# HazyResearch/flash-fft-conv

Measured on AMD Instinct MI355X. Metric: FFT-conv fwd+bwd seq/s, B=16 H=768 L=16384 fft=32768 bf16, higher is better.
Workload: dtype bf16; 1 GPU; FlashFFTConv(32768) B=16 H=768 L=16384 bf16, fwd+bwd incl. k->k_f and dk (BASELINE configs[1]); heads_per_rank=768, parallelism=head-shard x1 (no collective)

## Files before the change

flash-fft-conv_amd/csrc/ffc_body.h:

```cpp
#pragma once
#include <stdint.h>

#include "ffc_layout.h"
#include "ffc_plan.h"

#ifndef FFC_FN
#define FFC_FN inline __attribute__((always_inline))
#endif

namespace ffc {

struct ConvArgs {
  const void* u;
  const void* pregate;
  const void* postgate;
  void* y;
  const void* kf;
  const uint8_t* tab;
  PlanTabs t;
  int B, H, L;
  int npair;
  int nchunk, ppc;
  int conj_kf;
  int fast;
// ... 67 lines not shown
  template <bool CONJ, bool AFORM>
  static FFC_FN void cmm(A16& ore, A16& oim, const Op& d, const Mat& F, int ms_lim = 2) {
#pragma unroll
    for (int ms = 0; ms < 2; ms++) {
      if (ms >= ms_lim) continue;
      const W4& fr = F.w[ms][0];
      const W4& fi_re = F.w[ms][CONJ ? 1 : 2];
      const W4& fi_im = F.w[ms][CONJ ? 2 : 1];
      if (AFORM) {
        B::template mfma<DT>(ore, d.r[ms], fr);
        B::template mfma<DT>(oim, d.r[ms], fi_im);
        B::template mfma<DT>(ore, d.i[ms], fi_re);
        B::template mfma<DT>(oim, d.i[ms], fr);
      } else {
        B::template mfma<DT>(ore, fr, d.r[ms]);
        B::template mfma<DT>(oim, fi_im, d.r[ms]);
        B::template mfma<DT>(ore, fi_re, d.i[ms]);
        B::template mfma<DT>(oim, fr, d.i[ms]);
      }
    }
  }
  static FFC_FN void to_op(const A16& re, const A16& im, Op& o) {
#pragma unroll
    for (int ms = 0; ms < 2; ms++)
#pragma unroll
      for (int d = 0; d < 4; d++) {
        o.r[ms][d] = B::template pack<DT>(re[8 * ms + 2 * d], re[8 * ms + 2 * d + 1]);
        o.i[ms][d] = B::template pack<DT>(im[8 * ms + 2 * d], im[8 * ms + 2 * d + 1]);
      }
  }
  struct Mat2 { W4 w[2][2]; };
  static FFC_FN void load_mat2_issue(Mat2& m, const uint8_t* p, i32 lane) {
#pragma unroll
    for (int ms = 0; ms < 2; ms++)
#pragma unroll
      for (int f = 0; f < 2; f++) {
        U4 v = B::g_r128(p, lane + (ms * 3 + f) * 64);
        m.w[ms][f] = B::w4(v.x, v.y, v.z, v.w);
      }
  }
  static FFC_FN W4 neg4(const W4& x) {
    return B::w4(x[0] ^ B::uconst(0x80008000u), x[1] ^ B::uconst(0x80008000u), x[2] ^ B::uconst(0x80008000u), x[3] ^ B::uconst(0x80008000u));
  }
  template <bool AFORM>
  static FFC_FN void cmm2(A16& ore, A16& oim, const Op& d, const Mat2& F) {
#pragma unroll
    for (int ms = 0; ms < 2; ms++) {
      const W4 ni = neg4(d.i[ms]);
      if (AFORM) {
        B::template mfma<DT>(ore, d.r[ms], F.w[ms][0]);
        B::template mfma<DT>(oim, d.r[ms], F.w[ms][1]);
        B::template mfma<DT>(ore, ni, F.w[ms][1]);
        B::template mfma<DT>(oim, d.i[ms], F.w[ms][0]);
      } else {
        B::template mfma<DT>(ore, F.w[ms][0], d.r[ms]);
        B::template mfma<DT>(oim, F.w[ms][1], d.r[ms]);
        B::template mfma<DT>(ore, F.w[ms][1], ni);
        B::template mfma<DT>(oim, F.w[ms][0], d.i[ms]);
      }
    }
  }
  static FFC_FN void cmul(A16& re, A16& im, const CT16& t) { B::template cmul16<false>(re, im, t.re, t.im); }
  static FFC_FN void cmul_conj(A16& re, A16& im, const CT16& t) { B::template cmul16<true>(re, im, t.re, t.im); }
  static FFC_FN void cis_rev(i32 phase, float sign, f32* c, f32* s, int nmask = GEO::N - 1, float inv_n = 1.0f / (float)GEO::N) {
    f32 x = B::i2f(phase & nmask) * inv_n;
    f32 cc = B::cos_rev(x), ss = B::sin_rev(x);
    B::settle(cc, ss);
    *c = cc;
    *s = ss * sign;
  }
  static FFC_FN void chain8(i32 base, i32 step, float sign, float scale, f32 (&tr)[8], f32 (&ti)[8]) {
    f32 c0, s0, c1, s1, c8, s8;
    cis_rev(base, sign, &c0, &s0);
    cis_rev(step, sign, &c1, &s1);
    cis_rev(step * 8, sign, &c8, &s8);
    tr[0] = c0 * scale; ti[0] = s0 * scale;
    tr[4] = tr[0] * c8 - ti[0] * s8; ti[4] = tr[0] * s8 + ti[0] * c8;
#pragma unroll
    for (int i = 1; i < 4; i++) {
      tr[i] = tr[i - 1] * c1 - ti[i - 1] * s1; ti[i] = tr[i - 1] * s1 + ti[i - 1] * c1;
      tr[4 + i] = tr[3 + i] * c1 - ti[3 + i] * s1; ti[4 + i] = tr[3 + i] * s1 + ti[3 + i] * c1;
    }
  }
  using F2 = typename B::F2;
  static FFC_FN void chain8p(i32 base, i32 step, float sign, float scale, F2 (&tr)[4], F2 (&ti)[4],
                             int nmask = GEO::N - 1, float inv_n = 1.0f / (float)GEO::N, f32* w8c = nullptr, f32* w8s = nullptr) {
    f32 c0, s0, c1, s1, c8, s8;
    cis_rev(base, sign, &c0, &s0, nmask, inv_n);
    cis_rev(step, sign, &c1, &s1, nmask, inv_n);
    cis_rev(step * 8, sign, &c8, &s8, nmask, inv_n);
    c0 = c0 * scale; s0 = s0 * scale;
    f32 c2 = c1 * c1 - s1 * s1, s2 = (c1 + c1) * s1;
    tr[0] = B::f2(c0, c0 * c1 - s0 * s1);
    ti[0] = B::f2(s0, c0 * s1 + s0 * c1);
    B::cmulp(tr[0], ti[0], c2, s2, tr[1], ti[1]);
    B::cmulp(tr[0], ti[0], c8, s8, tr[2], ti[2]);
    B::cmulp(tr[1], ti[1], c8, s8, tr[3], ti[3]);
    if (w8c) { *w8c = c8; *w8s = s8; }
  }
  static FFC_FN void apply8(A16& re, A16& im, int half, const F2 (&tr)[4], const F2 (&ti)[4]) {
#pragma unroll
    for (int i = 0; i < 4; i++) B::template cmul2v<false>(re, im, 8 * half + 2 * i, tr[i], ti[i]);
  }
  static constexpr bool CHAIN16_A = GEO::N1 == 32 && (!B::LEAN_OUTER || GEO::N2 == 32);
  static FFC_FN void twiddle16(A16& re, A16& im, i32 base, i32 step, float sign, float scale,
                               int nmask = GEO::N - 1, float inv_n = 1.0f / (float)GEO::N) {
    F2 tr[4], ti[4];
    f32 c8, s8;
    chain8p(base, step, sign, scale, tr, ti, nmask, inv_n, &c8, &s8);
    apply8(re, im, 0, tr, ti);
    const f32 c16 = c8 * c8 - s8 * s8, s16 = (c8 + c8) * s8;
#pragma unroll
    for (int i = 0; i < 4; i++) B::cmulp(tr[i], ti[i], c16, s16, tr[i], ti[i]);
    apply8(re, im, 1, tr, ti);
  }
#ifndef FFC_PK_GATE
#define FFC_PK_GATE 1
#endif
  static FFC_FN u32 mul2(u32 a, u32 g) {
    if constexpr (DT == DT_F16 && FFC_PK_GATE != 0) return B::pk_mul_f16(a, g);
    f32 lo = B::template unpack_lo<DT>(a) * B::template unpack_lo<DT>(g);
    f32 hi = B::template unpack_hi<DT>(a) * B::template unpack_hi<DT>(g);
    return B::template pack<DT>(lo, hi);
  }
  static FFC_FN void xpose(const U2 (&raw)[8], int t, W4& op) {
#pragma unroll
    for (int d = 0; d < 4; d++) {
      u32 a = (t < 2) ? raw[2 * d].x : raw[2 * d].y;
      u32 b = (t < 2) ? raw[2 * d + 1].x : raw[2 * d + 1].y;
      op[d] = (t & 1) ? ((a >> 16) | (b & 0xffff0000u)) : ((a & 0xffffu) | (b << 16));
    }
  }

  static FFC_FN void xpose2(const U2 (&raw)[8], int tp, int th, W4& op) {
#pragma unroll
    for (int d = 0; d < 4; d++) {
      u32 a = tp ? raw[2 * d].y : raw[2 * d].x;
      u32 b = tp ? raw[2 * d + 1].y : raw[2 * d + 1].x;
      op[d] = th ? ((a >> 16) | (b & 0xffff0000u)) : ((a & 0xffffu) | (b << 16));
    }
  }

  static FFC_FN void copy_tab(const uint8_t* src, int lds_off, int bytes) {
    const i32 tid = B::lane() + B::wave() * 64;
    for (int i = 0; i < bytes / 16; i += GEO::WGW * 64) {
      i32 idx = tid + i;
      pred ok = idx < bytes / 16;
      U4 v = B::g_r128p(src, idx, ok);
      B::lds_w128(idx * 16 + lds_off, v, ok);
    }
  }
  static constexpr int TAB_T = GEO::WGW * 64;
  template <int BYTES>
  static FFC_FN void tab_issue(const uint8_t* src, U4 (&v)[(BYTES / 16 + TAB_T - 1) / TAB_T]) {
    const i32 tid = B::lane() + B::wave() * 64;
#pragma unroll
    for (int it = 0; it < (BYTES / 16 + TAB_T - 1) / TAB_T; it++) v[it] = B::g_r128(src, B::imin(tid + it * TAB_T, BYTES / 16 - 1));
  }
  template <int BYTES>
  static FFC_FN void tab_commit(int lds_off, const U4 (&v)[(BYTES / 16 + TAB_T - 1) / TAB_T]) {
    const i32 tid = B::lane() + B::wave() * 64;
#pragma unroll
    for (int it = 0; it < (BYTES / 16 + TAB_T - 1) / TAB_T; it++) {
      i32 idx = tid + it * TAB_T;
      B::lds_w128(idx * 16 + lds_off, v[it], idx < BYTES / 16);
    }
  }
  static FFC_FN void setup_tables(const uint8_t* tab, const PlanTabs& t) {
    U4 f1[(6144 / 16 + TAB_T - 1) / TAB_T], f2[(6144 / 16 + TAB_T - 1) / TAB_T], f3[(6144 / 16 + TAB_T - 1) / TAB_T],
       tw[(8192 / 16 + TAB_T - 1) / TAB_T], tw2[(8192 / 16 + TAB_T - 1) / TAB_T], fs[(3072 / 16 + TAB_T - 1) / TAB_T];
    if constexpr (GEO::OUTER) tab_issue<6144>(tab + t.mat[0], f1);
    tab_issue<6144>(tab + t.mat[1], f2);
    tab_issue<8192>(tab + t.twin, tw);
    if constexpr (GEO::N3 != GEO::N2) tab_issue<6144>(tab + t.mat[2], f3);
    if constexpr (GEO::TW2_SEP) tab_issue<8192>(tab + t.twin2, tw2);
    if constexpr (GEO::HAS_SP) tab_issue<3072>(tab + t.mat_sp, fs);
    B::sched_fence();
    if constexpr (GEO::OUTER) tab_commit<6144>(GEO::L_F1, f1);
    tab_commit<6144>(GEO::L_F2, f2);
    tab_commit<8192>(GEO::L_TW, tw);
    if constexpr (GEO::N3 != GEO::N2) tab_commit<6144>(GEO::L_F3, f3);
    if constexpr (GEO::TW2_SEP) tab_commit<8192>(GEO::L_TW2, tw2);
    if constexpr (GEO::HAS_SP) tab_commit<3072>(GEO::L_FS, fs);
    B::barrier();
  }
  static FFC_FN void lds_mat(Mat& m, int off) {
    const i32 lane = B::lane();
#pragma unroll
    for (int q = 0; q < 6; q++) {
      U4 v = B::lds_r128(lane * 16 + (off + q * 1024));
      m.w[q / 3][q % 3] = B::w4(v.x, v.y, v.z, v.w);
    }
#pragma unroll
    for (int q = 0; q < 6; q++) B::pin(m.w[q / 3][q % 3]);
  }
  static FFC_FN void lds_ct16(CT16& c, int off) {
    const i32 lane = B::lane();
#pragma unroll
    for (int rr = 0; rr < 8; rr++) {
      U4 v = B::lds_r128(lane * 16 + (off + rr * 1024));
      c.re[2 * rr] = B::as_f32(v.x); c.re[2 * rr + 1] = B::as_f32(v.y);
      c.im[2 * rr] = B::as_f32(v.z); c.im[2 * rr + 1] = B::as_f32(v.w);
    }
  }
  template <bool CONJ>
  static FFC_FN void cmul_lds(A16& re, A16& im, int off) {
    const i32 lane = B::lane();
#pragma unroll
    for (int rr = 0; rr < 8; rr++) {
      U4 v = B::lds_r128(lane * 16 + (off + rr * 1024));
      B::template cmul2<CONJ>(re, im, 2 * rr, B::as_f32(v.x), B::as_f32(v.y), B::as_f32(v.z), B::as_f32(v.w));
    }
  }
  static FFC_FN void cmul_small(CT16& t, int off) {
    const i32 hi = B::lane() >> 5;
#pragma unroll
    for (int rr = 0; rr < 8; rr++) {
      U4 v = B::lds_r128(hi * 128 + (off + rr * 16));
      f32 br[2] = {B::as_f32(v.x), B::as_f32(v.z)}, bi[2] = {B::as_f32(v.y), B::as_f32(v.w)};
#pragma unroll
      for (int q = 0; q < 2; q++) {
        int r = 2 * rr + q;
        f32 x = t.re[r], y = t.im[r];
        t.re[r] = x * br[q] - y * bi[q];
        t.im[r] = x * bi[q] + y * br[q];
      }
    }
  }

  struct Unit { int eb; int wq; };
  static FFC_FN Pass make_pass(const ConvArgs& a, int k0) {
    Pass ps;
    ps.k0 = k0; ps.R = a.R;
    ps.mat_fwd = a.tab + a.t.matk[k0][0]; ps.mat_inv = a.tab + a.t.matk[k0][1];
    return ps;
  }

  static FFC_FN int64_t row_off(int b, bool ok, int64_t sb, int h, int L) { return (int64_t)(ok ? b : 0) * sb + (int64_t)h * L; }
  struct RowIO {
    const uint16_t* src[2]; const uint16_t* gate[2]; uint16_t* dst[2]; bool valid[2];
  };
  static FFC_FN U4 gload8(const uint16_t* base, i32 n, int L, int fast, bool rowok) {
    if (B::FAST_ONLY || fast) return fast == 2 ? B::g_r128_nt(base, B::imin(n, L - 8) >> 3) : B::g_r128(base, B::imin(n, L - 8) >> 3);
    u32 w[4];
#pragma unroll
    for (int q = 0; q < 4; q++) {
      u32 lo = B::g_r16(base, n + 2 * q, ((n + 2 * q) < L) && rowok);
      u32 hi = B::g_r16(base, n + (2 * q + 1), ((n + (2 * q + 1)) < L) && rowok);
      w[q] = lo | (hi << 16);
    }
    U4 v; v.x = w[0]; v.y = w[1]; v.z = w[2]; v.w = w[3];
    return v;
  }
  static FFC_FN void gstore8(uint16_t* base, i32 n, int L, int fast, bool rowok, U4 v) {
    if (B::FAST_ONLY || fast) {
      if (fast == 2) B::g_w128_nt(base, n >> 3, v, (n < L) && rowok);
      else B::g_w128(base, n >> 3, v, (n < L) && rowok);
      return;
    }
    u32 w[4] = {v.x, v.y, v.z, v.w};
#pragma unroll
    for (int q = 0; q < 4; q++) {
      B::g_w16(base, n + 2 * q, w[q] & 0xffffu, ((n + 2 * q) < L) && rowok);
      B::g_w16(base, n + (2 * q + 1), w[q] >> 16, ((n + (2 * q + 1)) < L) && rowok);
    }
  }
  static FFC_FN i32 pair_off(i32 row, i32 m, pred* swapped) {
    i32 n2 = m / GEO::N3, n3 = m % GEO::N3;
    i32 sig = (n2 / GEO::PER) % GEO::CR;
    *swapped = (sig & 1) >= 1;
    return row * (GEO::Mi * 2) + (n2 * GEO::CR + (((n3 >> 3) ^ (sig >> 1)) << 1)) * 8;
  }
  static constexpr int CPR = GEO::OUTER ? 16 * GEO::S1 : GEO::Mi / 8;
  static constexpr int NCH = GEO::OUTER ? 8 : 2;

  template <int NC> struct RowRegsT { U4 v[NC][2]; };
  using RowRegs = RowRegsT<NCH>;
  template <int NC, int I0 = 0>
  static FFC_FN void rows_load(const ConvArgs& a, int h, int pq, Unit un, RowRegsT<NC>& X) {
    const i32 lane = B::opaque(B::lane());
    const int fast = a.fast ? (a.stream ? 2 : 1) : 0;
    if constexpr (!GEO::OUTER) {
      if (fast) {
#pragma unroll
        for (int ii = 0; ii < NC; ii++) {
          i32 idx = lane + (ii + I0) * 64;
          i32 row = idx / CPR, m = (idx % CPR) * 8;
#pragma unroll
          for (int pl = 0; pl < 2; pl++) {
            i32 b = (row + pq * GEO::G) * 2 + pl;
            X.v[ii][pl] = gload8_rows((const uint16_t*)a.u, b, h, a, a.sbu, m, 1, b < a.B);
          }
        }
        return;
      }
    }
#pragma unroll
    for (int ii = 0; ii < NC; ii++) {
      const int i = ii + I0;
      i32 idx = lane + i * 64;
      i32 row = idx / CPR, m = (idx % CPR) * 8 + (GEO::OUTER ? un.wq * 128 * GEO::S1 : 0);
#pragma unroll
      for (int pl = 0; pl < 2; pl++) {
        if constexpr (GEO::OUTER) {
          if (fast && ((i * 64) / CPR) * GEO::Mi >= a.L) { X.v[ii][pl] = U4{B::uconst(0), B::uconst(0), B::uconst(0), B::uconst(0)}; continue; }
          const int b = 2 * pq + pl;
          const bool ok = b < a.B;
          const int64_t ro = row_off(b, ok, a.sbu, h, a.L);
          X.v[ii][pl] = gload8((const uint16_t*)a.u + ro, row * GEO::Mi + m, a.L, fast, ok);
        } else {
          i32 b = (row + pq * GEO::G) * 2 + pl;
          X.v[ii][pl] = gload8_rows((const uint16_t*)a.u, b, h, a, a.sbu, m, fast, b < a.B);
        }
      }
    }
  }
#ifndef FFC_GATE_BATCH
#define FFC_GATE_BATCH 4
#endif
  template <int NC, int I0>
  static FFC_FN void rows_store_g(const ConvArgs& a, int h, int pq, Unit un, const RowRegsT<NC>& X) {
    constexpr int GB = FFC_GATE_BATCH <= 0 ? 1 : (NC < FFC_GATE_BATCH ? NC : FFC_GATE_BATCH);
    static_assert(NC % GB == 0, "gate batch");
    const i32 lane = B::opaque(B::lane());
    const int fast = a.stream ? 2 : 1;
    const bool hasg = a.pregate != nullptr, hasa = a.aux_in != nullptr;
#pragma unroll
    for (int ib = 0; ib < NC; ib += GB) {
      U4 G[GB][2], A[GB][2];
#pragma unroll
      for (int jj = 0; jj < GB; jj++) {
        const int i = ib + jj + I0;
        i32 idx = lane + i * 64;
        i32 row = idx / CPR, m = (idx % CPR) * 8 + (GEO::OUTER ? un.wq * 128 * GEO::S1 : 0);
        if (GEO::OUTER && ((i * 64) / CPR) * GEO::Mi >= a.L) continue;
#pragma unroll
        for (int pl = 0; pl < 2; pl++) {
          if constexpr (GEO::OUTER) {
            const int b = 2 * pq + pl;
            const bool ok = b < a.B;
            const i32 n = row * GEO::Mi + m;
            if (hasg) G[jj][pl] = gload8((const uint16_t*)a.pregate + row_off(b, ok, a.sbg, h, a.L), n, a.L, fast, ok);
            if (hasa) A[jj][pl] = gload8((const uint16_t*)a.aux_in + row_off(b, ok, a.sbai, h, a.L), n, a.L, fast, ok);
          } else {
            i32 b = (row + pq * GEO::G) * 2 + pl;
            if (hasg) G[jj][pl] = gload8_rows((const uint16_t*)a.pregate, b, h, a, a.sbg, m, fast, b < a.B);
            if (hasa) A[jj][pl] = gload8_rows((const uint16_t*)a.aux_in, b, h, a, a.sbai, m, fast, b < a.B);
          }
        }
      }
      B::sched_fence();
#pragma unroll
      for (int jj = 0; jj < GB; jj++) {
        const int ii = ib + jj, i = ii + I0;
        i32 idx = lane + i * 64;
        i32 row = idx / CPR, m = (idx % CPR) * 8 + (GEO::OUTER ? un.wq * 128 * GEO::S1 : 0);
        pred sw;
        i32 off = pair_off(row, m, &sw) + un.eb;
        const bool beyond = GEO::OUTER && ((i * 64) / CPR) * GEO::Mi >= a.L;
#pragma unroll
        for (int pl = 0; pl < 2; pl++) {
          U4 v = X.v[ii][pl];
          if (GEO::OUTER) {
            pred ok = ((row * GEO::Mi + m) < a.L) && ((2 * pq + pl) < a.B);
            v.x = B::sel(ok, v.x, B::uconst(0)); v.y = B::sel(ok, v.y, B::uconst(0));
            v.z = B::sel(ok, v.z, B::uconst(0)); v.w = B::sel(ok, v.w, B::uconst(0));
          }
          if (hasa && !beyond) {
            if constexpr (GEO::OUTER) {
              const int b = 2 * pq + pl;
              const bool ok = b < a.B;
              gstore8((uint16_t*)a.aux_out + row_off(b, ok, a.sbao, h, a.L), row * GEO::Mi + m, a.L, fast, ok, mul4(v, A[jj][pl]));
            } else {
              i32 b = (row + pq * GEO::G) * 2 + pl;
              gstore8_rows((uint16_t*)a.aux_out, b, h, a, a.sbao, m, fast, b < a.B, mul4(v, A[jj][pl]));
            }
          }
          if (hasg && !beyond) v = mul4(v, G[jj][pl]);
          U4 o;
          o.x = B::sel(sw, v.z, v.x); o.y = B::sel(sw, v.w, v.y);
          o.z = B::sel(sw, v.x, v.z); o.w = B::sel(sw, v.y, v.w);
          B::lds_w128(off + pl * GEO::PLANE, o, B::ptrue());
        }
      }
    }
  }
  template <int NC, int I0 = 0>
  static FFC_FN void rows_store(const ConvArgs& a, int h, int pq, Unit un, const RowRegsT<NC>& X) {
    if constexpr (FFC_GATE_BATCH > 0) {
      if (a.fast && (a.pregate || a.aux_in)) { rows_store_g<NC, I0>(a, h, pq, un, X); return; }
    }
    const i32 lane = B::opaque(B::lane());
    const int fast = a.fast ? (a.stream ? 2 : 1) : 0;
#pragma unroll
    for (int ii = 0; ii < NC; ii++) {
      const int i = ii + I0;
      i32 idx = lane + i * 64;
      i32 row = idx / CPR, m = (idx % CPR) * 8 + (GEO::OUTER ? un.wq * 128 * GEO::S1 : 0);
      pred sw;
      i32 off = pair_off(row, m, &sw) + un.eb;
#pragma unroll
      for (int pl = 0; pl < 2; pl++) {
        U4 v = X.v[ii][pl];
        if (fast && GEO::OUTER) {
          pred ok = ((row * GEO::Mi + m) < a.L) && ((2 * pq + pl) < a.B);
          v.x = B::sel(ok, v.x, B::uconst(0)); v.y = B::sel(ok, v.y, B::uconst(0));
          v.z = B::sel(ok, v.z, B::uconst(0)); v.w = B::sel(ok, v.w, B::uconst(0));
        }
        if (a.aux_in && !(GEO::OUTER && fast && ((i * 64) / CPR) * GEO::Mi >= a.L)) {
          if constexpr (GEO::OUTER) {
            const int b = 2 * pq + pl;
            const bool ok = b < a.B;
            const i32 n = row * GEO::Mi + m;
            U4 r = gload8((const uint16_t*)a.aux_in + row_off(b, ok, a.sbai, h, a.L), n, a.L, fast, ok);
            gstore8((uint16_t*)a.aux_out + row_off(b, ok, a.sbao, h, a.L), n, a.L, fast, ok, mul4(v, r));
          } else {
            i32 b = (row + pq * GEO::G) * 2 + pl;
            U4 r = gload8_rows((const uint16_t*)a.aux_in, b, h, a, a.sbai, m, fast, b < a.B);
            gstore8_rows((uint16_t*)a.aux_out, b, h, a, a.sbao, m, fast, b < a.B, mul4(v, r));
          }
        }
        if (a.pregate && !(GEO::OUTER && fast && ((i * 64) / CPR) * GEO::Mi >= a.L)) {
          U4 g;
          if constexpr (GEO::OUTER) {
            const int b = 2 * pq + pl;
            const bool ok = b < a.B;
            const int64_t ro = row_off(b, ok, a.sbg, h, a.L);
            g = gload8((const uint16_t*)a.pregate + ro, row * GEO::Mi + m, a.L, fast, ok);
          } else {
            i32 b = (row + pq * GEO::G) * 2 + pl;
            g = gload8_rows((const uint16_t*)a.pregate, b, h, a, a.sbg, m, fast, b < a.B);
          }
          v.x = mul2(v.x, g.x); v.y = mul2(v.y, g.y); v.z = mul2(v.z, g.z); v.w = mul2(v.w, g.w);
        }
        U4 o;
        o.x = B::sel(sw, v.z, v.x); o.y = B::sel(sw, v.w, v.y);
        o.z = B::sel(sw, v.x, v.z); o.w = B::sel(sw, v.y, v.w);
        B::lds_w128(off + pl * GEO::PLANE, o, B::ptrue());
      }
    }
  }
  template <int NC = NCH>
  static FFC_FN void rows_in(const ConvArgs& a, int h, int pq, Unit un) {
    RowRegsT<NC> X;
    rows_load<NC>(a, h, pq, un, X);
    rows_store<NC>(a, h, pq, un, X);
  }
  static constexpr bool HAS_DMA = GEO::OUTER && GEO::N1 == 32 && GEO::S1 == 1;
  static constexpr int DMA_ROW0 = GEO::N1 / 2;
  static FFC_FN void rows_dma(const ConvArgs& a, int h, int pq, Unit un) {
    if (a.stream) rows_dma_t<true>(a, h, pq, un);
    else rows_dma_t<false>(a, h, pq, un);
  }
  template <bool NT>
  static FFC_FN void rows_dma_t(const ConvArgs& a, int h, int pq, Unit un) {
    const i32 lane = B::opaque(B::lane());
#pragma unroll
    for (int pl = 0; pl < 2; pl++) {
      const int b = 2 * pq + pl;
      const uint16_t* base = (const uint16_t*)a.u + row_off(b < a.B ? b : a.B - 1, true, a.sbu, h, a.L);
#pragma unroll
      for (int r = 0; r < GEO::N1 / 2; r++) {
        i32 n = B::imin(lane * 2 + (r * GEO::Mi + un.wq * 128), a.L - 2);
        B::template g2lds32<NT>(base, n >> 1, un.eb + pl * GEO::PLANE + (DMA_ROW0 + r) * (GEO::Mi * 2) + un.wq * 256);
      }
    }
  }
  static FFC_FN void rows_dma_finish(const ConvArgs& a, int pq, Unit un) {
    B::vm_wait0();
    const i32 lane = B::opaque(B::lane());
#pragma unroll
    for (int pl = 0; pl < 2; pl++) {
      const bool ok = (2 * pq + pl) < a.B;
#pragma unroll
      for (int r = 0; r < GEO::N1 / 2; r++) {
        if (ok && (r + 1) * GEO::Mi <= a.L) continue;
        i32 n = lane * 2 + (r * GEO::Mi + un.wq * 128);
        B::lds_w32p(lane * 4 + (un.eb + pl * GEO::PLANE + (DMA_ROW0 + r) * (GEO::Mi * 2) + un.wq * 256), B::uconst(0),
                    B::pnot((n < a.L) && ok));
      }
    }
    B::lds_fence();
  }

  static FFC_FN U4 gload8_rows(const uint16_t* base, i32 b, int h, const ConvArgs& a, int64_t sb, i32 n, int fast, pred ok) {
    const int sbi = (int)sb;
    if (fast) {
      i32 o16 = b * (sbi >> 3) + (h * (a.L >> 3) + (n >> 3));
      return B::g_r128p(base, o16, ok && (n < a.L));
    }
    u32 w[4];
#pragma unroll
    for (int q = 0; q < 4; q++) {
      i32 e0 = b * sbi + (h * a.L + n + 2 * q);
      u32 lo = B::g_r16(base, e0, ok && ((n + 2 * q) < a.L));
      u32 hi = B::g_r16(base, e0 + 1, ok && ((n + (2 * q + 1)) < a.L));
      w[q] = lo | (hi << 16);
    }
    U4 v; v.x = w[0]; v.y = w[1]; v.z = w[2]; v.w = w[3];
    return v;
  }
  static FFC_FN void gstore8_rows(uint16_t* base, i32 b, int h, const ConvArgs& a, int64_t sb, i32 n, int fast, pred ok, U4 v) {
    const int sbi = (int)sb;
    if (fast) {
      i32 o16 = b * (sbi >> 3) + (h * (a.L >> 3) + (n >> 3));
      B::g_w128(base, o16, v, ok && (n < a.L));
      return;
    }
    u32 w[4] = {v.x, v.y, v.z, v.w};
#pragma unroll
    for (int q = 0; q < 4; q++) {
      i32 e0 = b * sbi + (h * a.L + n + 2 * q);
      B::g_w16(base, e0, w[q] & 0xffffu, ok && ((n + 2 * q) < a.L));
      B::g_w16(base, e0 + 1, w[q] >> 16, ok && ((n + (2 * q + 1)) < a.L));
    }
  }

#ifndef FFC_GATE_BATCH_OUT
#define FFC_GATE_BATCH_OUT FFC_GATE_BATCH
#endif
  template <int NC, bool ADD = false, bool GATE = true>
  static FFC_FN void rows_out_g(const ConvArgs& a, int h, int pq, Unit un) {
    static_assert(ADD || GATE, "rows_out_g: nothing to load");
    constexpr int GB = FFC_GATE_BATCH_OUT <= 0 ? 1 : (NC < FFC_GATE_BATCH_OUT ? NC : FFC_GATE_BATCH_OUT);
    static_assert(NC % GB == 0, "gate batch");
    const i32 lane = B::opaque(B::lane());
    const int fast = a.stream ? 2 : 1;
#pragma unroll
    for (int ib = 0; ib < NC; ib += GB) {
      U4 G[GB][2], Rr[GB][2];
#pragma unroll
      for (int jj = 0; jj < GB; jj++) {
        const int i = ib + jj;
        i32 idx = lane + i * 64;
        i32 row = idx / CPR, m = (idx % CPR) * 8 + (GEO::OUTER ? un.wq * 128 * GEO::S1 : 0);
#pragma unroll
        for (int pl = 0; pl < 2; pl++) {
          if constexpr (GEO::OUTER) {
            const int b = 2 * pq + pl;
            const bool ok = b < a.B;
            if constexpr (GATE) G[jj][pl] = gload8((const uint16_t*)a.postgate + row_off(b, ok, a.sbp, h, a.L), row * GEO::Mi + m, a.L, fast, ok);
            if constexpr (ADD) Rr[jj][pl] = gload8((const uint16_t*)a.addend + row_off(b, ok, a.sba, h, a.L), row * GEO::Mi + m, a.L, fast, ok);
          } else {
            i32 b = (row + pq * GEO::G) * 2 + pl;
            if constexpr (GATE) G[jj][pl] = gload8_rows((const uint16_t*)a.postgate, b, h, a, a.sbp, m, fast, b < a.B);
            if constexpr (ADD) Rr[jj][pl] = gload8_rows((const uint16_t*)a.addend, b, h, a, a.sba, m, fast, b < a.B);
          }
        }
      }
      B::sched_fence();
#pragma unroll
      for (int jj = 0; jj < GB; jj++) {
        const int i = ib + jj;
        i32 idx = lane + i * 64;
        i32 row = idx / CPR, m = (idx % CPR) * 8 + (GEO::OUTER ? un.wq * 128 * GEO::S1 : 0);
        pred sw;
        i32 off = pair_off(row, m, &sw) + un.eb;
#pragma unroll
        for (int pl = 0; pl < 2; pl++) {
          U4 o = B::lds_r128(off + pl * GEO::PLANE);
          U4 v;
          v.x = B::sel(sw, o.z, o.x); v.y = B::sel(sw, o.w, o.y);
          v.z = B::sel(sw, o.x, o.z); v.w = B::sel(sw, o.y, o.w);
          if constexpr (ADD && GATE) v = fma4(v, G[jj][pl], Rr[jj][pl]);
          else if constexpr (ADD) v = sum4(v, Rr[jj][pl]);
          else v = mul4(v, G[jj][pl]);
          if constexpr (GEO::OUTER) {
            const int b = 2 * pq + pl;
            const bool ok = b < a.B;
            gstore8((uint16_t*)a.y + row_off(b, ok, a.sby, h, a.L), row * GEO::Mi + m, a.L, fast, ok, v);
          } else {
            i32 b = (row + pq * GEO::G) * 2 + pl;
            gstore8_rows((uint16_t*)a.y, b, h, a, a.sby, m, fast, b < a.B, v);
          }
        }
      }
    }
  }
  template <int NC = NCH, bool ADD = B::HAS_ADD>
  static FFC_FN void rows_out(const ConvArgs& a, int h, int pq, Unit un) {
    if constexpr (FFC_GATE_BATCH > 0) {
      if (a.fast && a.postgate) { rows_out_g<NC, ADD>(a, h, pq, un); return; }
      if constexpr (ADD) {
        if (a.fast) { rows_out_g<NC, true, false>(a, h, pq, un); return; }
      }
    }
    const i32 lane = B::opaque(B::lane());
    const int fast = a.fast ? (a.stream ? 2 : 1) : 0;
#pragma unroll
    for (int i = 0; i < NC; i++) {
      i32 idx = lane + i * 64;
      i32 row = idx / CPR, m = (idx % CPR) * 8 + (GEO::OUTER ? un.wq * 128 * GEO::S1 : 0);
      pred sw;
      i32 off = pair_off(row, m, &sw) + un.eb;
#pragma unroll
      for (int pl = 0; pl < 2; pl++) {
        U4 o = B::lds_r128(off + pl * GEO::PLANE);
        U4 v;
        v.x = B::sel(sw, o.z, o.x); v.y = B::sel(sw, o.w, o.y);
// ... 1202 lines not shown
    kf_mul<SZ>(a, kfB, reB, imB); to_op(reB, imB, opB);
    reB = B::a16_zero(); imB = B::a16_zero();
    cmm<true, true>(reB, imB, opB, R.F2);
    cmul_conj(reA, imA, R.tw); to_op(reA, imA, opA);
    reA = B::a16_zero(); imA = B::a16_zero();
    cmm<true, true>(reA, imA, opA, R.F2);
    cmul_conj(reB, imB, R.tw); to_op(reB, imB, opB);
    reB = B::a16_zero(); imB = B::a16_zero();
    cmm<true, true>(reB, imB, opB, R.F2);
    oi_twiddle<RP>(a.s_inv, tauA, reA, imA, ps);
    tile_store(tauA, R, reA, imA);
    oi_twiddle<RP>(a.s_inv, tauB, reB, imB, ps);
    tile_store(tauB, R, reB, imB);
  }

  template <bool SZ>
  static FFC_FN void inner_tile2x_fold(const ConvArgs& a, int h, int tau, const InnerRegs& R, Unit un, uint8_t* zsA, uint8_t* zsB) {
    static_assert(CAN_FOLD && GEO::UPW >= 2, "folded outer twiddle, two units per workgroup");
    constexpr int DB = GEO::EBYTES;
    const i32 lane = B::opaque(B::lane());
    const uint8_t* fold = a.tab + a.t.fold;
    Mat2 FA, FB, GB, GA;
    load_mat2_issue(FA, fold + (0 * GEO::NT + tau) * 6144, lane);
    KfRegs kf;
    load_kf(a, h, tau, kf);
    Op opA, opB;
    load_tile_op(tau, opA, un, R);
    load_tile_op(tau, opB, un, R, DB);
    load_mat2_issue(FB, fold + (1 * GEO::NT + tau) * 6144, lane);
    A16 reA, imA, reB, imB;
    reA = B::a16_zero(); imA = B::a16_zero();
    cmm2<true>(reA, imA, opA, FA);
    reB = B::a16_zero(); imB = B::a16_zero();
    cmm2<true>(reB, imB, opB, FA);
    load_mat2_issue(GB, fold + (2 * GEO::NT + tau) * 6144, lane);
    cmul(reA, imA, R.tw); to_op(reA, imA, opA);
    reA = B::a16_zero(); imA = B::a16_zero();
    cmm2<false>(reA, imA, opA, FB);
    cmul(reB, imB, R.tw); to_op(reB, imB, opB);
    reB = B::a16_zero(); imB = B::a16_zero();
    cmm2<false>(reB, imB, opB, FB);
    load_mat2_issue(GA, fold + (3 * GEO::NT + tau) * 6144, lane);
    if constexpr (SZ) { z_store(zsA, tau, reA, imA, Z_STREAM); z_store(zsB, tau, reB, imB, Z_STREAM); }
    {
      CT16 k;
#pragma unroll
      for (int rq = 0; rq < 4; rq++) {
        u32 wv[4] = {kf.v[rq].x, kf.v[rq].y, kf.v[rq].z, kf.v[rq].w};
#pragma unroll
        for (int q = 0; q < 4; q++) {
          k.re[4 * rq + q] = B::template unpack_lo<DT>(wv[q]);
          k.im[4 * rq + q] = B::template unpack_hi<DT>(wv[q]);
        }
      }
      if constexpr (!SZ) k.im = B::a16_scale(k.im, a.conj_kf ? -1.0f : 1.0f);
      cmul(reA, imA, k); to_op(reA, imA, opA);
      reA = B::a16_zero(); imA = B::a16_zero();
      cmm2<true>(reA, imA, opA, GB);
      cmul(reB, imB, k); to_op(reB, imB, opB);
      reB = B::a16_zero(); imB = B::a16_zero();
      cmm2<true>(reB, imB, opB, GB);
    }
    cmul_conj(reA, imA, R.tw); to_op(reA, imA, opA);
    reA = B::a16_zero(); imA = B::a16_zero();
    cmm2<true>(reA, imA, opA, GA);
    cmul_conj(reB, imB, R.tw); to_op(reB, imB, opB);
    reB = B::a16_zero(); imB = B::a16_zero();
    cmm2<true>(reB, imB, opB, GA);
    tile_store(tau, R, reA, imA);
    tile_store(tau, R, reB, imB, DB);
  }
  template <bool SZ = false>
  static FFC_FN void inner_tile2x(const ConvArgs& a, int h, int tau, const InnerRegs& R, Unit un, uint8_t* zsA = nullptr, uint8_t* zsB = nullptr) {
    static_assert(GEO::N3 == GEO::N2 && GEO::OUTER && GEO::UPW >= 2, "inner_tile2x: two units per workgroup");
    constexpr int DB = GEO::EBYTES;
    KfRegs kf;
    load_kf(a, h, tau, kf);
    Op opA, opB;
    load_tile_op(tau, opA, un, R);
    load_tile_op(tau, opB, un, R, DB);
    A16 reA, imA, reB, imB;
    reA = B::a16_zero(); imA = B::a16_zero();
    cmm<false, true>(reA, imA, opA, R.F2);
    reB = B::a16_zero(); imB = B::a16_zero();
    cmm<false, true>(reB, imB, opB, R.F2);
    cmul(reA, imA, R.tw); to_op(reA, imA, opA);
    reA = B::a16_zero(); imA = B::a16_zero();
    cmm<false, false>(reA, imA, opA, R.F2);
    cmul(reB, imB, R.tw); to_op(reB, imB, opB);
    reB = B::a16_zero(); imB = B::a16_zero();
    cmm<false, false>(reB, imB, opB, R.F2);
    if constexpr (SZ) { z_store(zsA, tau, reA, imA, Z_STREAM); z_store(zsB, tau, reB, imB, Z_STREAM); }
    {
      CT16 k;
#pragma unroll
      for (int rq = 0; rq < 4; rq++) {
        u32 wv[4] = {kf.v[rq].x, kf.v[rq].y, kf.v[rq].z, kf.v[rq].w};
#pragma unroll
        for (int q = 0; q < 4; q++) {
          k.re[4 * rq + q] = B::template unpack_lo<DT>(wv[q]);
          k.im[4 * rq + q] = B::template unpack_hi<DT>(wv[q]);
        }
      }
      if constexpr (!SZ) k.im = B::a16_scale(k.im, a.conj_kf ? -1.0f : 1.0f);
      cmul(reA, imA, k); to_op(reA, imA, opA);
      reA = B::a16_zero(); imA = B::a16_zero();
      cmm<true, true>(reA, imA, opA, R.F2);
      cmul(reB, imB, k); to_op(reB, imB, opB);
      reB = B::a16_zero(); imB = B::a16_zero();
      cmm<true, true>(reB, imB, opB, R.F2);
    }
    cmul_conj(reA, imA, R.tw); to_op(reA, imA, opA);
    reA = B::a16_zero(); imA = B::a16_zero();
    cmm<true, true>(reA, imA, opA, R.F2);
    cmul_conj(reB, imB, R.tw); to_op(reB, imB, opB);
    reB = B::a16_zero(); imB = B::a16_zero();
    cmm<true, true>(reB, imB, opB, R.F2);
    {
      const i32 lane = B::opaque(B::lane());
      const i32 c = lane & 31, hi = lane >> 5;
      const i32 sUl = c / GEO::N2, mlane = (c % GEO::N2) * GEO::N3;
      if constexpr (GEO::N3 == 32) {
        i32 k1 = sUl * GEO::SV + tau * GEO::G;
        F2 tr[4], ti[4];
        f32 c8, s8;
        chain8p(B::mul24(mlane + hi * 4, k1), k1, 1.0f, a.s_inv, tr, ti, GEO::N - 1, 1.0f / (float)GEO::N, &c8, &s8);
        apply8(reA, imA, 0, tr, ti);
        apply8(reB, imB, 0, tr, ti);
        const f32 c16 = c8 * c8 - s8 * s8, s16 = (c8 + c8) * s8;
#pragma unroll
        for (int i = 0; i < 4; i++) B::cmulp(tr[i], ti[i], c16, s16, tr[i], ti[i]);
        apply8(reA, imA, 1, tr, ti);
        apply8(reB, imB, 1, tr, ti);
      } else
#pragma unroll
      for (int half = 0; half < 2; half++) {
        const int sV = (16 * half) / GEO::N3;
        i32 k1 = sUl * GEO::SV + (sV + tau * GEO::G);
        i32 n30 = hi * 4 + ((16 * half) % GEO::N3);
        F2 tr[4], ti[4];
        chain8p(B::mul24(mlane + n30, k1), k1, 1.0f, a.s_inv, tr, ti);
        apply8(reA, imA, half, tr, ti);
        apply8(reB, imB, half, tr, ti);
      }
    }
    tile_store(tau, R, reA, imA);
    tile_store(tau, R, reB, imB, DB);
  }

  static FFC_FN void unit_barrier() {
    if constexpr (GEO::NW > 1) B::barrier();
    else B::lds_fence();
  }
  template <bool HALF, bool PROF = false, bool RP = false, bool SZ = false, bool SP = false, bool GS = false>
  static FFC_FN void outer_jobs(const ConvArgs& a, int h, int p0, int p1, int u, Unit un, int wg_linear = 0) {
    static_assert(!GS || (HALF && !RP && !SP && HALF_C), "direct-store phase C: single-pass fft 32768, L <= N/2");
    constexpr int NC = HALF ? NCH / 2 : NCH;
    constexpr bool PREFETCH = HALF && !RP;
    constexpr bool FOLDF = CAN_FOLD && !RP && !SP && !PROF && !B::LEAN_OUTER;
    constexpr bool CROSS = !SP && !RP && !PROF && !B::LEAN_OUTER && GEO::N3 == GEO::N2 && GEO::NW > 1 && GEO::UPW >= 2;
    const int npass = RP ? a.R : 1;
    const int iters = ((p1 - p0 + GEO::UPW - 1) / GEO::UPW) * npass;
    RowRegsT<NC> X;
    if constexpr (PREFETCH) { if (p0 + u < p1) rows_load<NC>(a, h, p0 + u, un, X); }
    unsigned long long acc[8] = {0, 0, 0, 0, 0, 0, 0, 0}, t0 = 0, t1 = 0;
#define FFC_TICK(k) if (PROF) { t1 = B::clock(); acc[k] += t1 - t0; t0 = t1; }
    const bool second = B::wave() >= 4;
#define FFC_PRIO(x) if constexpr (GEO::NW > 1) B::template setprio<x>();
#pragma unroll 1
    for (int it = 0; it < iters; it++) {
      const int p = p0 + (RP ? it / npass : it) * GEO::UPW + u;
      const Pass ps = RP ? make_pass(a, it % npass) : Pass();
      const int hk = RP ? h * ps.R + ps.k0 : h;
      const bool act = p < p1;
      if (PROF) t0 = B::clock();
      FFC_PRIO(1)
      if (act) {
        if constexpr (RP) {
          rows_in_rp<NC>(a, h, p, un, ps);
        } else {
          if constexpr (!PREFETCH) rows_load<NC>(a, h, p, un, X);
          rows_store<NC>(a, h, p, un, X);
        }
        B::lds_fence();
        FFC_TICK(0)
        FFC_PRIO(0)
        outer_stage<true, HALF, RP, false, FOLDF>(a.L, un, a.s_fwd, ps);
        FFC_TICK(1)
      }
      unit_barrier();
      FFC_TICK(2)
      if constexpr (CROSS) {
        const int ug = u >> 1, wl = (u & 1) * GEO::NW + un.wq;
        const int pA = p0 + it * GEO::UPW + 2 * ug;
        if (pA < p1) {
          Unit ua;
          ua.eb = 2 * ug * GEO::EBYTES; ua.wq = wl;
          InnerRegs R;
          load_inner(R, ua);
          uint8_t* zA = SZ ? z_slot(a.zsave, h, a.npair, pA) : nullptr;
          if (pA + 1 < p1) {
#pragma unroll 1
            for (int tt = 0; tt < 2; tt++) {
              if (tt == 0) { FFC_PRIO(3) } else if (second) { FFC_PRIO(2) } else { FFC_PRIO(1) }
              if constexpr (FOLDF) inner_tile2x_fold<SZ>(a, hk, wl * 2 + tt, R, ua, zA, zA + (int64_t)GEO::N * 4);
              else inner_tile2x<SZ>(a, hk, wl * 2 + tt, R, ua, zA, zA + (int64_t)GEO::N * 4);
            }
          } else {
            inner_tile2<false, SZ, FOLDF, HALF>(a, hk, wl * 2, R, ua, Pass(), zA);
          }
        }
      } else if (act) {
        InnerRegs R;
        load_inner(R, un);
        if constexpr (SP) {
          Mat Fs;
          lds_mat_sp(Fs);
#pragma unroll 1
          for (int tt = 0; tt < GEO::TPW; tt += 2) inner_tile2_sp(a, hk, un.wq * GEO::TPW + tt, R, Fs, un);
        } else if constexpr (GEO::N3 == GEO::N2) {
#pragma unroll 1
          for (int tt = 0; tt < GEO::TPW; tt += 2) {
            if (tt == 0) { FFC_PRIO(3) } else if (second) { FFC_PRIO(2) } else { FFC_PRIO(1) }
            inner_tile2<RP, SZ, FOLDF, HALF>(a, hk, un.wq * GEO::TPW + tt, R, un, ps,
                                SZ ? (RP ? z_slot_rp(a.zsave, h, a.npair, p, ps.R, ps.k0) : z_slot(a.zsave, h, a.npair, p)) : nullptr);
          }
        } else {
          KfRegs kf0;
          load_kf(a, h, un.wq * GEO::TPW, kf0);
#pragma unroll 1
          for (int tt = 0; tt < GEO::TPW; tt++) {
            KfRegs kfn;
            if (tt + 1 < GEO::TPW) load_kf(a, h, un.wq * GEO::TPW + tt + 1, kfn);
            inner_tile(a, un.wq * GEO::TPW + tt, R, un, kf0);
            kf0 = kfn;
          }
        }
      }
      FFC_TICK(3)
      unit_barrier();
      FFC_TICK(4)
      FFC_PRIO(3)
      if constexpr (PREFETCH) { if (it + 1 < iters && p + GEO::UPW < p1) rows_load<NC>(a, h, p + GEO::UPW, un, X); }
      if constexpr (GS) {
        if (act) {
          outer_inv_half<true>(un, &a, h, p);
          FFC_TICK(5)
        }
      } else if (act) {
        outer_stage<false, HALF, RP>(a.L, un, 1.0f, ps, a.flags);
        B::lds_fence();
        FFC_TICK(5)
        FFC_PRIO(2)
        if constexpr (SZ) {
          if (a.yraw) {
            ConvArgs ar = a;
            ar.y = a.yraw; ar.postgate = nullptr; ar.addend = nullptr; ar.sby = (int64_t)a.H * a.L;
            if constexpr (RP) rows_out_rp<NC, false>(ar, h, p, un, ps);
            else rows_out<NC, false>(ar, h, p, un);
          }
        }
        if constexpr (RP) rows_out_rp<NC>(a, h, p, un, ps);
        else rows_out<NC>(a, h, p, un);
        FFC_TICK(6)
      }
    }
#undef FFC_TICK
#undef FFC_PRIO
    if (PROF && a.prof) {
      const i32 lane = B::lane();
      unsigned long long* dst = a.prof + ((long long)wg_linear * GEO::WGW + B::wave()) * 8;
#pragma unroll
      for (int k = 0; k < 8; k++) B::g_w64(dst, lane * 0 + k, B::u2_from64(acc[k]), lane < 1);
    }
  }

  template <bool HALF = false, bool SZ = false, bool SP = false, bool GS = false>
  static FFC_FN void conv(const ConvArgs& a, int h, int chunk) {
    setup_tables(a.tab, a.t);
    conv_job<HALF, false, SZ, SP, GS>(a, h, chunk);
  }
  template <bool HALF = false, bool RP = false, bool SZ = false, bool SP = false, bool GS = false>
  static FFC_FN void conv_job(const ConvArgs& a, int h, int chunk) {
    const int wv = B::wave();
    Unit un;
    un.wq = wv % GEO::NW;
    const int u = wv / GEO::NW;
    un.eb = u * GEO::EBYTES;
    const int p0 = chunk * a.ppc;
    int p1 = p0 + a.ppc;
    if (p1 > a.npair) p1 = a.npair;
    if constexpr (GEO::OUTER) {
      outer_jobs<HALF, false, RP, SZ, SP, GS>(a, h, p0, p1, u, un);
    } else {
      const int q0 = p0 / GEO::G, q1 = (p1 + GEO::G - 1) / GEO::G;
      const int iters = (q1 - q0 + GEO::UPW - 1) / GEO::UPW;
      InnerRegs R;
      load_inner(R, un);
      if constexpr (RP) {
        static_assert(GEO::G == 1, "inner-only multi-pass: one pair per tile");
#ifndef FFC_IP_MERGE
#define FFC_IP_MERGE 1
#endif
        if (FFC_IP_MERGE != 0 && a.fast && a.L <= GEO::N && !a.aux_in) {
          const i32 lane = B::opaque(B::lane());
#pragma unroll 1
          for (int it = 0; it < iters; it++) {
            const int q = q0 + it * GEO::UPW + u;
            if (q >= q1) continue;
            RowRegs X, Y;
            rows_load<NCH>(a, h, q, un, X);
            if (a.pregate) {
              RowRegs G;
#pragma unroll
              for (int ii = 0; ii < NCH; ii++) {
                i32 idx = lane + ii * 64;
                i32 m = (idx % CPR) * 8;
#pragma unroll
                for (int pl = 0; pl < 2; pl++) {
                  i32 b = (idx / CPR + q * GEO::G) * 2 + pl;
                  G.v[ii][pl] = gload8_rows((const uint16_t*)a.pregate, b, h, a, a.sbg, m, 1, b < a.B);
                }
              }
#pragma unroll
              for (int ii = 0; ii < NCH; ii++)
#pragma unroll
                for (int pl = 0; pl < 2; pl++) X.v[ii][pl] = mul4(X.v[ii][pl], G.v[ii][pl]);
            }
#pragma unroll 1
            for (int k0 = 0; k0 < a.R; k0++) {
              InnerPass ip;
              load_inner_pass(ip, k0);
              KfRegs kf;
              load_kf(a, h * a.R + k0, 0, kf);
#pragma unroll
              for (int ii = 0; ii < NCH; ii++) {
                i32 idx = lane + ii * 64;
                pred sw;
                i32 off = pair_off(idx / CPR, (idx % CPR) * 8, &sw) + un.eb;
#pragma unroll
                for (int pl = 0; pl < 2; pl++) {
                  const U4& v = X.v[ii][pl];
                  U4 o;
                  o.x = B::sel(sw, v.z, v.x); o.y = B::sel(sw, v.w, v.y);
                  o.z = B::sel(sw, v.x, v.z); o.w = B::sel(sw, v.y, v.w);
                  B::lds_w128(off + pl * GEO::PLANE, o, B::ptrue());
                }
              }
              B::lds_fence();
              inner_tile<true, SZ>(a, 0, R, un, kf, &ip, (SZ && a.zsave) ? z_slot_small(a.zsave, h, a.npair, q, a.R, k0) : nullptr);
              B::lds_fence();
#pragma unroll
              for (int ii = 0; ii < NCH; ii++) {
                i32 idx = lane + ii * 64;
                pred sw;
                i32 off = pair_off(idx / CPR, (idx % CPR) * 8, &sw) + un.eb;
#pragma unroll
                for (int pl = 0; pl < 2; pl++) {
                  U4 o = B::lds_r128(off + pl * GEO::PLANE);
                  U4 v;
                  v.x = B::sel(sw, o.z, o.x); v.y = B::sel(sw, o.w, o.y);
                  v.z = B::sel(sw, o.x, o.z); v.w = B::sel(sw, o.y, o.w);
                  if (k0 == 0) Y.v[ii][pl] = v;
                  else Y.v[ii][pl] = add4(Y.v[ii][pl], v, 1.0f);
                }
              }
              B::lds_fence();
            }
#pragma unroll
            for (int ii = 0; ii < NCH; ii++) {
              i32 idx = lane + ii * 64;
              i32 m = (idx % CPR) * 8;
#pragma unroll
              for (int pl = 0; pl < 2; pl++) {
                i32 b = (idx / CPR + q * GEO::G) * 2 + pl;
                U4 v = Y.v[ii][pl];
                if constexpr (SZ) {
                  if (a.yraw) gstore8_rows((uint16_t*)a.yraw, b, h, a, (int64_t)a.H * a.L, m, 1, b < a.B, v);
                }
                if constexpr (B::HAS_ADD) {
                  U4 r = gload8_rows((const uint16_t*)a.addend, b, h, a, a.sba, m, 1, b < a.B);
                  if (a.postgate) v = fma4(v, gload8_rows((const uint16_t*)a.postgate, b, h, a, a.sbp, m, 1, b < a.B), r);
                  else v = sum4(v, r);
                } else {
                  if (a.postgate) v = mul4(v, gload8_rows((const uint16_t*)a.postgate, b, h, a, a.sbp, m, 1, b < a.B));
                }
                gstore8_rows((uint16_t*)a.y, b, h, a, a.sby, m, 1, b < a.B, v);
              }
            }
          }
          return;
        }
#pragma unroll 1
        for (int it = 0; it < iters * a.R; it++) {
          const int q = q0 + (it / a.R) * GEO::UPW + u;
          const int k0 = it % a.R;
          if (q < q1) {
            Pass ps; ps.k0 = k0; ps.R = a.R;
            InnerPass ip;
            load_inner_pass(ip, k0);
            KfRegs kf;
            load_kf(a, h * a.R + k0, 0, kf);
            rows_in_rp<NCH>(a, h, q, un, ps);
            B::lds_fence();
            inner_tile<true, SZ>(a, 0, R, un, kf, &ip, (SZ && a.zsave) ? z_slot_small(a.zsave, h, a.npair, q, a.R, k0) : nullptr);
            B::lds_fence();
            if constexpr (SZ) {
              if (a.yraw) {
                ConvArgs ar = a;
                ar.y = a.yraw; ar.postgate = nullptr; ar.addend = nullptr; ar.sby = (int64_t)a.H * a.L;
                rows_out_rp<NCH, false>(ar, h, q, un, ps);
              }
            }
            rows_out_rp<NCH>(a, h, q, un, ps);
            B::lds_fence();
          }
        }
        return;
      }
#pragma unroll 1
      for (int it = 0; it < iters; it++) {
        const int q = q0 + it * GEO::UPW + u;
        const bool act = q < q1;
        if (act) {
          KfRegs kf;
          load_kf(a, h, 0, kf);
          rows_in(a, h, q, un);
          B::lds_fence();
          inner_tile<false, SZ>(a, 0, R, un, kf, nullptr, (SZ && a.zsave) ? z_slot_small(a.zsave, h, a.npair, q, 1, 0) : nullptr);
          B::lds_fence();
          if constexpr (SZ) {
            if (a.yraw) {
              ConvArgs ar = a;
              ar.y = a.yraw; ar.postgate = nullptr; ar.addend = nullptr; ar.sby = (int64_t)a.H * a.L;
              rows_out<NCH, false>(ar, h, q, un);
            }
          }
          rows_out(a, h, q, un);
        }
      }
    }
  }
};

}
```

flash-fft-conv_amd/csrc/ffc_bwd_launch.h:

```cpp
#pragma once
#ifndef FFC_GATE_BATCH
#define FFC_GATE_BATCH 1
#define FFC_GATE_BATCH_OUT 2
#endif
#include "ffc_dev.h"
using namespace ffc;

template <class GEO, int DT, bool HALF, int ZM, bool GS = false>
__global__ __launch_bounds__(GEO::WGW * 64, 2) __attribute__((amdgpu_num_vgpr(128))) void bwd_kernel(DkfArgs d) {
  if constexpr (GEO::NW == 1) {
    const int total = ((d.c.H + 7) & ~7) * d.c.nchunk;
    for (int id = blockIdx.x; id < total; id += gridDim.x) {
      int h, chunk;
      if (map_id(id, d.c.H, d.c.nchunk, &h, &chunk)) Modes<DevBO, GEO, DT>::template bwd<HALF, false, true, ZM>(d, h, chunk, blockIdx.x);
    }
  } else {
    int h, chunk;
    if (!map_block(d.c.H, d.c.nchunk, &h, &chunk)) return;
    stagger_start(d.c.flags);
    Modes<DevBO, GEO, DT>::template bwd<HALF, false, true, ZM, GS>(d, h, chunk, blockIdx.x);
  }
}
template <class GEO, int DT>
__global__ __launch_bounds__(GEO::WGW * 64, 2) void bwd_kernel_small(DkfArgs d) {
  using M = Modes<DevB, GEO, DT>;
  M::BD::setup_tables(d.c.tab, d.c.t);
  if constexpr (GEO::N == 1024) { if (d.c.R > 1) M::BD::setup_tables_ipass(d.c.tab, d.c.t, d.c.R); }
  const int total = ((d.c.H + 7) & ~7) * d.c.nchunk;
  for (int id = blockIdx.x; id < total; id += gridDim.x) {
    int h, chunk;
    if (map_id(id, d.c.H, d.c.nchunk, &h, &chunk)) M::template bwd<false, false, false>(d, h, chunk, id);
  }
}
template <class GEO, int DT, bool HALF, int ZM, bool FASTK>
__global__ __launch_bounds__(GEO::WGW * 64, 2) __attribute__((amdgpu_num_vgpr(128))) void bwd_rp_kernel(DkfArgs d) {
  using BK = typename std::conditional<FASTK, DevBOF, DevBO>::type;
  int h, chunk;
  if (!map_block(d.c.H, d.c.nchunk, &h, &chunk)) return;
  Modes<BK, GEO, DT>::BD::setup_tables(d.c.tab, d.c.t);
  const int wv = DevBO::wave(), wg = blockIdx.x;
#pragma unroll 1
  for (int k0 = 0; k0 < d.c.R; k0++) Modes<BK, GEO, DT>::template bwd<HALF, true, true, ZM>(d, h, chunk, wg, k0, wv);
}

template <int ZM>
struct BwdLaunchZ {
template <class GEO, int DT>
struct T {
  static int run(const DkfArgs& d, hipStream_t st) {
    static_assert(Body<DevB, GEO, DT>::IPASS_BYTES == IPASS_BYTES, "ffc_route.h");
    const BwdRoute r = bwd_route<GEO>(d, false);
    if (r.err) return ffc_fail(r.err);
    constexpr int T_ = GEO::WGW * 64;
    if constexpr (!GEO::OUTER && ZM != 0) {
      return ffc_fail("single-tile sizes are launched by the recomputing unit (run-time spectrum switch)");
    } else if constexpr (!GEO::OUTER) {
      return ffc_launch(bwd_kernel_small<GEO, DT>, "bwd_kernel", r.grid, T_, r.lds_max, r.lds, st, d);
    } else if (r.gs) {
      if constexpr (GEO::N == 32768)
        return ffc_launch(bwd_kernel<GEO, DT, true, ZM, true>, "bwd_kernel (direct store)", r.grid, T_, r.lds_max, r.lds, st, d);
      else
        return ffc_fail("internal: the backward route names a kernel that does not exist");
    } else {
      return pick([&](auto mp, auto half, auto fastk) -> int {
        constexpr bool MP = decltype(mp)::value, HALF = decltype(half)::value, FASTK = decltype(fastk)::value;
        if constexpr (MP && GEO::N == 32768)
          return ffc_launch(bwd_rp_kernel<GEO, DT, HALF, ZM, FASTK>, "bwd_rp_kernel", r.grid, T_, r.lds_max, r.lds, st, d);
        else if constexpr (!MP && !FASTK)
          return ffc_launch(bwd_kernel<GEO, DT, HALF, ZM>, "bwd_kernel", r.grid, T_, r.lds_max, r.lds, st, d);
        else
          return ffc_fail("internal: the backward route names a kernel that does not exist");
      }, r.multi_pass, r.half, r.fastk);
    }
  }
};
};
```

flash-fft-conv_amd/csrc/ffc_conv_launch.h:

```cpp
#pragma once
#include "ffc_dev.h"

template <class FAM>
struct ConvLaunch {
template <class GEO, int DT>
struct T {
  static int run(const ffc::ConvArgs& a, hipStream_t st) {
    using namespace ffc;
    static_assert(Body<DevB, GEO, DT>::IPASS_BYTES == IPASS_BYTES, "ffc_route.h");
    const FwdRoute r = fwd_route<GEO>(a);
    if (r.err) return ffc_fail(r.err);
    if (r.gs) {
      if constexpr (!FAM::HAS_ADD && GEO::N == 32768)
        return pick([&](auto sz) -> int {
          return ffc_launch(FAM::template kernel_gs<GEO, DT, decltype(sz)::value>(), FAM::what(false, decltype(sz)::value, false, true), r.grid, GEO::WGW * 64, r.lds_max, r.lds, st, a);
        }, r.sz);
      else
        return ffc_fail("internal: the forward route names a kernel that does not exist");
    }
    return pick([&](auto mp, auto half, auto sz, auto sp) -> int {
      constexpr bool MP = decltype(mp)::value, HALF = decltype(half)::value, SZ = decltype(sz)::value, SP = decltype(sp)::value;
      if constexpr (fwd_kernel_exists<GEO>(FAM::HAS_ADD, MP, HALF, SZ, SP))
        return ffc_launch(FAM::template kernel<GEO, DT, MP, HALF, SZ, SP>(), FAM::what(MP, SZ, SP, GEO::OUTER), r.grid, GEO::WGW * 64, r.lds_max, r.lds, st, a);
      else
        return ffc_fail("internal: the forward route names a kernel that does not exist");
    }, r.multi_pass, r.half, r.sz, r.sp);
  }
};
};
```

flash-fft-conv_amd/csrc/ffc_k_conv.hip:

```cpp
#include "ffc_conv_launch.h"
using namespace ffc;

static constexpr int SMALL_WAVES = 2;
template <class GEO, int DT, bool HALF, bool SZ = false, bool SP = false, bool GS = false>
__global__ __launch_bounds__(GEO::WGW * 64, GEO::OUTER ? 2 : SMALL_WAVES) void conv_kernel(ConvArgs a) {
  using BD = Body<DevB, GEO, DT>;
  if constexpr (GEO::OUTER && GEO::NW == 1) {
    BD::setup_tables(a.tab, a.t);
    const int total = ((a.H + 7) & ~7) * a.nchunk;
    for (int id = blockIdx.x; id < total; id += gridDim.x) {
      int h, chunk;
      if (map_id(id, a.H, a.nchunk, &h, &chunk)) BD::template conv_job<HALF, false, SZ>(a, h, chunk);
    }
  } else if constexpr (!GEO::OUTER) {
    BD::setup_tables(a.tab, a.t);
    const int total = ((a.H + 7) & ~7) * a.nchunk;
    for (int id = blockIdx.x; id < total; id += gridDim.x) {
      int h, chunk;
      if (map_id(id, a.H, a.nchunk, &h, &chunk)) BD::template conv_job<HALF, false, SZ>(a, h, chunk);
    }
  } else {
    int h, chunk;
    if (!map_block(a.H, a.nchunk, &h, &chunk)) return;
    stagger_start(a.flags);
    if constexpr (GEO::NW > 1 && !SP) {
      BD::setup_tables(a.tab, a.t);
      if (a.kfuse_k || a.kfuse_x) Modes<DevB, GEO, DT>::kfft_head(a, h);
      BD::template conv_job<HALF, false, SZ, SP, GS>(a, h, chunk);
    } else {
      BD::template conv<HALF, SZ, SP, GS>(a, h, chunk);
    }
  }
}

template <class GEO, int DT, bool HALF, bool SZ = false>
__global__ __launch_bounds__(GEO::WGW * 64, 2) void conv_rp_kernel(ConvArgs a) {
  using BD = Body<DevB, GEO, DT>;
  if constexpr (!GEO::OUTER) {
    BD::setup_tables(a.tab, a.t);
    BD::setup_tables_ipass(a.tab, a.t, a.R);
    const int total = ((a.H + 7) & ~7) * a.nchunk;
    for (int id = blockIdx.x; id < total; id += gridDim.x) {
      int h, chunk;
      if (map_id(id, a.H, a.nchunk, &h, &chunk)) BD::template conv_job<HALF, true, SZ>(a, h, chunk);
    }
  } else {
    int h, chunk;
    if (!map_block(a.H, a.nchunk, &h, &chunk)) return;
    BD::setup_tables(a.tab, a.t);
    BD::template conv_job<HALF, true, SZ>(a, h, chunk);
  }
}

struct ConvKernels {
  static constexpr bool HAS_ADD = false;
  template <class GEO, int DT, bool MP, bool HALF, bool SZ, bool SP>
  static constexpr auto kernel() {
    if constexpr (MP) return conv_rp_kernel<GEO, DT, HALF, SZ>;
    else return conv_kernel<GEO, DT, HALF, SZ, SP>;
  }
  template <class GEO, int DT, bool SZ>
  static constexpr auto kernel_gs() { return conv_kernel<GEO, DT, true, SZ, false, true>; }
  static const char* what(bool mp, bool sz, bool sp, bool outer) {
    if (mp) return sz && outer ? "conv_rp_kernel (spectrum-saving)" : "conv_rp_kernel";
    if (sz) return outer ? "conv_kernel (spectrum-saving)" : "conv_kernel (spectrum-saving, single tile)";
    return sp ? "conv_kernel (frequency-sparse)" : "conv_kernel";
  }
};
template __global__ void conv_kernel<Geo<1, 16, 16>, DT_BF16, true>(ConvArgs);
template __global__ void conv_kernel<Geo<1, 16, 16>, DT_F16, true>(ConvArgs);
template __global__ void conv_kernel<Geo<1, 16, 32>, DT_BF16, true>(ConvArgs);
template __global__ void conv_kernel<Geo<1, 16, 32>, DT_F16, true>(ConvArgs);
template __global__ void conv_kernel<Geo<1, 32, 32>, DT_BF16, true>(ConvArgs);
template __global__ void conv_kernel<Geo<1, 32, 32>, DT_F16, true>(ConvArgs);

static inline bool ffc_stride_ok(int64_t* sb, int64_t B, int64_t H, int64_t L) {
  if (*sb == 0) *sb = H * L;
  return *sb >= H * L && (B - 1) * *sb + H * L < ((int64_t)1 << 31);
}

extern "C" int64_t ffc_spectrum_bytes(const ffc_plan* p, int64_t B, int64_t H) {
  if (!p || B <= 0 || H <= 0) return 0;
  if (p->hp.N1 <= 1) {
    const int64_t G = (32 / p->hp.N2) * (32 / p->hp.N3);
    return H * (((B + 1) / 2 + G - 1) / G) * p->hp.R * 4096;
  }
  return ((B + 1) / 2) * H * (int64_t)p->hp.N * 4;
}

struct FwdCall {
  const void *u, *kf, *pregate, *postgate;
  void* y;
  int64_t B, H, L;
  void* stream;
  int conj_kf;
  int64_t sb_u, sb_pre, sb_post, sb_y;
  void *zsave, *yraw;
  int sparse;
  const void* addend; int64_t sb_add;
  const float* kfuse_k; int64_t kfuse_Lk;
  const void* kfuse_x; float kfuse_xscale;
};
static FwdCall fwd_call(const void* u, const void* kf, const void* pregate, const void* postgate, void* y, int64_t B, int64_t H, int64_t L,
                        void* stream) {
  FwdCall c{};
  c.u = u; c.kf = kf; c.pregate = pregate; c.postgate = postgate; c.y = y; c.B = B; c.H = H; c.L = L; c.stream = stream;
  return c;
}
static bool kfft_in_launch(const ffc_plan* p, int64_t B, int64_t H) {
  int nchunk = 0, ppc = 0;
  if (B > 0 && H > 0) ffc_choose_chunks(p, (int)H, (int)((B + 1) / 2), &nchunk, &ppc, true);
  return fwd_takes_kfft(p->hp, nchunk, 0, p->env_flags);
}

static int conv_fwd_impl(const ffc_plan* p, const FwdCall& c) {
  const void *u = c.u, *kf = c.kf, *pregate = c.pregate, *postgate = c.postgate, *addend = c.addend;
  void *y = c.y, *zsave = c.zsave;
  const int64_t B = c.B, H = c.H, L = c.L;
  const int sparse = c.sparse;
  int64_t sb_u = c.sb_u, sb_pre = c.sb_pre, sb_post = c.sb_post, sb_y = c.sb_y, sb_add = c.sb_add;
  if (!p || !u || !kf || !y) return ffc_fail("null arg");
  if (B <= 0 || H <= 0) return ffc_fail("empty batch/heads");
  if (L <= 0 || L > p->hp.N) return ffc_fail("L must be in (0, fft_size]");
  if ((uintptr_t)kf & 15) return ffc_fail("k_f must be 16-byte aligned");
  if (!ffc_stride_ok(&sb_u, B, H, L) || !ffc_stride_ok(&sb_pre, B, H, L) || !ffc_stride_ok(&sb_post, B, H, L) ||
      !ffc_stride_ok(&sb_y, B, H, L) || !ffc_stride_ok(&sb_add, B, H, L))
    return ffc_fail("tensor too large (>= 2^31 elements) or batch stride smaller than H*L");
  ConvArgs a{};
  a.u = u; a.pregate = pregate; a.postgate = postgate; a.y = y; a.kf = kf;
  a.tab = p->d_blob; a.t = p->hp.tabs;
  a.B = (int)B; a.H = (int)H; a.L = (int)L; a.npair = (int)((B + 1) / 2);
  a.sbu = sb_u; a.sbg = sb_pre; a.sbp = sb_post; a.sby = sb_y;
  a.addend = addend; a.sba = sb_add;
  a.conj_kf = c.conj_kf;
  a.zsave = zsave; a.yraw = (zsave || p->hp.N1 <= 1) ? c.yraw : nullptr;
  a.sparse = sparse;
  if (sparse && (sparse < 0 || sparse > 4 || zsave || p->hp.R > 1 || p->hp.N2 != 32 || p->hp.N3 != 32 || p->hp.N1 <= 1))
    return ffc_fail("frequency-sparse forward: fft 16384 / 32768, 1 <= rows <= 4, no spectrum buffer");
  if (zsave && (ffc_spectrum_bytes(p, B, H) == 0 || ((uintptr_t)zsave & 15))) return ffc_fail("spectrum buffer: unsupported plan or misaligned");
  a.s_inv = (float)p->hp.s_inv; a.s_fwd = (float)p->hp.s_fwd;
  a.flags = p->env_flags;
  a.fast = (L % 8 == 0) && !(((uintptr_t)u | (uintptr_t)y | (uintptr_t)pregate | (uintptr_t)postgate | (uintptr_t)addend) & 15) &&
           !((sb_u | sb_pre | sb_post | sb_y | sb_add) & 7);
  ffc_choose_chunks(p, a.H, a.npair, &a.nchunk, &a.ppc, true);
  a.persist = ffc_persist(p);
  a.R = p->hp.R;
  if (c.kfuse_k) {
    a.kfuse_k = c.kfuse_k; a.kfuse_Lk = (int)c.kfuse_Lk;
    a.kfuse_scale = (float)(p->hp.s_k / p->hp.s_fwd) / (p->hp.dtype == DT_F16 ? 256.f : 1.f);
    a.kfuse_fast = (c.kfuse_Lk % 4 == 0) && !((uintptr_t)c.kfuse_k & 15);
  }
  if (c.kfuse_x) { a.kfuse_x = c.kfuse_x; a.kfuse_scale = c.kfuse_xscale; a.kfuse_Lk = p->hp.N; a.kfuse_fast = 1; }
  a.stream = p->env_stream >= 0 ? p->env_stream : (p->hp.R > 1 ? 0 : 1);
  if (addend) return ffc_conv_res_launch(p->hp.N, p->hp.dtype, a, (hipStream_t)c.stream);
  return ffc_dispatch<ConvLaunch<ConvKernels>::T>(p->hp.N, p->hp.dtype, a, (hipStream_t)c.stream);
}

extern "C" int ffc_conv_fwd_strided(const ffc_plan* p, const void* u, const void* kf, const void* pregate, const void* postgate,
                                    void* y, int64_t B, int64_t H, int64_t L, int conj_kf, int64_t sb_u, int64_t sb_pre,
                                    int64_t sb_post, int64_t sb_y, void* stream) {
  FwdCall c = fwd_call(u, kf, pregate, postgate, y, B, H, L, stream);
  c.conj_kf = conj_kf; c.sb_u = sb_u; c.sb_pre = sb_pre; c.sb_post = sb_post; c.sb_y = sb_y;
  return conv_fwd_impl(p, c);
}
extern "C" int ffc_conv_fwd_z(const ffc_plan* p, const void* u, const void* kf, const void* pregate, const void* postgate, void* y,
                              void* zsave, void* y_raw, int64_t B, int64_t H, int64_t L, int64_t sb_u, int64_t sb_pre, int64_t sb_post,
                              int64_t sb_y, void* stream) {
  if (!zsave && !(y_raw && p && p->hp.N1 <= 1)) return ffc_fail("null spectrum buffer (y_raw alone: single-tile sizes, fft <= 2048)");
  if (y_raw && ((uintptr_t)y_raw & 15)) return ffc_fail("y_raw must be 16-byte aligned");
  FwdCall c = fwd_call(u, kf, pregate, postgate, y, B, H, L, stream);
  c.zsave = zsave; c.yraw = y_raw; c.sb_u = sb_u; c.sb_pre = sb_pre; c.sb_post = sb_post; c.sb_y = sb_y;
  return conv_fwd_impl(p, c);
}

extern "C" int ffc_conv_fwd_res(const ffc_plan* p, const void* u, const void* kf, const void* pregate, const void* postgate,
                                const void* addend, void* y, void* zsave, void* y_raw, int64_t B, int64_t H, int64_t L, int conj_kf,
                                int64_t sb_u, int64_t sb_pre, int64_t sb_post, int64_t sb_add, int64_t sb_y, void* stream) {
  if (!p) return ffc_fail("null arg");
  if (y_raw && !zsave && p->hp.N1 > 1) return ffc_fail("y_raw without a spectrum buffer: single-tile sizes only (fft <= 2048)");
  if (y_raw && ((uintptr_t)y_raw & 15)) return ffc_fail("y_raw must be 16-byte aligned");
  if ((zsave || y_raw) && conj_kf) return ffc_fail("spectrum buffer / y_raw: forward pass only (conj_kf = 0)");
  if (addend && y && B > 0 && H > 0 && L > 0) {
    const int64_t sa = sb_add ? sb_add : H * L, sy = sb_y ? sb_y : H * L;
    const uintptr_t a0 = (uintptr_t)addend, a1 = a0 + (uintptr_t)(((B - 1) * sa + H * L) * 2);
    const uintptr_t y0 = (uintptr_t)y, y1 = y0 + (uintptr_t)(((B - 1) * sy + H * L) * 2);
    if (a0 < y1 && y0 < a1) return ffc_fail("addend overlaps y");
  }
  FwdCall c = fwd_call(u, kf, pregate, postgate, y, B, H, L, stream);
  c.conj_kf = conj_kf; c.zsave = zsave; c.yraw = y_raw; c.addend = addend;
  c.sb_u = sb_u; c.sb_pre = sb_pre; c.sb_post = sb_post; c.sb_y = sb_y; c.sb_add = sb_add;
  return conv_fwd_impl(p, c);
}

extern "C" int ffc_conv_fwd_sparse(const ffc_plan* p, const void* u, const void* kf, const void* pregate, const void* postgate,
                                   void* y, int64_t B, int64_t H, int64_t L, int conj_kf, int rows, void* stream) {
  if (rows < 1) return ffc_fail("frequency-sparse forward: rows must be >= 1");
  FwdCall c = fwd_call(u, kf, pregate, postgate, y, B, H, L, stream);
  c.conj_kf = conj_kf; c.sparse = rows;
  return conv_fwd_impl(p, c);
}

extern "C" int ffc_conv_fwd(const ffc_plan* p, const void* u, const void* kf, const void* pregate, const void* postgate, void* y,
                            int64_t B, int64_t H, int64_t L, int conj_kf, void* stream) {
  return ffc_conv_fwd_strided(p, u, kf, pregate, postgate, y, B, H, L, conj_kf, 0, 0, 0, 0, stream);
}

template <class GEO, int DT, bool GS = false>
__global__ __launch_bounds__(GEO::WGW * 64, 2) void conv_prof_kernel(ConvArgs a) {
  int h, chunk;
  if (!map_block(a.H, a.nchunk, &h, &chunk)) return;
  using BD = Body<DevB, GEO, DT>;
  BD::setup_tables(a.tab, a.t);
  const int wv = DevB::wave();
  typename BD::Unit un;
  un.wq = wv % GEO::NW;
  const int u = wv / GEO::NW;
  un.eb = u * GEO::EBYTES;
  const int p0 = chunk * a.ppc;
  int p1 = p0 + a.ppc;
  if (p1 > a.npair) p1 = a.npair;
  if constexpr (GS) BD::template outer_jobs<true, true, false, false, false, true>(a, h, p0, p1, u, un, blockIdx.x);
  else if (16 * GEO::Mi >= a.L) BD::template outer_jobs<true, true>(a, h, p0, p1, u, un, blockIdx.x);
  else BD::template outer_jobs<false, true>(a, h, p0, p1, u, un, blockIdx.x);
}

extern "C" int ffc_conv_fwd_prof(const ffc_plan* p, const void* u, const void* kf, void* y, int64_t B, int64_t H, int64_t L,
                                 unsigned long long* prof, int* grid_out, void* stream) {
  if (!p || p->hp.N != 32768 || p->hp.dtype != DT_BF16) return ffc_fail("prof build: N=32768 bf16 only");
  using GEO = Geo<32, 32, 32>;
  ConvArgs a{};
  a.u = u; a.y = y; a.kf = kf; a.tab = p->d_blob; a.t = p->hp.tabs;
  a.B = (int)B; a.H = (int)H; a.L = (int)L; a.npair = (int)((B + 1) / 2); a.s_inv = (float)p->hp.s_inv; a.s_fwd = (float)p->hp.s_fwd;
  a.fast = (L % 8 == 0) && !(((uintptr_t)u | (uintptr_t)y) & 15);
  a.sbu = a.sbg = a.sbp = a.sby = H * L;
  a.flags = p->env_flags;
  a.prof = prof;
  ffc_choose_chunks(p, a.H, a.npair, &a.nchunk, &a.ppc);
  const FwdRoute r = fwd_route<GEO>(a);
  const int grid = r.grid;
  if (grid_out) *grid_out = grid;
  if (r.gs) return ffc_launch(conv_prof_kernel<GEO, DT_BF16, true>, "conv_prof_kernel", grid, GEO::WGW * 64, GEO::LDS_BYTES, GEO::LDS_BYTES, (hipStream_t)stream, a);
  return ffc_launch(conv_prof_kernel<GEO, DT_BF16>, "conv_prof_kernel", grid, GEO::WGW * 64, GEO::LDS_BYTES, GEO::LDS_BYTES, (hipStream_t)stream, a);
}

extern "C" int ffc_conv_fwd_k(const ffc_plan* p, const float* k, int64_t Lk, void* kf_out, const void* u, const void* pregate,
                              const void* postgate, void* y, void* zsave, void* y_raw, int64_t B, int64_t H, int64_t L, void* stream) {
  if (!p || !k || !kf_out) return ffc_fail("null arg");
  if (y_raw && ((uintptr_t)y_raw & 15)) return ffc_fail("y_raw must be 16-byte aligned");
  const bool fuse = kfft_in_launch(p, B, H) && Lk > 0 && Lk <= p->hp.N && H * Lk < ((int64_t)1 << 31);
  if (!fuse) {
    int rc = ffc_kernel_fft(p, k, H, Lk, kf_out, stream);
    if (rc) return rc;
  }
  FwdCall c = fwd_call(u, kf_out, pregate, postgate, y, B, H, L, stream);
  c.zsave = zsave; c.yraw = y_raw;
  if (fuse) { c.kfuse_k = k; c.kfuse_Lk = Lk; }
  return conv_fwd_impl(p, c);
}

extern "C" int ffc_conv_fwd_kx(const ffc_plan* p, const void* xpair, float scale, void* kf_out, const void* u, void* y, void* zsave,
                               int64_t B, int64_t H, int64_t L, void* stream) {
  if (!p || !xpair || !kf_out) return ffc_fail("null arg");
  const bool fuse = kfft_in_launch(p, B, H) && !((uintptr_t)xpair & 15);
  if (!fuse) {
    int rc = ffc_kernel_fft_c(p, xpair, H, kf_out, scale, stream);
    if (rc) return rc;
  }
  FwdCall c = fwd_call(u, kf_out, nullptr, nullptr, y, B, H, L, stream);
  c.zsave = zsave;
  if (fuse) { c.kfuse_x = xpair; c.kfuse_xscale = scale; }
  return conv_fwd_impl(p, c);
}
```

flash-fft-conv_amd/csrc/ffc_modes.h:

```cpp
#pragma once
#include "ffc_body.h"

namespace ffc {

struct KfArgs {
  const float* k;
  void* kf;
  const uint8_t* tab;
  PlanTabs t;
  int H, Lk;
  float scale;
  float s_fwd;
  float prescale;
  const void* xpair;
  int fast;
  int R;
};

struct DkfArgs {
  ConvArgs c;
  const void* dout;
  float* ws;
  int64_t sbd, sbdu, sbdpre, sbdpost;
  void* du;
// ... 688 lines not shown
    ConvArgs av = a;
    ConvArgs ad = a;
    ad.u = d.dout; ad.pregate = a.postgate; ad.sbu = d.sbd; ad.sbg = a.sbp;
    float* slab = RP ? d.ws + (((int64_t)chunk * a.H + h) * a.R + k0) * (GEO::NT * 2048)
                     : d.ws + ((int64_t)chunk * a.H + h) * (GEO::NT * 2048);
    InnerRegs R;
    if constexpr (GEO::OUTER) {
      const int iters = (p1 - p0 + GEO::UPW - 1) / GEO::UPW;
      uint8_t* zs = (uint8_t*)d.zscratch + ((int64_t)(wg_linear * GEO::UPW + u)) * (GEO::N * 4);
      WAcc W;
      w_acc_zero(W);
#pragma unroll 1
      for (int it = 0; it < iters; it++) {
        const int p = p0 + it * GEO::UPW + u;
        const bool act = p < p1;
        if (act) {
          if constexpr (RP) BD::template rows_in_rp<NCX>(av, h, p, un, ps);
          else BD::template rows_in<NCX>(av, h, p, un);
          B::lds_fence();
          BD::template outer_stage<true, HALF, RP>(a.L, un, a.s_fwd, ps);
        }
        BD::unit_barrier();
        if (act) {
          BD::template load_inner<false>(R, un);
#pragma unroll 1
          for (int tt = 0; tt < GEO::TPW; tt++) {
            A16 re, im;
            BD::template tile_fwd<false>(un.wq * GEO::TPW + tt, R, un, re, im);
            z_store(zs, un.wq * GEO::TPW + tt, re, im, (a.flags & 4) != 0);
          }
        }
        BD::unit_barrier();
        if (act) {
          if constexpr (RP) BD::template rows_in_rp<NCX>(ad, h, p, un, ps);
          else BD::template rows_in<NCX>(ad, h, p, un);
          B::lds_fence();
          BD::template outer_stage<true, HALF, RP>(a.L, un, a.s_fwd, ps);
        }
        BD::unit_barrier();
        if (act) {
          BD::template load_inner<false>(R, un);
          bwd_tiles<false, RP>(a, h, un, R, zs, slab, it == 0, W, ps);
        } else if (it == 0) {
#pragma unroll 1
          for (int tt = GEO::TPW; tt < GEO::TPW; tt++) w_zero(slab, un.wq * GEO::TPW + tt);
        }
        BD::unit_barrier();
      }
      w_acc_finish(slab, u, un, W);
    } else if (a.R > 1) {
      if constexpr (GEO::N == 1024) {
        BD::setup_tables_ipass(a.tab, a.t, a.R);
        const int q0 = p0, q1 = p1;
        const int iters = (q1 - q0 + GEO::UPW - 1) / GEO::UPW;
        BD::template load_inner<false>(R, un);
#pragma unroll 1
        for (int k0 = 0; k0 < a.R; k0++) {
          Pass ps; ps.k0 = k0; ps.R = a.R;
          InnerPass ip;
          BD::load_inner_pass_lean(ip, k0);
          A16 wre = B::a16_zero(), wim = B::a16_zero();
#pragma unroll 1
          for (int it = 0; it < iters; it++) {
            const int q = q0 + it * GEO::UPW + u;
            if (q < q1) {
              ZReg zv;
              A16 re, im;
              BD::template rows_in_rp<BD::NCH>(av, h, q, un, ps);
              B::lds_fence();
              BD::template tile_fwd<true, true, false, true>(0, R, un, re, im, &ip);
              z_pack(re, im, zv);
              B::lds_fence();
              BD::template rows_in_rp<BD::NCH>(ad, h, q, un, ps);
              B::lds_fence();
              BD::template tile_fwd<true, true, false, true>(0, R, un, re, im, &ip);
              w_add(wre, wim, zv, re, im);
              B::lds_fence();
            }
          }
          reduce_store_w(d.ws + (((int64_t)chunk * a.H + h) * a.R + k0) * 2048, u, wre, wim);
        }
      }
    } else {
      const int q0 = p0 / GEO::G, q1 = (p1 + GEO::G - 1) / GEO::G;
      const int iters = (q1 - q0 + GEO::UPW - 1) / GEO::UPW;
      BD::load_inner(R, un);
      A16 wre, wim;
      wre = B::a16_zero(); wim = B::a16_zero();
#pragma unroll 1
      for (int it = 0; it < iters; it++) {
        const int q = q0 + it * GEO::UPW + u;
        if (q < q1) {
          ZReg zv;
          A16 re, im;
          BD::rows_in(av, h, q, un);
          B::lds_fence();
          BD::tile_fwd(0, R, un, re, im);
          z_pack(re, im, zv);
          B::lds_fence();
          BD::rows_in(ad, h, q, un);
          B::lds_fence();
          BD::tile_fwd(0, R, un, re, im);
#pragma unroll
          for (int r = 0; r < 16; r++) {
            u32 pr = zv.r[r >> 1], pi = zv.i[r >> 1];
            f32 ur = (r & 1) ? B::template unpack_hi<DT>(pr) : B::template unpack_lo<DT>(pr);
            f32 ui = (r & 1) ? B::template unpack_hi<DT>(pi) : B::template unpack_lo<DT>(pi);
            wre[r] = wre[r] + (re[r] * ur + im[r] * ui);
            wim[r] = wim[r] + (im[r] * ur - re[r] * ui);
          }
          B::lds_fence();
        }
      }
      reduce_store_w(slab, u, wre, wim);
    }
  }
  static FFC_FN void z_unpack(const typename BD::KfRegs& z, A16& re, A16& im) {
#pragma unroll
    for (int rq = 0; rq < 4; rq++) {
      u32 wv[4] = {z.v[rq].x, z.v[rq].y, z.v[rq].z, z.v[rq].w};
#pragma unroll
      for (int q = 0; q < 4; q++) {
        re[4 * rq + q] = B::template unpack_lo<DT>(wv[q]);
        im[4 * rq + q] = B::template unpack_hi<DT>(wv[q]);
      }
    }
  }
  static FFC_FN void kf_plain_mul(const typename BD::KfRegs& kf, A16& re, A16& im) {
    typename BD::CT16 k;
#pragma unroll
    for (int rq = 0; rq < 4; rq++) {
      u32 wv[4] = {kf.v[rq].x, kf.v[rq].y, kf.v[rq].z, kf.v[rq].w};
#pragma unroll
      for (int q = 0; q < 4; q++) {
        k.re[4 * rq + q] = B::template unpack_lo<DT>(wv[q]);
        k.im[4 * rq + q] = B::template unpack_hi<DT>(wv[q]);
      }
    }
    BD::cmul(re, im, k);
  }
  static FFC_FN void kf_conj_mul(const typename BD::KfRegs& kf, A16& re, A16& im) {
    typename BD::CT16 k;
#pragma unroll
    for (int rq = 0; rq < 4; rq++) {
      u32 wv[4] = {kf.v[rq].x, kf.v[rq].y, kf.v[rq].z, kf.v[rq].w};
#pragma unroll
      for (int q = 0; q < 4; q++) {
        k.re[4 * rq + q] = B::template unpack_lo<DT>(wv[q]);
        k.im[4 * rq + q] = B::template unpack_hi<DT>(wv[q]);
      }
    }
    BD::cmul_conj(re, im, k);
  }
  template <bool HALF = false, bool RP = false, bool SETUP = true, int ZM = -1, bool GS = false>
  static FFC_FN void bwd(const DkfArgs& d, int h, int chunk, int wg_linear, int k0 = 0, int wv_in = 0) {
    static_assert(!GS || (HALF && !RP && BD::HALF_C), "direct-store phase C: single-pass fft 32768, L <= N/2");
    const ConvArgs& a = d.c;
    const Pass ps = RP ? make_pass(a.tab, a.t, a.R, k0) : Pass();
    const int hk = RP ? h * a.R + k0 : h;
    constexpr int NCX = HALF ? BD::NCH / 2 : BD::NCH;
    if constexpr (!RP && SETUP) BD::setup_tables(a.tab, a.t);
    const int wv = RP ? wv_in : B::wave();
    Unit un;
    un.wq = wv % GEO::NW;
    const int u = wv / GEO::NW;
    un.eb = u * GEO::EBYTES;
    const int p0 = chunk * a.ppc;
    int p1 = p0 + a.ppc;
    if (p1 > a.npair) p1 = a.npair;
    ConvArgs av = a;
    ConvArgs ad = a;
    ad.u = d.dout; ad.pregate = a.postgate; ad.sbu = d.sbd; ad.sbg = a.sbp;
    ConvArgs ao = a;
    ao.y = d.du; ao.postgate = a.pregate; ao.sby = d.sbdu; ao.sbp = a.sbg;
    ConvArgs ap = a;
    ap.y = d.dpre; ap.postgate = a.u; ap.sby = d.sbdpre; ap.sbp = a.sbu;
    ConvArgs aq = a;
    aq.y = d.dpost; aq.postgate = d.dout; aq.sby = d.sbdpost; aq.sbp = d.sbd;
    const bool dpost_tf = d.dpost != nullptr && d.yraw == nullptr;
    if constexpr (!(RP && GEO::OUTER)) {
      if (d.dpost && d.yraw) { ad.aux_in = d.yraw; ad.aux_out = d.dpost; ad.sbai = (int64_t)a.H * a.L; ad.sbao = d.sbdpost; }
    }
    float* slab = RP ? d.ws + (((int64_t)chunk * a.H + h) * a.R + k0) * (GEO::NT * 2048)
                     : d.ws + ((int64_t)chunk * a.H + h) * (GEO::NT * 2048);
    InnerRegs R;
    if constexpr (GEO::OUTER) {
      const int iters = (p1 - p0 + GEO::UPW - 1) / GEO::UPW;
      uint8_t* zs = (uint8_t*)d.zscratch + ((int64_t)(wg_linear * GEO::UPW + u)) * (GEO::N * 4);
      WAcc W;
      w_acc_zero(W);
      const bool have_z = ZM < 0 ? d.zin != nullptr : ZM == 1;
      constexpr bool FOLDZ = BD::CAN_FOLD && GEO::N1 == 32 && ZM == 1 && !RP;
      constexpr bool DMA_OK = BD::HAS_DMA && HALF && !RP && ZM != 0;
      const bool dma = DMA_OK && have_z && a.fast && !ad.pregate && !ad.aux_in && !dpost_tf && !(a.flags & 8);
      if constexpr (DMA_OK) { if (dma && p0 + u < p1) BD::rows_dma(ad, h, p0 + u, un); }
      const bool second = wv >= 4;
#define FFC_BPRIO(x) if constexpr (GEO::NW > 1) B::template setprio<x>();
#pragma unroll 1
      for (int it = 0; it < iters; it++) {
        const int p = p0 + it * GEO::UPW + u;
        const bool act = p < p1;
        FFC_BPRIO(1)
        const void* zp = !have_z ? (const void*)zs
                         : RP ? (const void*)BD::z_slot_rp(const_cast<void*>(d.zin), h, a.npair, act ? p : p0, a.R, k0)
                              : (const void*)BD::z_slot(const_cast<void*>(d.zin), h, a.npair, act ? p : p0);
        if (have_z) {
          if (dpost_tf) {
            BD::unit_barrier();
            if (act) {
              BD::template load_inner<false>(R, un);
#pragma unroll 1
              for (int tt = 0; tt < GEO::TPW; tt++) {
                const int tau = un.wq * GEO::TPW + tt;
                typename BD::KfRegs zv, kf;
                z_load(zp, tau, zv, BD::Z_STREAM);
                BD::load_kf(a, hk, tau, kf);
                A16 re, im;
                z_unpack(zv, re, im);
                kf_plain_mul(kf, re, im);
                BD::template tile_inv<false, RP>(a.s_inv, tau, R, un, re, im, 0, ps);
              }
            }
            BD::unit_barrier();
            if (act) {
              BD::template outer_stage<false, HALF, RP>(a.L, un, 1.0f, ps, a.flags);
              B::lds_fence();
              if constexpr (RP) BD::template rows_out_rp<NCX>(aq, h, p, un, ps);
              else BD::template rows_out<NCX>(aq, h, p, un);
            }
          }
          if (act) {
            bool done = false;
            if constexpr (DMA_OK) {
              if (dma) {
                BD::rows_dma_finish(ad, p, un);
                FFC_BPRIO(0)
                BD::template outer_stage<true, HALF, RP, true, FOLDZ>(a.L, un, a.s_fwd, ps);
                done = true;
              }
            }
            if (!done) {
              if constexpr (RP) BD::template rows_in_rp<NCX>(ad, h, p, un, ps);
              else BD::template rows_in<NCX>(ad, h, p, un);
              B::lds_fence();
              FFC_BPRIO(0)
              BD::template outer_stage<true, HALF, RP, false, FOLDZ>(a.L, un, a.s_fwd, ps);
            }
          }
        } else {
          if (act) {
            if constexpr (RP) BD::template rows_in_rp<NCX>(av, h, p, un, ps);
            else BD::template rows_in<NCX>(av, h, p, un);
            B::lds_fence();
            FFC_BPRIO(0)
            BD::template outer_stage<true, HALF, RP>(a.L, un, a.s_fwd, ps);
          }
          BD::unit_barrier();
          FFC_BPRIO(3)
          if (act) {
            BD::template load_inner<false>(R, un);
#pragma unroll 1
            for (int tt = 0; tt < GEO::TPW; tt++) {
              const int tau = un.wq * GEO::TPW + tt;
              A16 re, im;
              BD::template tile_fwd<false>(tau, R, un, re, im);
              z_store(zs, tau, re, im, (a.flags & 4) != 0);
              if (dpost_tf) {
                typename BD::KfRegs kf;
                BD::load_kf(a, hk, tau, kf);
                kf_plain_mul(kf, re, im);
                BD::template tile_inv<false, RP>(a.s_inv, tau, R, un, re, im, 0, ps);
              }
            }
          }
          BD::unit_barrier();
          FFC_BPRIO(1)
          if (dpost_tf) {
            if (act) {
              BD::template outer_stage<false, HALF, RP>(a.L, un, 1.0f, ps, a.flags);
              B::lds_fence();
              if constexpr (RP) BD::template rows_out_rp<NCX>(aq, h, p, un, ps);
              else BD::template rows_out<NCX>(aq, h, p, un);
            }
          }
          if (act) {
            if constexpr (RP) BD::template rows_in_rp<NCX>(ad, h, p, un, ps);
            else BD::template rows_in<NCX>(ad, h, p, un);
            B::lds_fence();
            FFC_BPRIO(0)
            BD::template outer_stage<true, HALF, RP>(a.L, un, a.s_fwd, ps);
          }
        }
        BD::unit_barrier();
        FFC_BPRIO(3)
        if (act) {
          BD::template load_inner<false>(R, un);
          bwd_tiles<true, RP, ZM == 1>(a, hk, un, R, zp, slab, it == 0, W, ps, have_z && BD::Z_STREAM, second);
        } else if (it == 0) {
#pragma unroll 1
          for (int tt = GEO::TPW; tt < GEO::TPW; tt++) w_zero(slab, un.wq * GEO::TPW + tt);
        }
        BD::unit_barrier();
        FFC_BPRIO(3)
        if constexpr (GS) {
          if (act) {
            BD::template outer_inv_half<true>(un, &ao, h, p, [&]() {
              if constexpr (DMA_OK) {
                if (dma && p + GEO::UPW < p1) { B::lds_wait0(); BD::rows_dma(ad, h, p + GEO::UPW, un); }
              }
            });
          }
        } else if (act) {
          BD::template outer_stage<false, HALF, RP>(a.L, un, 1.0f, ps, a.flags);
          B::lds_fence();
          if constexpr (DMA_OK) { if (dma && p + GEO::UPW < p1) BD::rows_dma(ad, h, p + GEO::UPW, un); }
          FFC_BPRIO(2)
          if constexpr (RP) {
            BD::template rows_out_rp<NCX>(ao, h, p, un, ps);
            if (d.dpre) BD::template rows_out_rp<NCX>(ap, h, p, un, ps);
          } else {
            BD::template rows_out<NCX>(ao, h, p, un);
            if (d.dpre) BD::template rows_out<NCX>(ap, h, p, un);
          }
        }
      }
#undef FFC_BPRIO
      if constexpr (!RP && GEO::NW > 1) {
        if (d.dk_out || d.dk_pair) {
          using MB = Modes<B, GEO, DT_BF16>;
          if constexpr (DT != DT_BF16) {
            B::barrier();
            MB::BD::setup_tables(d.tab_bf, d.t_bf);
          }
          if constexpr (GEO::UPW == 1) MB::dk_tail(d, h, un.wq);
          else MB::dk_tail_multi(d, h, u, un.wq);
          return;
        }
      }
      if constexpr (RP && GEO::NW > 1 && GEO::UPW == 1 && DT == DT_BF16) {
        if (d.dk_out) { dk_tail_rp(d, h, un.wq, ps); return; }
      }
      w_acc_finish(slab, u, un, W);
    } else if (a.R > 1) {
      if constexpr (GEO::N == 1024) {
        if constexpr (SETUP) BD::setup_tables_ipass(a.tab, a.t, a.R);
        const int q0 = p0, q1 = p1;
        const int iters = (q1 - q0 + GEO::UPW - 1) / GEO::UPW;
        BD::template load_inner<false>(R, un);
#pragma unroll 1
        for (int k0 = 0; k0 < a.R; k0++) {
          Pass ps; ps.k0 = k0; ps.R = a.R;
          InnerPass ip;
          BD::load_inner_pass_lean(ip, k0);
          A16 wre = B::a16_zero(), wim = B::a16_zero();
#pragma unroll 1
          for (int it = 0; it < iters; it++) {
            const int q = q0 + it * GEO::UPW + u;
            if (q < q1) {
              ZReg zv;
              A16 re, im;
              typename BD::KfRegs kf;
              BD::load_kf(a, h * a.R + k0, 0, kf);
              typename BD::KfRegs zk;
              if (d.zin) {
                z_load(BD::z_slot_small(const_cast<void*>(d.zin), h, a.npair, q, a.R, k0), 0, zk, BD::Z_STREAM);
              } else {
                BD::template rows_in_rp<BD::NCH>(av, h, q, un, ps);
                B::lds_fence();
                BD::template tile_fwd<true, true, false, true>(0, R, un, re, im, &ip);
                z_pack(re, im, zv);
                B::lds_fence();
              }
              if (ad.aux_in && k0 == 0) BD::template rows_aux_rp<BD::NCH>(ad, h, q, un);
              BD::template rows_in_rp<BD::NCH>(ad, h, q, un, ps);
              B::lds_fence();
              BD::template tile_fwd<true, true, false, true>(0, R, un, re, im, &ip);
              if (d.zin) w_add_k(wre, wim, zk, re, im);
              else w_add(wre, wim, zv, re, im);
              kf_conj_mul(kf, re, im);
              B::lds_fence();
              BD::template tile_inv<true, false, true, false, true>(a.s_inv, 0, R, un, re, im, 0, Pass(), &ip);
              B::lds_fence();
              BD::template rows_out_rp<BD::NCH>(ao, h, q, un, ps);
              if (d.dpre) BD::template rows_out_rp<BD::NCH>(ap, h, q, un, ps);
              B::lds_fence();
            }
          }
          reduce_store_w(d.ws + (((int64_t)chunk * a.H + h) * a.R + k0) * 2048, u, wre, wim);
        }
      }
    } else {
      const int q0 = p0 / GEO::G, q1 = (p1 + GEO::G - 1) / GEO::G;
      const int iters = (q1 - q0 + GEO::UPW - 1) / GEO::UPW;
      BD::load_inner(R, un);
      A16 wre = B::a16_zero(), wim = B::a16_zero();
#pragma unroll 1
      for (int it = 0; it < iters; it++) {
        const int q = q0 + it * GEO::UPW + u;
        if (q < q1) {
          ZReg zv;
          A16 re, im;
          typename BD::KfRegs kf;
          BD::load_kf(a, h, 0, kf);
          typename BD::KfRegs zk;
          if (d.zin) {
            z_load(BD::z_slot_small(const_cast<void*>(d.zin), h, a.npair, q, 1, 0), 0, zk, BD::Z_STREAM);
          } else {
            BD::rows_in(av, h, q, un);
            B::lds_fence();
            BD::tile_fwd(0, R, un, re, im);
            z_pack(re, im, zv);
            B::lds_fence();
          }
          BD::rows_in(ad, h, q, un);
          B::lds_fence();
          BD::tile_fwd(0, R, un, re, im);
          if (d.zin) w_add_k(wre, wim, zk, re, im);
          else w_add(wre, wim, zv, re, im);
          kf_conj_mul(kf, re, im);
          B::lds_fence();
          BD::tile_inv(a.s_inv, 0, R, un, re, im);
          B::lds_fence();
          BD::rows_out(ao, h, q, un);
          if (d.dpre) BD::rows_out(ap, h, q, un);
          B::lds_fence();
        }
      }
      reduce_store_w(slab, u, wre, wim);
    }
  }

  static FFC_FN void w_add(A16& wre, A16& wim, const ZReg& zv, const A16& re, const A16& im) {
#pragma unroll
    for (int r = 0; r < 16; r++) {
      u32 pr = zv.r[r >> 1], pi = zv.i[r >> 1];
      f32 ur = (r & 1) ? B::template unpack_hi<DT>(pr) : B::template unpack_lo<DT>(pr);
      f32 ui = (r & 1) ? B::template unpack_hi<DT>(pi) : B::template unpack_lo<DT>(pi);
      wre[r] = wre[r] + (re[r] * ur + im[r] * ui);
      wim[r] = wim[r] + (im[r] * ur - re[r] * ui);
    }
  }
  static FFC_FN void w_add_k(A16& wre, A16& wim, const typename BD::KfRegs& z, const A16& re, const A16& im) {
#pragma unroll
    for (int rq = 0; rq < 4; rq++) {
      u32 wv[4] = {z.v[rq].x, z.v[rq].y, z.v[rq].z, z.v[rq].w};
#pragma unroll
      for (int q = 0; q < 4; q++) {
        const int r = 4 * rq + q;
        f32 ur = B::template unpack_lo<DT>(wv[q]), ui = B::template unpack_hi<DT>(wv[q]);
        wre[r] = wre[r] + (re[r] * ur + im[r] * ui);
        wim[r] = wim[r] + (im[r] * ur - re[r] * ui);
      }
    }
  }
  static FFC_FN void reduce_store_w(float* slab, int u, const A16& wre, const A16& wim) {
    static_assert(!GEO::OUTER, "single-tile geometries");
    if constexpr (GEO::UPW == 1) {
      store_w(slab, wre, wim);
    } else {
      static_assert(GEO::UPW == 8 && GEO::UPW * GEO::EBYTES >= 8 * 4096, "one wave per unit, 4 KB of exchange buffer each");
      const i32 lane = B::opaque(B::lane());
      f32 sr[2], si[2];
#pragma unroll
      for (int plane = 0; plane < 2; plane++) {
        B::barrier();
#pragma unroll
        for (int r = 0; r < 16; r++) B::lds_w32(((u * 16 + r) * 64 + lane) * 4, B::as_u32(plane ? wim[r] : wre[r]));
        B::barrier();
#pragma unroll
        for (int k = 0; k < 2; k++) {
          f32 acc = B::fconst(0.f);
#pragma unroll
          for (int v = 0; v < 8; v++) acc = acc + B::as_f32(B::lds_r32(((v * 16 + (2 * u + k)) * 64 + lane) * 4));
          if (plane) si[k] = acc; else sr[k] = acc;
        }
      }
      B::barrier();
      const i32 c = lane & 31, hi = lane >> 5;
      const i32 idx = ((hi + 2 * (u >> 1)) * 32 + c) * 2 + (u & 1);
      U4 n;
      n.x = B::as_u32(sr[0]); n.y = B::as_u32(si[0]); n.z = B::as_u32(sr[1]); n.w = B::as_u32(si[1]);
      B::g_w128(slab, idx, n, B::ptrue());
    }
  }
  static FFC_FN void store_w(float* slab, const A16& re, const A16& im) {
// ... 227 lines not shown
```

flash-fft-conv_amd/csrc/ffc_route.h:

```cpp
#pragma once
#include <stdint.h>
#include <type_traits>
#include "ffc_body.h"
#include "ffc_modes.h"
#include "ffc_big.h"

namespace ffc {

template <class F>
inline int pick(F&& f) { return f(); }
template <class F, class... Bs>
inline int pick(F&& f, bool b, Bs... bs) {
  return b ? pick([&](auto... r) { return f(std::true_type{}, r...); }, bs...)
           : pick([&](auto... r) { return f(std::false_type{}, r...); }, bs...);
}
template <class F>
inline int level_dispatch(int n0, bool f16, bool fwd, F&& f) {
  return pick([&](auto n32, auto h, auto fw) -> int {
    return f(std::integral_constant<int, decltype(n32)::value ? 32 : 16>{}, std::integral_constant<int, decltype(h)::value ? DT_F16 : DT_BF16>{}, fw);
  }, n0 == 32, f16, fwd);
}

template <class F>
inline bool with_geo(int N, F&& f) {
  switch (N) {
    case 256: f(Geo<1, 16, 16>{}); return true;
    case 512: f(Geo<1, 16, 32>{}); return true;
    case 1024: case 2048: f(Geo<1, 32, 32>{}); return true;
    case 4096: f(Geo<16, 16, 16>{}); return true;
    case 8192: f(Geo<32, 16, 16>{}); return true;
    case 16384: f(Geo<16, 32, 32>{}); return true;
    case 32768: case 65536: case 131072: f(Geo<32, 32, 32>{}); return true;
  }
  return false;
}

static constexpr int IPASS_BYTES = 2 * 6144 + 2 * 8192;
static constexpr const char* NO_MULTI_PASS = "multi-pass plan on a geometry without multi-pass kernels";

inline int cap_two_per_cu(int grid, int persist) {
  const int cap = (persist > 0 && persist < (1 << 29)) ? 2 * persist : (1 << 30);
  return grid > cap ? cap : grid;
}

struct FwdRoute {
  bool multi_pass;
  bool half;
  bool sz;
  bool sp;
  int grid, lds_max, lds;
  const char* err;
  bool gs;
};
template <class GEO>
inline bool direct_store_ok(bool half, bool multi_pass, int fast, bool plain, int flags) {
  return GEO::N == 32768 && half && !multi_pass && fast && plain && !(flags & 256);
}
template <class GEO>
inline FwdRoute fwd_route(const ConvArgs& a) {
  FwdRoute r{};
  r.grid = ((a.H + 7) & ~7) * a.nchunk;
  r.lds_max = r.lds = GEO::LDS_BYTES;
  if (a.R > 1) {
    r.multi_pass = true;
    if (GEO::N == 32768) {
      r.half = 16 * GEO::Mi >= a.L;
      r.sz = a.zsave != nullptr;
    } else if (GEO::N == 1024) {
      r.sz = a.zsave || a.yraw;
      r.grid = cap_two_per_cu(r.grid, a.persist);
      r.lds_max = GEO::LDS_BYTES + 2 * IPASS_BYTES;
      r.lds = GEO::LDS_BYTES + a.R * IPASS_BYTES;
    } else {
      r.err = NO_MULTI_PASS;
    }
    return r;
  }
  if (GEO::OUTER && GEO::NW == 1 && r.grid > a.persist) r.grid = a.persist;
  if (!GEO::OUTER && a.persist > 0 && a.persist < (1 << 29) && r.grid > 2 * a.persist) r.grid = 2 * a.persist;
  r.half = GEO::OUTER && (GEO::N1 / 2) * GEO::Mi >= a.L;
  if (a.sparse) {
    if (GEO::HAS_SP) r.sp = true;
    else r.err = "frequency-sparse kernel: fft 16384 / 32768 only";
    return r;
  }
  r.sz = a.zsave || (!GEO::OUTER && a.yraw);
  r.gs = direct_store_ok<GEO>(r.half, false, a.fast, !a.postgate && !a.addend && !a.yraw, a.flags);
  return r;
}
template <class GEO>
constexpr bool fwd_kernel_exists(bool add, bool multi_pass, bool half, bool sz, bool sp) {
  if (multi_pass) return !sp && (GEO::N == 32768 || (GEO::N == 1024 && !half));
  if (sp) return GEO::HAS_SP && !add && !sz;
  return GEO::OUTER || !half;
}

struct BwdRoute {
  bool multi_pass;
  bool half;
  bool fastk;
  bool small;
  int grid, lds_max, lds;
  const char* err;
  bool gs;
};
template <class GEO>
inline BwdRoute bwd_route(const DkfArgs& d, bool dkf) {
  const ConvArgs& c = d.c;
  BwdRoute r{};
  r.grid = ((c.H + 7) & ~7) * c.nchunk;
  r.lds_max = r.lds = GEO::LDS_BYTES;
  if (c.R > 1 && GEO::OUTER) {
    if (GEO::N != 32768) { r.err = NO_MULTI_PASS; return r; }
    r.multi_pass = true;
    r.half = 16 * GEO::Mi >= c.L;
    r.fastk = !dkf && c.fast && (FFC_RP_FASTK != 0);
    return r;
  }
  if (GEO::OUTER) {
    if (GEO::NW == 1 && c.persist > 0 && r.grid > c.persist) r.grid = c.persist;
    r.half = (GEO::N1 / 2) * GEO::Mi >= c.L;
    r.gs = !dkf && direct_store_ok<GEO>(r.half, false, c.fast, !c.pregate && !d.dpre, c.flags);
    return r;
  }
  r.small = true;
  if (c.R > 1 && GEO::N != 1024) { r.err = NO_MULTI_PASS; return r; }
  r.lds_max = GEO::LDS_BYTES + 2 * IPASS_BYTES;
  r.lds = GEO::LDS_BYTES + (c.R > 1 ? c.R * IPASS_BYTES : 0);
  if (!dkf) r.grid = cap_two_per_cu(r.grid, c.persist);
  return r;
}

inline bool fwd_takes_kfft(const HostPlan& hp, int nchunk, int sparse, int flags) {
  return nchunk == 1 && hp.N >= 8192 && hp.N <= 32768 && hp.R == 1 && !sparse && !(flags & 64);
}
enum { DK_SEPARATE = 0, DK_TAIL = 1, DK_TAIL_MULTI = 2 };
inline bool bwd_takes_dk(const HostPlan& hp, int nchunk, int flags) {
  return nchunk == 1 && hp.N >= ((flags & 128) ? 8192 : 16384) && hp.N <= 32768 && hp.R == 1 && !(flags & 32);
}
inline bool bwd_takes_dk_multi(const HostPlan& hp, int nchunk, int flags) {
  return nchunk == 1 && hp.R > 1 && hp.N1 > 1 && hp.dtype == DT_BF16 && !(flags & 32);
}
inline int bwd_dk_form(const HostPlan& hp, int nchunk, int flags, bool complex_rows) {
  if (bwd_takes_dk(hp, nchunk, flags)) return DK_TAIL;
  return (!complex_rows && bwd_takes_dk_multi(hp, nchunk, flags)) ? DK_TAIL_MULTI : DK_SEPARATE;
}
inline void set_dk_tail(DkfArgs* d, float* dk, void* pair, int Lk, float scale, int fast, const uint8_t* tab_bf, const PlanTabs& t_bf) {
  d->dk_out = dk; d->dk_pair = pair; d->Lk = Lk; d->dk_scale = scale; d->dk_fast = fast;
  d->tab_bf = tab_bf; d->t_bf = t_bf;
}

inline int decode_dtype(int dtype, int dir, BigArgs* a) {
  a->lf32 = (dtype & 16) ? 1 : 0;
  a->half = (dtype & 32) ? 1 : 0;
  const int e = (dtype >> 8) & 0xff;
  if (e > 30 || (e && !(a->lf32 && dir))) return -1;
  a->lpre = (float)(1u << e);
  return dtype & 15;
}
inline const char* set_long_side(BigArgs* a, int dir, int64_t Hin, int64_t Llong, int64_t pitch_in, int64_t pitch_out, int64_t pitch_gate) {
  const int64_t hl = Hin * Llong;
  if ((dir ? pitch_out : pitch_in) != 0) return "outer pass: the short side (pair-plane tensor) is contiguous, its pitch must be 0";
  int64_t pl = dir ? pitch_in : pitch_out, pg = a->gate ? pitch_gate : 0;
  if (!pl) pl = hl;
  if (!pg) pg = hl;
  if (pl < hl || pg < hl) return "outer pass: a batch pitch is smaller than Hin * Llong";
  if (a->lf32 && pl != hl) return "outer pass: the fp32 long side is contiguous";
  a->pin = dir ? pl : 0; a->pout = dir ? 0 : pl; a->pgate = pg;
  a->strided = (pl != hl || pg != hl) ? 1 : 0;
  a->fast = (Llong % 8 == 0) && !(((uintptr_t)a->in | (uintptr_t)a->out | (uintptr_t)a->gate) & 15) && !((pl | pg) & 7);
  return nullptr;
}
inline bool half_rows_ok(const BigArgs& a, int64_t Bv, int64_t npair) { return !a.half || (Bv == 1 && npair == 1); }
inline const char* set_level(BigArgs* a, int dir, int64_t Bv, int64_t npair, int64_t Hin, int64_t Mi, int64_t Llong, float scale,
                             int64_t pitch_in, int64_t pitch_out, int64_t pitch_gate) {
  a->Bp_valid = (int)Bv; a->npair = (int)npair; a->Hin = (int)Hin; a->Mi = (int)Mi; a->Llong = (int)Llong; a->scale = scale;
  return set_long_side(a, dir, Hin, Llong, pitch_in, pitch_out, pitch_gate);
}
inline bool level_pipe(const BigArgs& a, bool fwd, bool opt_in) {
  return opt_in && a.R == 1 && a.fast && !a.lf32 && !a.half && !a.strided && !(fwd && a.gate);
}
inline bool level_wide(const BigArgs& a) { return a.Llong > 32 * a.Mi; }
inline const char* level_wide_check(const BigArgs& a) {
  if (a.strided) return "outer pass (R passes), wide form: contiguous long side only";
  if (a.lf32 || a.half) return "outer pass (R passes), long side beyond the first 32 rows: 16-bit rows and all short-side rows only";
  if (GeoBig<32>::WGW % a.R) return "outer pass (R passes), wide form: R must divide the workgroup's waves";
  return nullptr;
}
inline int level_wide_cols(int R) { return 128 * (GeoBig<32>::WGW / R); }
inline int64_t level_blocks(const BigArgs& a, int cols) { return (int64_t)a.npair * a.Hin * (a.Mi / cols); }

}
```

flash-fft-conv_amd/csrc/ffc_sim.cpp:

```cpp
#include <math.h>
#include <pthread.h>
#include <stdint.h>
#include <stdlib.h>
#include <string.h>

#include <atomic>
#include <thread>
#include <vector>

#define FFC_FN inline __attribute__((always_inline))
#include "ffc_body.h"
#include "ffc_modes.h"
#include "ffc_big.h"
#include "ffc_route.h"

namespace ffc {

template <class T>
struct Vec {
  T v[64];
  Vec() {}
  Vec(T s) { for (int i = 0; i < 64; i++) v[i] = s; }
};
#define VOP(op)                                                                           \
  template <class T> inline Vec<T> operator op(const Vec<T>& a, const Vec<T>& b) {        \
    Vec<T> r; for (int i = 0; i < 64; i++) r.v[i] = a.v[i] op b.v[i]; return r; }         \
  template <class T> inline Vec<T> operator op(const Vec<T>& a, T b) {                    \
    Vec<T> r; for (int i = 0; i < 64; i++) r.v[i] = a.v[i] op b; return r; }              \
  template <class T> inline Vec<T> operator op(T a, const Vec<T>& b) {                    \
    Vec<T> r; for (int i = 0; i < 64; i++) r.v[i] = a op b.v[i]; return r; }
VOP(+) VOP(-) VOP(*) VOP(/) VOP(%) VOP(&) VOP(|) VOP(^)
#undef VOP
template <class T> inline Vec<T> operator<<(const Vec<T>& a, int s) { Vec<T> r; for (int i = 0; i < 64; i++) r.v[i] = a.v[i] << s; return r; }
template <class T> inline Vec<T> operator>>(const Vec<T>& a, int s) { Vec<T> r; for (int i = 0; i < 64; i++) r.v[i] = a.v[i] >> s; return r; }
inline Vec<uint32_t> operator&(const Vec<uint32_t>& a, unsigned b) { Vec<uint32_t> r; for (int i = 0; i < 64; i++) r.v[i] = a.v[i] & b; return r; }
inline Vec<int> operator*(const Vec<int>& a, long b) { return a * (int)b; }
inline Vec<bool> operator<(const Vec<int>& a, int b) { Vec<bool> r; for (int i = 0; i < 64; i++) r.v[i] = a.v[i] < b; return r; }
inline Vec<bool> operator<(const Vec<int>& a, const Vec<int>& b) { Vec<bool> r; for (int i = 0; i < 64; i++) r.v[i] = a.v[i] < b.v[i]; return r; }
inline Vec<bool> operator>=(const Vec<int>& a, int b) { Vec<bool> r; for (int i = 0; i < 64; i++) r.v[i] = a.v[i] >= b; return r; }
inline Vec<bool> operator&&(const Vec<bool>& a, const Vec<bool>& b) { Vec<bool> r; for (int i = 0; i < 64; i++) r.v[i] = a.v[i] && b.v[i]; return r; }
inline Vec<bool> operator&&(const Vec<bool>& a, bool b) { Vec<bool> r; for (int i = 0; i < 64; i++) r.v[i] = a.v[i] && b; return r; }

struct WgCtx {
  std::vector<uint8_t> lds;
  pthread_barrier_t bar;
  int nwaves;
};
static thread_local WgCtx* g_wg = nullptr;
static thread_local int g_wave = 0;
static thread_local Vec<float> g_agpr[128];
static std::atomic<long> g_dma_count{0};
static std::atomic<long> g_gs_count{0};
static int g_sim_flags = 0;

static inline float dt_to_f32(int DT, uint16_t h) { return DT == DT_BF16 ? bf16_to_f32(h) : f16_to_f32(h); }
static inline uint16_t f32_to_dt(int DT, float f) { return DT == DT_BF16 ? f32_to_bf16(f) : f32_to_f16(f); }

struct SimB {
  static constexpr bool LEAN_OUTER = false;
  static constexpr bool FAST_ONLY = false;
  static constexpr bool HAS_ADD = false;
  using f32 = Vec<float>;
  using i32 = Vec<int>;
  using u32 = Vec<uint32_t>;
  using pred = Vec<bool>;
  struct U2 { u32 x, y; };
  struct U4 { u32 x, y, z, w; };
  struct A16 { f32 v[16]; f32& operator[](int i) { return v[i]; } const f32& operator[](int i) const { return v[i]; } };
  struct W4 { u32 v[4]; u32& operator[](int i) { return v[i]; } const u32& operator[](int i) const { return v[i]; } };
  struct A4 { f32 v[4]; f32& operator[](int i) { return v[i]; } const f32& operator[](int i) const { return v[i]; } };
  static A4 a4_zero() { A4 z; for (int i = 0; i < 4; i++) z.v[i] = f32(0.f); return z; }
  template <bool CONJ> static void cmul16(A16& re, A16& im, const A16& tr, const A16& ti) {
    for (int r = 0; r < 16; r++) {
      f32 a = re[r], b = im[r];
      if (!CONJ) { re[r] = a * tr[r] - b * ti[r]; im[r] = a * ti[r] + b * tr[r]; }
      else { re[r] = a * tr[r] + b * ti[r]; im[r] = b * tr[r] - a * ti[r]; }
    }
  }
  struct F2 { f32 x, y; };
  static F2 f2(const f32& a, const f32& b) { F2 v; v.x = a; v.y = b; return v; }
  static f32 f2_lo(const F2& v) { return v.x; }
  static f32 f2_hi(const F2& v) { return v.y; }
  static void cmulp(const F2& xr, const F2& xi, const f32& wr, const f32& wi, F2& yr, F2& yi) {
    F2 r, i;
    r.x = xr.x * wr - xi.x * wi; r.y = xr.y * wr - xi.y * wi;
    i.x = xr.x * wi + xi.x * wr; i.y = xr.y * wi + xi.y * wr;
    yr = r; yi = i;
  }
  template <bool CONJ>
  static void cmul2v(A16& re, A16& im, int r0, const F2& tr, const F2& ti) { cmul2<CONJ>(re, im, r0, tr.x, tr.y, ti.x, ti.y); }
  static void cmac2_conj(F2& wr, F2& wi, const A16& a, const A16& b, int r0, const F2& zr, const F2& zi) {
    wr.x = wr.x + (a[r0] * zr.x + b[r0] * zi.x);
    wr.y = wr.y + (a[r0 + 1] * zr.y + b[r0 + 1] * zi.y);
    wi.x = wi.x + (b[r0] * zr.x - a[r0] * zi.x);
    wi.y = wi.y + (b[r0 + 1] * zr.y - a[r0 + 1] * zi.y);
  }
  static void agpr_reserve() {}
  template <int I> static f32 agpr_get() { return g_agpr[I]; }
  template <int I> static void agpr_set(const f32& x) { g_agpr[I] = x; }
  static void pin(W4&) {}
  static void pin4(U4&) {}
  static void sched_fence() {}
  template <bool CONJ>
  static void cmul2(A16& re, A16& im, int r0, const f32& tr0, const f32& tr1, const f32& ti0, const f32& ti1) {
    const f32* tr[2] = {&tr0, &tr1}; const f32* ti[2] = {&ti0, &ti1};
    for (int q = 0; q < 2; q++) {
      f32 a = re[r0 + q], b = im[r0 + q];
      if (!CONJ) { re[r0 + q] = a * *tr[q] - b * *ti[q]; im[r0 + q] = a * *ti[q] + b * *tr[q]; }
      else { re[r0 + q] = a * *tr[q] + b * *ti[q]; im[r0 + q] = b * *tr[q] - a * *ti[q]; }
    }
  }
  static A16 a16_scale(const A16& a, float s) { A16 r; for (int i = 0; i < 16; i++) r[i] = a[i] * f32(s); return r; }
  static A16 a16_zero() { A16 z; for (int i = 0; i < 16; i++) z.v[i] = f32(0.f); return z; }
  static W4 w4(const u32& a, const u32& b, const u32& c, const u32& e) { W4 v; v.v[0] = a; v.v[1] = b; v.v[2] = c; v.v[3] = e; return v; }
  static bool HAS_TR;

  static i32 lane() { i32 r; for (int i = 0; i < 64; i++) r.v[i] = i; return r; }
  static int wave() { return g_wave; }
  static void barrier() { if (g_wg->nwaves > 1) pthread_barrier_wait(&g_wg->bar); }
  static f32 fconst(float c) { return f32(c); }
  static pred ptrue() { return pred(true); }
  static pred pfalse() { return pred(false); }
  static f32 as_f32(const u32& a) { f32 r; for (int i = 0; i < 64; i++) memcpy(&r.v[i], &a.v[i], 4); return r; }
  static u32 as_u32(const f32& a) { u32 r; for (int i = 0; i < 64; i++) memcpy(&r.v[i], &a.v[i], 4); return r; }

  static uint8_t* L() { return g_wg->lds.data(); }
  static void chk(int off, int n) { if (off < 0 || off + n > (int)g_wg->lds.size() || (off & (n - 1))) abort(); }
  static U2 lds_r64(const i32& off) {
    U2 r;
    for (int i = 0; i < 64; i++) { chk(off.v[i], 8); memcpy(&r.x.v[i], L() + off.v[i], 4); memcpy(&r.y.v[i], L() + off.v[i] + 4, 4); }
    return r;
  }
  static void lds_w64(const i32& off, const U2& v) {
    for (int i = 0; i < 64; i++) { chk(off.v[i], 8); memcpy(L() + off.v[i], &v.x.v[i], 4); memcpy(L() + off.v[i] + 4, &v.y.v[i], 4); }
  }
  static void lds_w32(const i32& off, const u32& v) {
    for (int i = 0; i < 64; i++) { chk(off.v[i], 4); memcpy(L() + off.v[i], &v.v[i], 4); }
  }
  static void lds_w128(const i32& off, const U4& v, const pred& p) {
    for (int i = 0; i < 64; i++)
      if (p.v[i]) {
        chk(off.v[i], 16);
        memcpy(L() + off.v[i], &v.x.v[i], 4); memcpy(L() + off.v[i] + 4, &v.y.v[i], 4);
        memcpy(L() + off.v[i] + 8, &v.z.v[i], 4); memcpy(L() + off.v[i] + 12, &v.w.v[i], 4);
      }
  }
  static U4 lds_r128(const i32& off) {
    U4 r;
    for (int i = 0; i < 64; i++) {
      chk(off.v[i], 16);
      memcpy(&r.x.v[i], L() + off.v[i], 4); memcpy(&r.y.v[i], L() + off.v[i] + 4, 4);
      memcpy(&r.z.v[i], L() + off.v[i] + 8, 4); memcpy(&r.w.v[i], L() + off.v[i] + 12, 4);
    }
    return r;
  }
  static void lds_w16(const i32& off, const u32& v) {
    for (int i = 0; i < 64; i++) { chk(off.v[i], 2); uint16_t h = (uint16_t)v.v[i]; memcpy(L() + off.v[i], &h, 2); }
  }
  static u32 lds_r32(const i32& off) {
    u32 r;
    for (int i = 0; i < 64; i++) { chk(off.v[i], 4); memcpy(&r.v[i], L() + off.v[i], 4); }
    return r;
  }
  static u32 lds_r16(const i32& off) {
    u32 r;
    for (int i = 0; i < 64; i++) { chk(off.v[i], 2); uint16_t h; memcpy(&h, L() + off.v[i], 2); r.v[i] = h; }
    return r;
  }
  static U2 lds_r64_tr(const i32& off) {
    U2 r;
    for (int g = 0; g < 4; g++) {
      uint16_t M[16][4];
      for (int i = 0; i < 16; i++) { chk(off.v[g * 16 + i], 8); memcpy(M[i], L() + off.v[g * 16 + i], 8); }
      for (int i = 0; i < 16; i++) {
        uint16_t e[4];
        for (int j = 0; j < 4; j++) e[j] = M[4 * j + (i >> 2)][i & 3];
        r.x.v[g * 16 + i] = e[0] | ((uint32_t)e[1] << 16);
        r.y.v[g * 16 + i] = e[2] | ((uint32_t)e[3] << 16);
      }
    }
    return r;
  }
  static void lds_fence() {}
  template <bool NT>
  static void g2lds32(const void* base, const i32& dw, int lds_off) {
    g_dma_count++;
    for (int i = 0; i < 64; i++) { chk(lds_off + 4 * i, 4); memcpy(L() + lds_off + 4 * i, (const uint32_t*)base + dw.v[i], 4); }
  }
  template <bool NT>
  static void g2lds128(const void* base, const i32& o16, int lds_off) {
    g_dma_count++;
    for (int i = 0; i < 64; i++) { chk(lds_off + 16 * i, 16); memcpy(L() + lds_off + 16 * i, (const uint8_t*)base + 16 * (int64_t)o16.v[i], 16); }
  }
  static void vm_wait0() {}
  static void lds_wait0() {}
  static void lds_w32p(const i32& off, const u32& v, const pred& p) {
    for (int i = 0; i < 64; i++) if (p.v[i]) { chk(off.v[i], 4); memcpy(L() + off.v[i], &v.v[i], 4); }
  }
  static pred pnot(const pred& p) { pred r; for (int i = 0; i < 64; i++) r.v[i] = !p.v[i]; return r; }
  static i32 mul24(const i32& a, const i32& b) { return a * b; }
  static unsigned long long clock() { return 0; }
  template <int P> static void setprio() {}
  static U2 u2_from64(unsigned long long v) { U2 r; r.x = u32((uint32_t)v); r.y = u32((uint32_t)(v >> 32)); return r; }
  static void settle(f32&, f32&) {}
  static f32 i2f(const i32& a) { f32 r; for (int i = 0; i < 64; i++) r.v[i] = (float)a.v[i]; return r; }
// ... 1 lines not shown
  static f32 sin_rev(const f32& a) { f32 r; for (int i = 0; i < 64; i++) r.v[i] = (float)sin(6.283185307179586 * (double)a.v[i]); return r; }
  static i32 opaque(const i32& x) { return x; }
  static u32 uconst(uint32_t c) { return u32(c); }
  static i32 imin(const i32& a, int b) { i32 r; for (int i = 0; i < 64; i++) r.v[i] = a.v[i] < b ? a.v[i] : b; return r; }
  static u32 merge_lo(const u32& a, const u32& b) { u32 r; for (int i = 0; i < 64; i++) r.v[i] = (a.v[i] & 0xffffu) | (b.v[i] << 16); return r; }
  static u32 merge_hi(const u32& a, const u32& b) { u32 r; for (int i = 0; i < 64; i++) r.v[i] = (a.v[i] >> 16) | (b.v[i] & 0xffff0000u); return r; }
  static u32 sel(const pred& p, const u32& a, const u32& b) { u32 r; for (int i = 0; i < 64; i++) r.v[i] = p.v[i] ? a.v[i] : b.v[i]; return r; }
  static u32 g_r16(const void* base, const i32& e, const pred& p) {
    u32 r;
    for (int i = 0; i < 64; i++) { uint16_t h = 0; if (p.v[i]) memcpy(&h, (const uint8_t*)base + (int64_t)e.v[i] * 2, 2); r.v[i] = h; }
    return r;
  }
  static void g_w16(void* base, const i32& e, const u32& v, const pred& p) {
    for (int i = 0; i < 64; i++) if (p.v[i]) { uint16_t h = (uint16_t)v.v[i]; memcpy((uint8_t*)base + (int64_t)e.v[i] * 2, &h, 2); }
  }
  static u32 g_r32(const void* base, const i32& e, const pred& p) {
    u32 r;
    for (int i = 0; i < 64; i++) { uint32_t h = 0; if (p.v[i]) memcpy(&h, (const uint8_t*)base + (int64_t)e.v[i] * 4, 4); r.v[i] = h; }
    return r;
  }
  static void g_w32(void* base, const i32& e, const u32& v, const pred& p) {
    for (int i = 0; i < 64; i++) if (p.v[i]) memcpy((uint8_t*)base + (int64_t)e.v[i] * 4, &v.v[i], 4);
  }
  static U2 g_r64(const void* base, const i32& o8, const pred& p) {
    U2 r;
    for (int i = 0; i < 64; i++) {
      if (p.v[i]) { const uint8_t* q = (const uint8_t*)base + (int64_t)o8.v[i] * 8; memcpy(&r.x.v[i], q, 4); memcpy(&r.y.v[i], q + 4, 4); }
      else { r.x.v[i] = 0; r.y.v[i] = 0; }
    }
    return r;
  }
  static void g_w64(void* base, const i32& o8, const U2& v, const pred& p) {
    for (int i = 0; i < 64; i++)
      if (p.v[i]) { uint8_t* q = (uint8_t*)base + (int64_t)o8.v[i] * 8; memcpy(q, &v.x.v[i], 4); memcpy(q + 4, &v.y.v[i], 4); }
  }
  static void g_w64_nt(void* base, const i32& o8, const U2& v, const pred& p) { g_w64(base, o8, v, p); }
  static U4 g_r128(const void* base, const i32& o16) {
    U4 r;
    for (int i = 0; i < 64; i++) {
      const uint8_t* q = (const uint8_t*)base + (int64_t)o16.v[i] * 16;
      memcpy(&r.x.v[i], q, 4); memcpy(&r.y.v[i], q + 4, 4); memcpy(&r.z.v[i], q + 8, 4); memcpy(&r.w.v[i], q + 12, 4);
    }
    return r;
  }
  static U4 g_r128_nt(const void* base, const i32& o16) { return g_r128(base, o16); }
  static U4 g_r128p(const void* base, const i32& o16, const pred& p) {
    U4 r;
    for (int i = 0; i < 64; i++) {
      if (p.v[i]) {
        const uint8_t* q = (const uint8_t*)base + (int64_t)o16.v[i] * 16;
        memcpy(&r.x.v[i], q, 4); memcpy(&r.y.v[i], q + 4, 4); memcpy(&r.z.v[i], q + 8, 4); memcpy(&r.w.v[i], q + 12, 4);
      } else { r.x.v[i] = r.y.v[i] = r.z.v[i] = r.w.v[i] = 0; }
    }
    return r;
  }
  static void g_w128(void* base, const i32& o16, const U4& v, const pred& p) {
    for (int i = 0; i < 64; i++)
      if (p.v[i]) {
        uint8_t* q = (uint8_t*)base + (int64_t)o16.v[i] * 16;
        memcpy(q, &v.x.v[i], 4); memcpy(q + 4, &v.y.v[i], 4); memcpy(q + 8, &v.z.v[i], 4); memcpy(q + 12, &v.w.v[i], 4);
      }
  }
  static void g_w128_nt(void* base, const i32& o16, const U4& v, const pred& p) { g_w128(base, o16, v, p); }
  template <int DT>
  static void mfma(A16& acc, const W4& a, const W4& b) {
    float A[32][16], Bm[16][32];
    for (int l = 0; l < 64; l++)
      for (int e = 0; e < 8; e++) {
        uint16_t ha = (uint16_t)(a[e >> 1].v[l] >> (16 * (e & 1)));
        uint16_t hb = (uint16_t)(b[e >> 1].v[l] >> (16 * (e & 1)));
        A[l & 31][8 * (l >> 5) + e] = dt_to_f32(DT, ha);
        Bm[8 * (l >> 5) + e][l & 31] = dt_to_f32(DT, hb);
      }
    for (int l = 0; l < 64; l++)
      for (int r = 0; r < 16; r++) {
        int i = acc_row(r, l >> 5), j = l & 31;
        float s = 0;
        for (int k = 0; k < 16; k++) s += A[i][k] * Bm[k][j];
        acc[r].v[l] += s;
      }
  }
  template <int DT>
  static void mfma16(A4& acc, const W4& a, const W4& b) {
    float A[16][32], Bm[32][16];
    for (int l = 0; l < 64; l++)
      for (int e = 0; e < 8; e++) {
        uint16_t ha = (uint16_t)(a[e >> 1].v[l] >> (16 * (e & 1)));
        uint16_t hb = (uint16_t)(b[e >> 1].v[l] >> (16 * (e & 1)));
        A[l & 15][8 * (l >> 4) + e] = dt_to_f32(DT, ha);
        Bm[8 * (l >> 4) + e][l & 15] = dt_to_f32(DT, hb);
      }
    for (int l = 0; l < 64; l++)
      for (int r = 0; r < 4; r++) {
        int i = 4 * (l >> 4) + r, j = l & 15;
        float s = 0;
        for (int k = 0; k < 32; k++) s += A[i][k] * Bm[k][j];
        acc[r].v[l] += s;
      }
  }
  template <int DT> static u32 pack(const f32& lo, const f32& hi) {
    u32 r;
    for (int i = 0; i < 64; i++) r.v[i] = f32_to_dt(DT, lo.v[i]) | ((uint32_t)f32_to_dt(DT, hi.v[i]) << 16);
    return r;
  }
  static u32 pk_mul_f16(const u32& a, const u32& b) {
    u32 r;
    for (int i = 0; i < 64; i++) {
      float lo = f16_to_f32((uint16_t)a.v[i]) * f16_to_f32((uint16_t)b.v[i]);
      float hi = f16_to_f32((uint16_t)(a.v[i] >> 16)) * f16_to_f32((uint16_t)(b.v[i] >> 16));
      r.v[i] = f32_to_f16(lo) | ((uint32_t)f32_to_f16(hi) << 16);
    }
    return r;
  }
  template <int DT> static f32 unpack_lo(const u32& a) { f32 r; for (int i = 0; i < 64; i++) r.v[i] = dt_to_f32(DT, (uint16_t)a.v[i]); return r; }
  template <int DT> static f32 unpack_hi(const u32& a) { f32 r; for (int i = 0; i < 64; i++) r.v[i] = dt_to_f32(DT, (uint16_t)(a.v[i] >> 16)); return r; }
};
bool SimB::HAS_TR = true;
struct SimBO : SimB { static constexpr bool LEAN_OUTER = true; };
struct SimBA : SimB { static constexpr bool HAS_ADD = true; };
struct SimBOF : SimBO { static constexpr bool FAST_ONLY = true; };
static bool g_force_slow = false;

template <class F>
static void run_wg(int nwaves, int lds_bytes, F fn) {
  WgCtx ctx;
  ctx.lds.assign(lds_bytes, 0xCD);
  ctx.nwaves = nwaves;
  pthread_barrier_init(&ctx.bar, nullptr, nwaves);
  std::vector<std::thread> th;
  for (int w = 0; w < nwaves; w++)
    th.emplace_back([&, w]() { g_wg = &ctx; g_wave = w; fn(); });
  for (auto& t : th) t.join();
  pthread_barrier_destroy(&ctx.bar);
}

static constexpr int NO_KERNEL = -8;
template <class GEO> constexpr int sim_lds() { return GEO::LDS_BYTES + (GEO::OUTER ? 0 : 4 * IPASS_BYTES); }
template <class F>
static int sim_jobs(int H, int nchunk, int lds, F job) {
  for (int h = 0; h < H; h++)
    for (int c = 0; c < nchunk; c++) run_wg(8, lds, [&]() { job(h, c); });
  return 0;
}

template <class GEO, int DT, class SB = SimB>
static int sim_conv_t(const ConvArgs& a) {
  using BD = Body<SB, GEO, DT>;
  static_assert(BD::IPASS_BYTES == IPASS_BYTES && GEO::WGW == 8, "ffc_route.h");
  const FwdRoute r = fwd_route<GEO>(a);
  if (r.err) return NO_KERNEL;
  if (r.gs) {
    if constexpr (!SB::HAS_ADD && GEO::N == 32768) {
      g_gs_count++;
      return pick([&](auto sz) -> int {
        return sim_jobs(a.H, a.nchunk, r.lds, [&](int h, int c) {
          BD::setup_tables(a.tab, a.t);
          if (a.kfuse_k || a.kfuse_x) Modes<SB, GEO, DT>::kfft_head(a, h);
          BD::template conv_job<true, false, decltype(sz)::value, false, true>(a, h, c);
        });
      }, r.sz);
    } else {
      return NO_KERNEL;
    }
  }
  return pick([&](auto mp, auto half, auto sz, auto sp) -> int {
    constexpr bool MP = decltype(mp)::value, HALF = decltype(half)::value, SZ = decltype(sz)::value, SP = decltype(sp)::value;
    if constexpr (!fwd_kernel_exists<GEO>(SB::HAS_ADD, MP, HALF, SZ, SP)) {
      return NO_KERNEL;
    } else if constexpr (MP) {
      return sim_jobs(a.H, a.nchunk, r.lds, [&](int h, int c) {
        BD::setup_tables(a.tab, a.t);
        if constexpr (!GEO::OUTER) BD::setup_tables_ipass(a.tab, a.t, a.R);
        BD::template conv_job<HALF, true, SZ>(a, h, c);
      });
    } else {
      return sim_jobs(a.H, a.nchunk, r.lds, [&](int h, int c) {
        if constexpr (GEO::OUTER && GEO::NW > 1 && !SP && !SB::HAS_ADD) {
          if (a.kfuse_k || a.kfuse_x) {
            BD::setup_tables(a.tab, a.t);
            Modes<SB, GEO, DT>::kfft_head(a, h);
            BD::template conv_job<HALF, false, SZ>(a, h, c);
            return;
          }
        }
        BD::template conv<HALF, SZ, SP>(a, h, c);
      });
    }
  }, r.multi_pass, r.half, r.sz, r.sp);
}

template <template <class, int> class FN, class... A>
static int dispatch(int N, int dtype, A&&... args) {
  int rc = 0;
  const bool found = with_geo(N, [&](auto geo) {
    using GEO = decltype(geo);
    rc = dtype == DT_BF16 ? FN<GEO, DT_BF16>::run(args...) : FN<GEO, DT_F16>::run(args...);
  });
  return found ? rc : -1;
}
template <class GEO, int DT> struct ConvRun { static int run(const ConvArgs& a) { return sim_conv_t<GEO, DT>(a); } };
template <class GEO, int DT> struct ConvResRun { static int run(const ConvArgs& a) { return sim_conv_t<GEO, DT, SimBA>(a); } };
template <class GEO, int DT> struct KfRun {
  static int run(const KfArgs& a) {
    const int nunits = GEO::OUTER ? a.H : (a.H + GEO::G - 1) / GEO::G;
    for (int wg = 0; wg < (nunits + GEO::UPW - 1) / GEO::UPW; wg++)
      run_wg(GEO::WGW, sim_lds<GEO>(), [&]() { Modes<SimB, GEO, DT>::kfft(a, wg); });
    return 0;
  }
};
template <class GEO, int DT, bool DKF>
static int sim_bwd_t(const DkfArgs& d) {
  using MO = Modes<SimBO, GEO, DT>;
  const BwdRoute r = bwd_route<GEO>(d, DKF);
  if (r.err) return NO_KERNEL;
  const int H = d.c.H, nchunk = d.c.nchunk, lds = sim_lds<GEO>();
  if (r.gs) {
    if constexpr (GEO::N == 32768) {
      g_gs_count++;
      if (d.zin) return sim_jobs(H, nchunk, lds, [&](int h, int c) { MO::template bwd<true, false, true, 1, true>(d, h, c, h * nchunk + c); });
      return sim_jobs(H, nchunk, lds, [&](int h, int c) { MO::template bwd<true, false, true, 0, true>(d, h, c, h * nchunk + c); });
    } else {
      return NO_KERNEL;
    }
  }
  return pick([&](auto mp, auto half, auto fastk, auto zm) -> int {
    constexpr bool MP = decltype(mp)::value, HALF = decltype(half)::value, FASTK = decltype(fastk)::value, ZM = decltype(zm)::value;
    if constexpr (!GEO::OUTER) {
      if constexpr (MP || HALF || FASTK || ZM) return NO_KERNEL;
      else if constexpr (DKF) return sim_jobs(H, nchunk, lds, [&](int h, int c) { MO::dkf(d, h, c, h * nchunk + c); });
      else return sim_jobs(H, nchunk, lds, [&](int h, int c) { MO::bwd(d, h, c, h * nchunk + c); });
    } else if constexpr (MP) {
      if constexpr (GEO::N != 32768 || (DKF && (FASTK || ZM))) {
        return NO_KERNEL;
      } else {
        using MK = Modes<typename std::conditional<FASTK, SimBOF, SimBO>::type, GEO, DT>;
        return sim_jobs(H, nchunk, lds, [&](int h, int c) {
          MK::BD::setup_tables(d.c.tab, d.c.t);
          for (int k0 = 0; k0 < d.c.R; k0++) {
            if constexpr (DKF) MK::template dkf<HALF, true>(d, h, c, h * nchunk + c, k0, SimBO::wave());
            else MK::template bwd<HALF, true>(d, h, c, h * nchunk + c, k0, SimBO::wave());
          }
        });
      }
    } else if constexpr (FASTK || (DKF && ZM)) {
      return NO_KERNEL;
    } else if constexpr (DKF) {
      return sim_jobs(H, nchunk, lds, [&](int h, int c) { MO::template dkf<HALF>(d, h, c, h * nchunk + c); });
    } else if constexpr (ZM) {
      return sim_jobs(H, nchunk, lds, [&](int h, int c) { MO::template bwd<HALF, false, true, 1>(d, h, c, h * nchunk + c); });
    } else {
      return sim_jobs(H, nchunk, lds, [&](int h, int c) { MO::template bwd<HALF>(d, h, c, h * nchunk + c); });
    }
  }, r.multi_pass, r.half, r.fastk, !DKF && GEO::OUTER && !r.multi_pass && d.zin != nullptr);
}
template <class GEO, int DT> struct DkfRun { static int run(const DkfArgs& d) { return sim_bwd_t<GEO, DT, true>(d); } };
template <class GEO, int DT> struct BwdRun { static int run(const DkfArgs& d) { return sim_bwd_t<GEO, DT, false>(d); } };
template <class GEO, int DT> struct DkRun {
  static int run(const DkArgs& a) {
    const int nunits = GEO::OUTER ? a.H : (a.H + GEO::G - 1) / GEO::G;
    for (int wg = 0; wg < (nunits + GEO::UPW - 1) / GEO::UPW; wg++)
      run_wg(GEO::WGW, sim_lds<GEO>(), [&]() { Modes<SimB, GEO, DT>::dkifft(a, wg); });
    return 0;
  }
};
template <class GEO, int DT> struct UpwGet { static int run(int* out) { *out = GEO::UPW; return 0; } };

template <int DT>
static void sim_outer_inv_half(const HostPlan& p, const uint16_t* e_in, uint16_t* e_out) {
  using GEO = Geo<32, 32, 32>;
  using BD = Body<SimB, GEO, DT>;
  run_wg(8, GEO::LDS_BYTES, [&]() {
    BD::setup_tables(p.blob.data(), p.tabs);
    typename BD::Unit un;
    un.eb = 0; un.wq = g_wave;
    if (g_wave == 0)
      for (int pl = 0; pl < 2; pl++)
        for (int row = 0; row < 32; row++)
          for (int m = 0; m < 1024; m++)
            memcpy(SimB::L() + pl * GEO::PLANE + e_off<GEO, int>(row, m), &e_in[(pl * 32 + row) * 1024 + m], 2);
    SimB::barrier();
    BD::template outer_inv_half<false>(un);
    SimB::barrier();
    if (g_wave == 0)
      for (int pl = 0; pl < 2; pl++)
        for (int row = 0; row < 16; row++)
          for (int m = 0; m < 1024; m++)
            memcpy(&e_out[(pl * 16 + row) * 1024 + m], SimB::L() + pl * GEO::PLANE + e_off<GEO, int>(row, m), 2);
  });
}
}

using namespace ffc;

extern "C" {

void ffcsim_set_tr(int on) { SimB::HAS_TR = on != 0; }
void ffcsim_force_slow_io(int on) { g_force_slow = on != 0; }

int ffcsim_selftest_primitives(const uint32_t* in, uint32_t* out) {
  run_wg(1, 1024, [&]() {
    using Bk = SimB;
    Bk::W4 a, b;
    for (int i = 0; i < 4; i++) for (int l = 0; l < 64; l++) { a[i].v[l] = in[l * 8 + i]; b[i].v[l] = in[l * 8 + 4 + i]; }
    Bk::A16 acc = Bk::a16_zero(), acc2 = Bk::a16_zero();
    Bk::mfma<DT_BF16>(acc, a, b);
    Bk::mfma<DT_F16>(acc2, a, b);
    Bk::i32 lane = Bk::lane();
    Bk::U2 w; w.x = a[0]; w.y = a[1];
    Bk::lds_w64(lane * 8, w);
    Bk::U2 t = Bk::lds_r64_tr(((lane * 5 + 3) & 63) * 8);
    Bk::u32 p0 = Bk::pack<DT_BF16>(acc[0], acc[1]), p1 = Bk::pack<DT_F16>(acc[0], acc[1]);
    Bk::f32 u0 = Bk::unpack_lo<DT_F16>(a[2]), u1 = Bk::unpack_hi<DT_F16>(a[2]);
    Bk::f32 u2 = Bk::unpack_lo<DT_BF16>(a[2]), u3 = Bk::unpack_hi<DT_BF16>(a[2]);
    for (int l = 0; l < 64; l++) {
      for (int i = 0; i < 16; i++) { memcpy(&out[l * 40 + i], &acc[i].v[l], 4); memcpy(&out[l * 40 + 16 + i], &acc2[i].v[l], 4); }
      out[l * 40 + 32] = t.x.v[l]; out[l * 40 + 33] = t.y.v[l];
      out[l * 40 + 34] = p0.v[l]; out[l * 40 + 35] = p1.v[l];
      memcpy(&out[l * 40 + 36], &u0.v[l], 4); memcpy(&out[l * 40 + 37], &u1.v[l], 4);
      memcpy(&out[l * 40 + 38], &u2.v[l], 4); memcpy(&out[l * 40 + 39], &u3.v[l], 4);
    }
  });
  return 0;
}

int ffcsim_mfma16(int dtype, const uint32_t* a, const uint32_t* b, float* d) {
  SimB::W4 wa, wb;
  SimB::A4 acc;
  for (int l = 0; l < 64; l++)
    for (int i = 0; i < 4; i++) { wa[i].v[l] = a[l * 4 + i]; wb[i].v[l] = b[l * 4 + i]; acc[i].v[l] = d[l * 4 + i]; }
  if (dtype == DT_BF16) SimB::mfma16<DT_BF16>(acc, wa, wb);
  else SimB::mfma16<DT_F16>(acc, wa, wb);
  for (int l = 0; l < 64; l++)
    for (int i = 0; i < 4; i++) d[l * 4 + i] = acc[i].v[l];
  return 0;
}

int ffcsim_outer_inv_half(int dtype, const uint16_t* e_in, uint16_t* e_out) {
  HostPlan p;
  if (!build_plan(32768, dtype, &p)) return -1;
  if (dtype == DT_BF16) sim_outer_inv_half<DT_BF16>(p, e_in, e_out);
  else sim_outer_inv_half<DT_F16>(p, e_in, e_out);
  return 0;
}

int ffcsim_plan_info(int N, int dtype, int* nt, double* s_fwd, double* s_k, int32_t* kf_freq ) {
  HostPlan p;
  if (!build_plan(N, dtype, &p)) return -1;
  *nt = p.NT * p.R; *s_fwd = p.s_fwd; *s_k = p.s_k;
  if (kf_freq) memcpy(kf_freq, p.kf_freq.data(), p.kf_freq.size() * 4);
  return 0;
}

static int g_sparse_rows = 0;
void ffcsim_set_sparse(int rows) { g_sparse_rows = rows; }
static void* g_z = nullptr; static void* g_yraw = nullptr; static int g_flags = 0;
void ffcsim_set_z(void* z, void* yraw, int flags) { g_z = z; g_yraw = yraw; g_flags = flags; }
long ffcsim_dma_count() { return g_dma_count.exchange(0); }
long ffcsim_gs_count() { return g_gs_count.exchange(0); }
void ffcsim_set_flags(int flags) { g_sim_flags = flags; }
static float* g_dk_out = nullptr; static int g_dk_lk = 0;
void ffcsim_set_fused_dk(float* dk, int Lk) { g_dk_out = dk; g_dk_lk = Lk; }
static const float* g_kfuse_k = nullptr; static int g_kfuse_lk = 0;
void ffcsim_set_fused_k(const float* k, int Lk) { g_kfuse_k = k; g_kfuse_lk = Lk; }
static const void* g_kfuse_x = nullptr; static float g_kfuse_xscale = 1.f;
void ffcsim_set_fused_kx(const void* xpair, float scale) { g_kfuse_x = xpair; g_kfuse_xscale = scale; }
static void* g_dk_pair = nullptr; static float g_dk_pair_scale = 1.f;
void ffcsim_set_fused_dkpair(void* outpair, float scale) { g_dk_pair = outpair; g_dk_pair_scale = scale; }
static int g_big_pipe = 0;
void ffcsim_set_big_pipe(int on) { g_big_pipe = on; }
int ffcsim_conv_fwd(int N, int dtype, const void* u, const void* kf, const void* pregate, const void* postgate,
                    void* y, int B, int H, int L, int conj_kf) {
  HostPlan p;
  if (!build_plan(N, dtype, &p)) return -1;
  if (L > N || L <= 0) return -2;
  ConvArgs a{};
  a.u = u; a.pregate = pregate; a.postgate = postgate; a.y = y; a.kf = kf;
  a.tab = p.blob.data(); a.t = p.tabs;
  a.B = B; a.H = H; a.L = L; a.npair = (B + 1) / 2;
  a.sbu = a.sbg = a.sbp = a.sby = (int64_t)H * L;
  a.nchunk = 1; a.ppc = a.npair; a.conj_kf = conj_kf; a.s_inv = (float)p.s_inv; a.s_fwd = (float)p.s_fwd;
  a.fast = (L % 8 == 0) && !g_force_slow;
  a.R = p.R;
  a.flags = g_sim_flags;
  a.sparse = g_sparse_rows;
  if (p.N1 > 1 && p.R == 1) { a.zsave = g_z; a.yraw = g_z ? g_yraw : nullptr; }
  if (p.N1 <= 1) { a.zsave = g_z; a.yraw = g_yraw; }
  const bool kfuse = fwd_takes_kfft(p, a.nchunk, a.sparse, 0);
  if (g_kfuse_x && kfuse) {
    a.kfuse_x = g_kfuse_x; a.kfuse_scale = g_kfuse_xscale; a.kfuse_Lk = N; a.kfuse_fast = 1;
  }
  if (g_kfuse_k && kfuse) {
    a.kfuse_k = g_kfuse_k; a.kfuse_Lk = g_kfuse_lk; a.kfuse_scale = (float)(p.s_k / p.s_fwd) / (dtype == DT_F16 ? 256.f : 1.f); a.kfuse_fast = (g_kfuse_lk % 4 == 0) && !g_force_slow;
  }
  return dispatch<ConvRun>(N, dtype, a);
}

int ffcsim_conv_fwd_res(int N, int dtype, const void* u, const void* kf, const void* pregate, const void* postgate, const void* addend,
                        void* y, void* zsave, void* y_raw, int B, int H, int L, int conj_kf, int64_t sb_u, int64_t sb_pre, int64_t sb_post,
                        int64_t sb_add, int64_t sb_y) {
  HostPlan p;
  if (!build_plan(N, dtype, &p)) return -1;
  if (L > N || L <= 0 || B <= 0 || H <= 0) return -2;
  if (y_raw && !zsave && p.N1 > 1) return -3;
  const int64_t hl = (int64_t)H * L;
  if (!sb_u) sb_u = hl; if (!sb_pre) sb_pre = hl; if (!sb_post) sb_post = hl; if (!sb_add) sb_add = hl; if (!sb_y) sb_y = hl;
  if (sb_u < hl || sb_pre < hl || sb_post < hl || sb_add < hl || sb_y < hl) return -2;
  if (addend) {
    const uintptr_t a0 = (uintptr_t)addend, a1 = a0 + (uintptr_t)(((B - 1) * sb_add + hl) * 2);
    const uintptr_t y0 = (uintptr_t)y, y1 = y0 + (uintptr_t)(((B - 1) * sb_y + hl) * 2);
    if (a0 < y1 && y0 < a1) return -4;
  }
  ConvArgs a{};
  a.u = u; a.pregate = pregate; a.postgate = postgate; a.y = y; a.kf = kf; a.addend = addend;
  a.tab = p.blob.data(); a.t = p.tabs;
  a.B = B; a.H = H; a.L = L; a.npair = (B + 1) / 2;
  a.sbu = sb_u; a.sbg = sb_pre; a.sbp = sb_post; a.sby = sb_y; a.sba = sb_add;
  a.nchunk = 1; a.ppc = a.npair; a.conj_kf = conj_kf; a.s_inv = (float)p.s_inv; a.s_fwd = (float)p.s_fwd;
  a.fast = (L % 8 == 0) && !((sb_u | sb_pre | sb_post | sb_y | sb_add) & 7) && !g_force_slow;
  a.R = p.R;
  a.flags = g_sim_flags;
  a.zsave = zsave; a.yraw = y_raw;
  if (!addend) return dispatch<ConvRun>(N, dtype, a);
  return dispatch<ConvResRun>(N, dtype, a);
}



static int sim_level_args(BigArgs* a, int* dtype, int fwd, const void* in, void* out, const void* gate, int Bp_valid, int npair, int Hin, int Mi,
                          int Llong, float scale, int64_t pitch_in, int64_t pitch_out, int64_t pitch_gate) {
  *dtype = decode_dtype(*dtype, fwd, a);
  if (*dtype < 0) return -1;
  if (!half_rows_ok(*a, Bp_valid, npair)) return -4;
  if (Llong <= 0) return -5;
  if (pitch_in || pitch_out || (gate && pitch_gate)) { a->in = in; a->out = out; a->gate = gate; }
  const bool bad = set_level(a, fwd, Bp_valid, npair, Hin, Mi, Llong, scale, pitch_in, pitch_out, pitch_gate) != nullptr;
  a->in = in; a->out = out; a->gate = gate;
  if (bad) return -7;
  if (g_force_slow) a->fast = 0;
  return 0;
}
int ffcsim_big_outer_r_strided(int N0, int R, int c, int dtype, int fwd, const void* in, void* out, const void* gate, int Bp_valid, int npair,
                               int Hin, int Mi, int Llong, float scale, int64_t pitch_in, int64_t pitch_out, int64_t pitch_gate) {
  HostPlan p;
  if (R > 1 && N0 != 32) return -3;
  BigArgs a{};
  a.R = R; a.c = c;
  const int rc = sim_level_args(&a, &dtype, fwd, in, out, gate, Bp_valid, npair, Hin, Mi, Llong, scale, pitch_in, pitch_out, pitch_gate);
  if (!build_plan(R > 1 ? 32768 * R : (N0 == 16 ? 16384 : 32768), dtype, &p)) return -1;
  if (rc) return rc;
  a.fmat = p.blob.data() + (R > 1 ? p.tabs.matk[c][fwd ? 0 : 1] : p.tabs.mat[0]);
  if (Mi % (N0 == 16 ? GeoBig<16>::Mi : GeoBig<32>::Mi)) return -2;
  const bool pipe = level_pipe(a, fwd != 0, g_big_pipe != 0);
  return level_dispatch(N0, dtype == DT_F16, fwd != 0, [&](auto n0, auto dt, auto fw) -> int {
    constexpr int NN = decltype(n0)::value, DD = decltype(dt)::value;
    constexpr bool FF = decltype(fw)::value;
    const int nblk = (int)level_blocks(a, GeoBig<NN>::Mi), npw = pipe ? (nblk < 3 ? nblk : 3) : nblk;
    for (int wg = 0; wg < npw; wg++)
      run_wg(GeoBig<NN>::WGW + (pipe ? 1 : 0), pipe ? BigBody<SimB, NN, DD>::PIPE_LDS : GeoBig<NN>::LDS_BYTES, [&]() {
        if (pipe) BigBody<SimB, NN, DD>::template run_pipe<FF>(a, wg, npw);
        else if (a.strided) BigBody<SimB, NN, DD, true>::template run<FF>(a, wg);
        else BigBody<SimB, NN, DD>::template run<FF>(a, wg);
      });
    return 0;
  });
}
int ffcsim_big_outer_r(int N0, int R, int c, int dtype, int fwd, const void* in, void* out, const void* gate, int Bp_valid, int npair,
                       int Hin, int Mi, int Llong, float scale) {
  return ffcsim_big_outer_r_strided(N0, R, c, dtype, fwd, in, out, gate, Bp_valid, npair, Hin, Mi, Llong, scale, 0, 0, 0);
}
int ffcsim_big_outer(int N0, int dtype, int fwd, const void* in, void* out, const void* gate, int Bp_valid, int npair,
                     int Hin, int Mi, int Llong, float scale) {
  return ffcsim_big_outer_r(N0, 1, 0, dtype, fwd, in, out, gate, Bp_valid, npair, Hin, Mi, Llong, scale);
}
int ffcsim_big_outer_strided(int N0, int dtype, int fwd, const void* in, void* out, const void* gate, int Bp_valid, int npair,
                             int Hin, int Mi, int Llong, float scale, int64_t pitch_in, int64_t pitch_out, int64_t pitch_gate) {
  return ffcsim_big_outer_r_strided(N0, 1, 0, dtype, fwd, in, out, gate, Bp_valid, npair, Hin, Mi, Llong, scale, pitch_in, pitch_out, pitch_gate);
}

int ffcsim_big_outer_all_strided(int R, int dtype, int fwd, const void* in, void* out, const void* gate, int Bp_valid, int npair,
                                 int Hin, int Mi, int Llong, float scale, int64_t pitch_in, int64_t pitch_out, int64_t pitch_gate) {
  HostPlan p;
  BigArgs a{};
  a.R = R; a.c = 0;
  const int rc = sim_level_args(&a, &dtype, fwd, in, out, gate, Bp_valid, npair, Hin, Mi, Llong, scale, pitch_in, pitch_out, pitch_gate);
  if (R < 2 || R > 4 || !build_plan(32768 * R, dtype, &p)) return -1;
  if (rc) return rc;
  for (int c = 0; c < R; c++) a.fmats[c] = p.blob.data() + p.tabs.matk[c][fwd ? 0 : 1];
  a.fmat = a.fmats[0];
  if (Mi % GeoBig<32>::Mi) return -2;
  if (Llong > R * 32 * Mi) return -5;
  if (level_wide(a)) {
    BigArgs w = a;
    w.strided = 0;
    if (level_wide_check(w)) return -6;
    if (pitch_in || pitch_out || pitch_gate) return -7;
    a.wide = 1;
  }
  return level_dispatch(32, dtype == DT_F16, fwd != 0, [&](auto n0, auto dt, auto fw) -> int {
    constexpr int DD = decltype(dt)::value;
    constexpr bool FF = decltype(fw)::value;
    if constexpr (decltype(n0)::value != 32) return -3;
    const int nblk = (int)level_blocks(a, a.wide ? level_wide_cols(a.R) : GeoBig<32>::Mi);
    for (int wg = 0; wg < nblk; wg++)
      run_wg(GeoBig<32>::WGW, GeoBig<32>::LDS_BYTES, [&]() {
        if (a.wide) BigBody<SimB, 32, DD>::template run_wide<FF>(a, wg);
        else if (a.strided) BigBody<SimB, 32, DD, true>::template run_all<FF>(a, wg);
        else BigBody<SimB, 32, DD>::template run_all<FF>(a, wg);
      });
    return 0;
  });
}
int ffcsim_big_outer_all(int R, int dtype, int fwd, const void* in, void* out, const void* gate, int Bp_valid, int npair,
                         int Hin, int Mi, int Llong, float scale) {
  return ffcsim_big_outer_all_strided(R, dtype, fwd, in, out, gate, Bp_valid, npair, Hin, Mi, Llong, scale, 0, 0, 0);
}

int ffcsim_upw(int N) { int u = 0; dispatch<UpwGet>(N, 0, &u); return u; }

int ffcsim_launch_route(int N, int dtype, int B, int H, int L, int nchunk, int persist, int flags, int* out) {
  HostPlan p;
  if (!build_plan(N, dtype, &p)) return -1;
  static char buf[16];
  DkfArgs d{};
  ConvArgs& a = d.c;
  a.B = B; a.H = H; a.L = L; a.npair = (B + 1) / 2; a.nchunk = nchunk; a.persist = persist; a.R = p.R;
  a.zsave = (flags & (1 << 16)) ? buf : nullptr; a.yraw = (flags & (1 << 17)) ? buf : nullptr;
  a.sparse = (flags & (1 << 18)) ? 2 : 0; a.fast = (flags & (1 << 19)) ? 1 : 0;
  with_geo(N, [&](auto geo) {
    using GEO = decltype(geo);
    const FwdRoute f = fwd_route<GEO>(a);
    const int fo[8] = {f.multi_pass, f.half, f.sz, f.sp, f.grid, f.lds_max, f.lds, f.err != nullptr};
    memcpy(out, fo, sizeof fo);
    for (int dkf = 0; dkf < 2; dkf++) {
      const BwdRoute b = bwd_route<GEO>(d, dkf != 0);
      const int bo[8] = {b.multi_pass, b.half, b.fastk, b.small, b.grid, b.lds_max, b.lds, b.err != nullptr};
      memcpy(out + 8 + 8 * dkf, bo, sizeof bo);
    }
  });
  out[24] = fwd_takes_kfft(p, nchunk, a.sparse, flags & 0xffff);
  out[25] = bwd_dk_form(p, nchunk, flags & 0xffff, false);
  out[26] = bwd_dk_form(p, nchunk, flags & 0xffff, true);
  return 0;
}

int ffcsim_launch_sink(int N, int dtype, int B, int H, int L, int flags, int* out) {
  HostPlan p;
  if (!build_plan(N, dtype, &p)) return -1;
  static char buf[16];
  DkfArgs d{};
  ConvArgs& a = d.c;
  a.B = B; a.H = H; a.L = L; a.npair = (B + 1) / 2; a.nchunk = 1; a.R = p.R; a.flags = flags & 0xffff;
  a.zsave = (flags & (1 << 16)) ? buf : nullptr; a.yraw = (flags & (1 << 17)) ? buf : nullptr;
  a.sparse = (flags & (1 << 18)) ? 2 : 0; a.fast = (flags & (1 << 19)) ? 1 : 0;
  with_geo(N, [&](auto geo) {
    using GEO = decltype(geo);
    ConvArgs f = a;
    f.postgate = (flags & (1 << 20)) ? buf : nullptr; f.addend = (flags & (1 << 21)) ? buf : nullptr;
    out[0] = fwd_route<GEO>(f).gs;
    a.pregate = (flags & (1 << 20)) ? buf : nullptr; d.dpre = (flags & (1 << 21)) ? buf : nullptr;
    out[1] = bwd_route<GEO>(d, false).gs;
    out[2] = bwd_route<GEO>(d, true).gs;
  });
  return 0;
}

int ffcsim_kernel_fft_c(int N, int dtype, const void* xpair, int H, void* kf, float scale) {
  HostPlan p;
  if (!build_plan(N, dtype, &p)) return -1;
  KfArgs a{};
  a.xpair = xpair; a.kf = kf; a.tab = p.blob.data(); a.t = p.tabs; a.H = H; a.Lk = N; a.scale = scale; a.prescale = 1.f; a.s_fwd = (float)p.s_fwd; a.fast = 1;
  a.R = p.R;
  return dispatch<KfRun>(N, dtype, a);
}

int ffcsim_kernel_fft(int N, int dtype, const float* k, int H, int Lk, void* kf) {
  HostPlan p;
  if (!build_plan(N, dtype, &p)) return -1;
  KfArgs a{};
  a.k = k; a.kf = kf; a.tab = p.blob.data(); a.t = p.tabs; a.H = H; a.Lk = Lk;
  a.s_fwd = (float)p.s_fwd;
  a.prescale = dtype == DT_F16 ? 256.f : 1.f;
  a.scale = (float)(p.s_k / p.s_fwd) / a.prescale; a.fast = (Lk % 4 == 0) && !g_force_slow;
  a.R = p.R;
  return dispatch<KfRun>(N, dtype, a);
}

int ffcsim_conv_bwd_dkf(int N, int dtype, const void* dout, const void* u, const void* pregate, const void* postgate,
                        float* ws, int B, int H, int L, int nchunk) {
  HostPlan p;
  if (!build_plan(N, dtype, &p)) return -1;
  DkfArgs d{};
  ConvArgs& a = d.c;
  a.u = u; a.pregate = pregate; a.postgate = postgate; a.tab = p.blob.data(); a.t = p.tabs;
  a.B = B; a.H = H; a.L = L; a.npair = (B + 1) / 2; a.s_fwd = (float)p.s_fwd;
  a.sbu = a.sbg = a.sbp = a.sby = (int64_t)H * L; d.sbd = d.sbdu = d.sbdpre = d.sbdpost = (int64_t)H * L;
  int upw = ffcsim_upw(N);
  int per_iter = p.N1 > 1 ? upw : upw * p.G;
  int iters_total = (a.npair + per_iter - 1) / per_iter;
  if (nchunk > iters_total) nchunk = iters_total;
  int ipc = (iters_total + nchunk - 1) / nchunk;
  a.ppc = ipc * per_iter; a.nchunk = (a.npair + a.ppc - 1) / a.ppc;
  a.fast = (L % 8 == 0) && !g_force_slow;
  a.R = p.R;
  d.dout = dout; d.ws = ws;
  std::vector<uint8_t> zs((size_t)H * a.nchunk * upw * N * 4 + 16);
  d.zscratch = zs.data();
  int rc = dispatch<DkfRun>(N, dtype, d);
  return rc < 0 ? rc : a.nchunk;
}

int ffcsim_conv_bwd(int N, int dtype, const void* dout, const void* u, const void* kf, const void* pregate, const void* postgate,
                    void* du, void* dpre, void* dpost, float* ws, int B, int H, int L, int nchunk) {
  HostPlan p;
  if (!build_plan(N, dtype, &p)) return -1;
  DkfArgs d{};
  ConvArgs& a = d.c;
  a.u = u; a.kf = kf; a.pregate = pregate; a.postgate = postgate; a.tab = p.blob.data(); a.t = p.tabs;
  a.B = B; a.H = H; a.L = L; a.npair = (B + 1) / 2; a.s_inv = (float)p.s_inv; a.s_fwd = (float)p.s_fwd;
  a.sbu = a.sbg = a.sbp = a.sby = (int64_t)H * L; d.sbd = d.sbdu = d.sbdpre = d.sbdpost = (int64_t)H * L;
  int upw = ffcsim_upw(N);
  int per_iter = p.N1 > 1 ? upw : upw * p.G;
  int iters_total = (a.npair + per_iter - 1) / per_iter;
  if (nchunk > iters_total) nchunk = iters_total;
  int ipc = (iters_total + nchunk - 1) / nchunk;
  a.ppc = ipc * per_iter; a.nchunk = (a.npair + a.ppc - 1) / a.ppc;
  a.fast = (L % 8 == 0) && !g_force_slow;
  a.R = p.R;
  d.dout = dout; d.ws = ws; d.du = du; d.dpre = dpre; d.dpost = (p.N1 > 1 || g_yraw) ? dpost : nullptr;
  a.flags = g_sim_flags;
  if (p.N1 > 1 && p.R == 1 && g_z) { d.zin = g_z; d.yraw = g_yraw; a.flags = g_flags | g_sim_flags; a.stream = 1; }
  if (p.N1 <= 1) { d.zin = g_z; d.yraw = dpost ? g_yraw : nullptr; }
  HostPlan pbf;
  if (g_dk_pair && bwd_dk_form(p, a.nchunk, 128, true) != DK_SEPARATE) {
    if (!build_plan(N, DT_BF16, &pbf)) return -1;
    set_dk_tail(&d, nullptr, g_dk_pair, N, g_dk_pair_scale, 1, pbf.blob.data(), pbf.tabs);
  } else if (g_dk_out && bwd_dk_form(p, a.nchunk, 128, false) != DK_SEPARATE) {
    if (!build_plan(N, DT_BF16, &pbf)) return -1;
    set_dk_tail(&d, g_dk_out, nullptr, g_dk_lk, (float)(1.0 / p.s_fwd), (g_dk_lk % 4 == 0) && !g_force_slow, pbf.blob.data(), pbf.tabs);
  }
  std::vector<uint8_t> zs((size_t)H * a.nchunk * upw * N * 4 + 16);
  d.zscratch = zs.data();
  int rc = dispatch<BwdRun>(N, dtype, d);
  return rc < 0 ? rc : a.nchunk;
}

int ffcsim_kernel_ifft_grad_c(int N, const float* ws, int nslab, int H, void* outpair, float scale) {
  HostPlan p;
  if (!build_plan(N, DT_BF16, &p)) return -1;
  DkArgs a{};
  a.ws = ws; a.outpair = outpair; a.tab = p.blob.data(); a.t = p.tabs; a.H = H; a.Lk = N; a.nslab = nslab; a.scale = scale; a.s_inv = (float)p.s_inv; a.fast = 1;
  a.R = p.R;
  return dispatch<DkRun>(N, DT_BF16, a);
}

int ffcsim_kernel_ifft_grad(int N, int dtype, const float* ws, int nslab, int H, int Lk, float* dk) {
  HostPlan p;
  (void)dtype;
  dtype = DT_BF16;
  if (!build_plan(N, dtype, &p)) return -1;
  DkArgs a{};
  a.ws = ws; a.dk = dk; a.tab = p.blob.data(); a.t = p.tabs; a.H = H; a.Lk = Lk; a.nslab = nslab;
  a.scale = (float)(1.0 / p.s_fwd); a.s_inv = (float)p.s_inv;
  a.fast = (Lk % 4 == 0) && !g_force_slow;
  a.R = p.R;
  return dispatch<DkRun>(N, dtype, a);
}

}
```

Measured before the change: 11.12 million seq/s.

## Add plain-row specialization for direct-store fwd/bwd kernels without gates

Adds a PL template variant of the direct-store conv and backward kernels, used when no pregate, aux or postgate inputs are present. It loads input rows with a simpler unconditional path that masks with selects instead of the general gated loader. It drops the p<p1 activity test when there is one unit per wave, forces the LDS-DMA row path in backward, and passes the wave index to the bf16 table setup. The goal is to cut predicate and gate-handling overhead and register pressure in the hot loop, at the cost of more kernel instantiations and new assumptions about the row bounds.

```diff
diff --git a/flash-fft-conv_amd/csrc/ffc_body.h b/flash-fft-conv_amd/csrc/ffc_body.h
--- a/flash-fft-conv_amd/csrc/ffc_body.h
+++ b/flash-fft-conv_amd/csrc/ffc_body.h
@@ -243,36 +243,36 @@
   }
   static constexpr int TAB_T = GEO::WGW * 64;
   template <int BYTES>
-  static FFC_FN void tab_issue(const uint8_t* src, U4 (&v)[(BYTES / 16 + TAB_T - 1) / TAB_T]) {
-    const i32 tid = B::lane() + B::wave() * 64;
+  static FFC_FN void tab_issue(const uint8_t* src, U4 (&v)[(BYTES / 16 + TAB_T - 1) / TAB_T], int wv = -1) {
+    const i32 tid = B::lane() + (wv >= 0 ? wv : B::wave()) * 64;
 #pragma unroll
     for (int it = 0; it < (BYTES / 16 + TAB_T - 1) / TAB_T; it++) v[it] = B::g_r128(src, B::imin(tid + it * TAB_T, BYTES / 16 - 1));
   }
   template <int BYTES>
-  static FFC_FN void tab_commit(int lds_off, const U4 (&v)[(BYTES / 16 + TAB_T - 1) / TAB_T]) {
-    const i32 tid = B::lane() + B::wave() * 64;
+  static FFC_FN void tab_commit(int lds_off, const U4 (&v)[(BYTES / 16 + TAB_T - 1) / TAB_T], int wv = -1) {
+    const i32 tid = B::lane() + (wv >= 0 ? wv : B::wave()) * 64;
 #pragma unroll
     for (int it = 0; it < (BYTES / 16 + TAB_T - 1) / TAB_T; it++) {
       i32 idx = tid + it * TAB_T;
       B::lds_w128(idx * 16 + lds_off, v[it], idx < BYTES / 16);
     }
   }
-  static FFC_FN void setup_tables(const uint8_t* tab, const PlanTabs& t) {
+  static FFC_FN void setup_tables(const uint8_t* tab, const PlanTabs& t, int wv = -1) {
     U4 f1[(6144 / 16 + TAB_T - 1) / TAB_T], f2[(6144 / 16 + TAB_T - 1) / TAB_T], f3[(6144 / 16 + TAB_T - 1) / TAB_T],
        tw[(8192 / 16 + TAB_T - 1) / TAB_T], tw2[(8192 / 16 + TAB_T - 1) / TAB_T], fs[(3072 / 16 + TAB_T - 1) / TAB_T];
-    if constexpr (GEO::OUTER) tab_issue<6144>(tab + t.mat[0], f1);
-    tab_issue<6144>(tab + t.mat[1], f2);
-    tab_issue<8192>(tab + t.twin, tw);
-    if constexpr (GEO::N3 != GEO::N2) tab_issue<6144>(tab + t.mat[2], f3);
-    if constexpr (GEO::TW2_SEP) tab_issue<8192>(tab + t.twin2, tw2);
-    if constexpr (GEO::HAS_SP) tab_issue<3072>(tab + t.mat_sp, fs);
+    if constexpr (GEO::OUTER) tab_issue<6144>(tab + t.mat[0], f1, wv);
+    tab_issue<6144>(tab + t.mat[1], f2, wv);
+    tab_issue<8192>(tab + t.twin, tw, wv);
+    if constexpr (GEO::N3 != GEO::N2) tab_issue<6144>(tab + t.mat[2], f3, wv);
+    if constexpr (GEO::TW2_SEP) tab_issue<8192>(tab + t.twin2, tw2, wv);
+    if constexpr (GEO::HAS_SP) tab_issue<3072>(tab + t.mat_sp, fs, wv);
     B::sched_fence();
-    if constexpr (GEO::OUTER) tab_commit<6144>(GEO::L_F1, f1);
-    tab_commit<6144>(GEO::L_F2, f2);
-    tab_commit<8192>(GEO::L_TW, tw);
-    if constexpr (GEO::N3 != GEO::N2) tab_commit<6144>(GEO::L_F3, f3);
-    if constexpr (GEO::TW2_SEP) tab_commit<8192>(GEO::L_TW2, tw2);
-    if constexpr (GEO::HAS_SP) tab_commit<3072>(GEO::L_FS, fs);
+    if constexpr (GEO::OUTER) tab_commit<6144>(GEO::L_F1, f1, wv);
+    tab_commit<6144>(GEO::L_F2, f2, wv);
+    tab_commit<8192>(GEO::L_TW, tw, wv);
+    if constexpr (GEO::N3 != GEO::N2) tab_commit<6144>(GEO::L_F3, f3, wv);
+    if constexpr (GEO::TW2_SEP) tab_commit<8192>(GEO::L_TW2, tw2, wv);
+    if constexpr (GEO::HAS_SP) tab_commit<3072>(GEO::L_FS, fs, wv);
     B::barrier();
   }
   static FFC_FN void lds_mat(Mat& m, int off) {
@@ -536,6 +536,67 @@
     RowRegsT<NC> X;
     rows_load<NC>(a, h, pq, un, X);
     rows_store<NC>(a, h, pq, un, X);
+  }
+  template <int NC, bool NT>
+  static FFC_FN void rows_load_pl_t(const ConvArgs& a, int h, int pq, Unit un, RowRegsT<NC>& X) {
+    static_assert(GEO::OUTER, "plain-row kernels: sizes with an outer digit");
+    const i32 lane = B::opaque(B::lane());
+#pragma unroll
+    for (int ii = 0; ii < NC; ii++) {
+      i32 idx = lane + ii * 64;
+      i32 row = idx / CPR, m = (idx % CPR) * 8 + un.wq * 128 * GEO::S1;
+#pragma unroll
+      for (int pl = 0; pl < 2; pl++) {
+        const int b = 2 * pq + pl;
+        const bool ok = b < a.B;
+        const uint16_t* base = (const uint16_t*)a.u + row_off(b, ok, a.sbu, h, a.L);
+        const i32 n16 = B::imin(row * GEO::Mi + m, a.L - 8) >> 3;
+        X.v[ii][pl] = NT ? B::g_r128_nt(base, n16) : B::g_r128(base, n16);
+      }
+    }
+  }
+  template <int NC>
+  static FFC_FN void rows_load_pl(const ConvArgs& a, int h, int pq, Unit un, RowRegsT<NC>& X) {
+    if (a.stream) rows_load_pl_t<NC, true>(a, h, pq, un, X);
+    else rows_load_pl_t<NC, false>(a, h, pq, un, X);
+  }
+  template <int NC>
+  static FFC_FN void rows_store_pl(const ConvArgs& a, int pq, Unit un, const RowRegsT<NC>& X) {
+    const i32 lane = B::opaque(B::lane());
+#pragma unroll
+    for (int ii = 0; ii < NC; ii++) {
+      i32 idx = lane + ii * 64;
+      i32 row = idx / CPR, m = (idx % CPR) * 8 + un.wq * 128 * GEO::S1;
+      pred sw;
+      i32 off = pair_off(row, m, &sw) + un.eb;
+#pragma unroll
+      for (int pl = 0; pl < 2; pl++) {
+        U4 v = X.v[ii][pl];
+        pred ok = ((row * GEO::Mi + m) < a.L) && ((2 * pq + pl) < a.B);
+        v.x = B::sel(ok, v.x, B::uconst(0)); v.y = B::sel(ok, v.y, B::uconst(0));
+        v.z = B::sel(ok, v.z, B::uconst(0)); v.w = B::sel(ok, v.w, B::uconst(0));
+        U4 o;
+        o.x = B::sel(sw, v.z, v.x); o.y = B::sel(sw, v.w, v.y);
+        o.z = B::sel(sw, v.x, v.z); o.w = B::sel(sw, v.y, v.w);
+        B::lds_w128(off + pl * GEO::PLANE, o, B::ptrue());
+      }
+    }
+  }
+  template <int NC, bool PL>
+  static FFC_FN void rows_load_sel(const ConvArgs& a, int h, int pq, Unit un, RowRegsT<NC>& X) {
+    if constexpr (PL) rows_load_pl<NC>(a, h, pq, un, X);
+    else rows_load<NC>(a, h, pq, un, X);
+  }
+  template <int NC, bool PL>
+  static FFC_FN void rows_store_sel(const ConvArgs& a, int h, int pq, Unit un, const RowRegsT<NC>& X) {
+    if constexpr (PL) rows_store_pl<NC>(a, pq, un, X);
+    else rows_store<NC>(a, h, pq, un, X);
+  }
+  template <int NC, bool PL>
+  static FFC_FN void rows_in_sel(const ConvArgs& a, int h, int pq, Unit un) {
+    RowRegsT<NC> X;
+    rows_load_sel<NC, PL>(a, h, pq, un, X);
+    rows_store_sel<NC, PL>(a, h, pq, un, X);
   }
   static constexpr bool HAS_DMA = GEO::OUTER && GEO::N1 == 32 && GEO::S1 == 1;
   static constexpr int DMA_ROW0 = GEO::N1 / 2;
@@ -2044,9 +2105,10 @@
     if constexpr (GEO::NW > 1) B::barrier();
     else B::lds_fence();
   }
-  template <bool HALF, bool PROF = false, bool RP = false, bool SZ = false, bool SP = false, bool GS = false>
+  template <bool HALF, bool PROF = false, bool RP = false, bool SZ = false, bool SP = false, bool GS = false, bool PL = false>
   static FFC_FN void outer_jobs(const ConvArgs& a, int h, int p0, int p1, int u, Unit un, int wg_linear = 0) {
     static_assert(!GS || (HALF && !RP && !SP && HALF_C), "direct-store phase C: single-pass fft 32768, L <= N/2");
+    static_assert(!PL || GS, "plain input rows: a form of the direct-store kernels");
     constexpr int NC = HALF ? NCH / 2 : NCH;
     constexpr bool PREFETCH = HALF && !RP;
     constexpr bool FOLDF = CAN_FOLD && !RP && !SP && !PROF && !B::LEAN_OUTER;
@@ -2054,7 +2116,7 @@
     const int npass = RP ? a.R : 1;
     const int iters = ((p1 - p0 + GEO::UPW - 1) / GEO::UPW) * npass;
     RowRegsT<NC> X;
-    if constexpr (PREFETCH) { if (p0 + u < p1) rows_load<NC>(a, h, p0 + u, un, X); }
+    if constexpr (PREFETCH) { if (p0 + u < p1) rows_load_sel<NC, PL>(a, h, p0 + u, un, X); }
     unsigned long long acc[8] = {0, 0, 0, 0, 0, 0, 0, 0}, t0 = 0, t1 = 0;
 #define FFC_TICK(k) if (PROF) { t1 = B::clock(); acc[k] += t1 - t0; t0 = t1; }
     const bool second = B::wave() >= 4;
@@ -2064,15 +2126,15 @@
       const int p = p0 + (RP ? it / npass : it) * GEO::UPW + u;
       const Pass ps = RP ? make_pass(a, it % npass) : Pass();
       const int hk = RP ? h * ps.R + ps.k0 : h;
-      const bool act = p < p1;
+      const bool act = (PL && GEO::UPW == 1) || p < p1;
       if (PROF) t0 = B::clock();
       FFC_PRIO(1)
       if (act) {
         if constexpr (RP) {
           rows_in_rp<NC>(a, h, p, un, ps);
         } else {
-          if constexpr (!PREFETCH) rows_load<NC>(a, h, p, un, X);
-          rows_store<NC>(a, h, p, un, X);
+          if constexpr (!PREFETCH) rows_load_sel<NC, PL>(a, h, p, un, X);
+          rows_store_sel<NC, PL>(a, h, p, un, X);
         }
         B::lds_fence();
         FFC_TICK(0)
@@ -2133,7 +2195,7 @@
       unit_barrier();
       FFC_TICK(4)
       FFC_PRIO(3)
-      if constexpr (PREFETCH) { if (it + 1 < iters && p + GEO::UPW < p1) rows_load<NC>(a, h, p + GEO::UPW, un, X); }
+      if constexpr (PREFETCH) { if (it + 1 < iters && p + GEO::UPW < p1) rows_load_sel<NC, PL>(a, h, p + GEO::UPW, un, X); }
       if constexpr (GS) {
         if (act) {
           outer_inv_half<true>(un, &a, h, p);
@@ -2167,12 +2229,12 @@
     }
   }
 
-  template <bool HALF = false, bool SZ = false, bool SP = false, bool GS = false>
+  template <bool HALF = false, bool SZ = false, bool SP = false, bool GS = false, bool PL = false>
   static FFC_FN void conv(const ConvArgs& a, int h, int chunk) {
     setup_tables(a.tab, a.t);
-    conv_job<HALF, false, SZ, SP, GS>(a, h, chunk);
-  }
-  template <bool HALF = false, bool RP = false, bool SZ = false, bool SP = false, bool GS = false>
+    conv_job<HALF, false, SZ, SP, GS, PL>(a, h, chunk);
+  }
+  template <bool HALF = false, bool RP = false, bool SZ = false, bool SP = false, bool GS = false, bool PL = false>
   static FFC_FN void conv_job(const ConvArgs& a, int h, int chunk) {
     const int wv = B::wave();
     Unit un;
@@ -2183,7 +2245,7 @@
     int p1 = p0 + a.ppc;
     if (p1 > a.npair) p1 = a.npair;
     if constexpr (GEO::OUTER) {
-      outer_jobs<HALF, false, RP, SZ, SP, GS>(a, h, p0, p1, u, un);
+      outer_jobs<HALF, false, RP, SZ, SP, GS, PL>(a, h, p0, p1, u, un);
     } else {
       const int q0 = p0 / GEO::G, q1 = (p1 + GEO::G - 1) / GEO::G;
       const int iters = (q1 - q0 + GEO::UPW - 1) / GEO::UPW;
diff --git a/flash-fft-conv_amd/csrc/ffc_bwd_launch.h b/flash-fft-conv_amd/csrc/ffc_bwd_launch.h
--- a/flash-fft-conv_amd/csrc/ffc_bwd_launch.h
+++ b/flash-fft-conv_amd/csrc/ffc_bwd_launch.h
@@ -6,7 +6,7 @@
 #include "ffc_dev.h"
 using namespace ffc;
 
-template <class GEO, int DT, bool HALF, int ZM, bool GS = false>
+template <class GEO, int DT, bool HALF, int ZM, bool GS = false, bool PL = false>
 __global__ __launch_bounds__(GEO::WGW * 64, 2) __attribute__((amdgpu_num_vgpr(128))) void bwd_kernel(DkfArgs d) {
   if constexpr (GEO::NW == 1) {
     const int total = ((d.c.H + 7) & ~7) * d.c.nchunk;
@@ -18,7 +18,7 @@
     int h, chunk;
     if (!map_block(d.c.H, d.c.nchunk, &h, &chunk)) return;
     stagger_start(d.c.flags);
-    Modes<DevBO, GEO, DT>::template bwd<HALF, false, true, ZM, GS>(d, h, chunk, blockIdx.x);
+    Modes<DevBO, GEO, DT>::template bwd<HALF, false, true, ZM, GS, PL>(d, h, chunk, blockIdx.x);
   }
 }
 template <class GEO, int DT>
@@ -58,7 +58,9 @@
       return ffc_launch(bwd_kernel_small<GEO, DT>, "bwd_kernel", r.grid, T_, r.lds_max, r.lds, st, d);
     } else if (r.gs) {
       if constexpr (GEO::N == 32768)
-        return ffc_launch(bwd_kernel<GEO, DT, true, ZM, true>, "bwd_kernel (direct store)", r.grid, T_, r.lds_max, r.lds, st, d);
+        return pick([&](auto pl) -> int {
+          return ffc_launch(bwd_kernel<GEO, DT, true, ZM, true, decltype(pl)::value>, "bwd_kernel (direct store)", r.grid, T_, r.lds_max, r.lds, st, d);
+        }, r.pl);
       else
         return ffc_fail("internal: the backward route names a kernel that does not exist");
     } else {
diff --git a/flash-fft-conv_amd/csrc/ffc_conv_launch.h b/flash-fft-conv_amd/csrc/ffc_conv_launch.h
--- a/flash-fft-conv_amd/csrc/ffc_conv_launch.h
+++ b/flash-fft-conv_amd/csrc/ffc_conv_launch.h
@@ -12,9 +12,9 @@
     if (r.err) return ffc_fail(r.err);
     if (r.gs) {
       if constexpr (!FAM::HAS_ADD && GEO::N == 32768)
-        return pick([&](auto sz) -> int {
-          return ffc_launch(FAM::template kernel_gs<GEO, DT, decltype(sz)::value>(), FAM::what(false, decltype(sz)::value, false, true), r.grid, GEO::WGW * 64, r.lds_max, r.lds, st, a);
-        }, r.sz);
+        return pick([&](auto sz, auto pl) -> int {
+          return ffc_launch(FAM::template kernel_gs<GEO, DT, decltype(sz)::value, decltype(pl)::value>(), FAM::what(false, decltype(sz)::value, false, true), r.grid, GEO::WGW * 64, r.lds_max, r.lds, st, a);
+        }, r.sz, r.pl);
       else
         return ffc_fail("internal: the forward route names a kernel that does not exist");
     }
diff --git a/flash-fft-conv_amd/csrc/ffc_k_conv.hip b/flash-fft-conv_amd/csrc/ffc_k_conv.hip
--- a/flash-fft-conv_amd/csrc/ffc_k_conv.hip
+++ b/flash-fft-conv_amd/csrc/ffc_k_conv.hip
@@ -2,7 +2,7 @@
 using namespace ffc;
 
 static constexpr int SMALL_WAVES = 2;
-template <class GEO, int DT, bool HALF, bool SZ = false, bool SP = false, bool GS = false>
+template <class GEO, int DT, bool HALF, bool SZ = false, bool SP = false, bool GS = false, bool PL = false>
 __global__ __launch_bounds__(GEO::WGW * 64, GEO::OUTER ? 2 : SMALL_WAVES) void conv_kernel(ConvArgs a) {
   using BD = Body<DevB, GEO, DT>;
   if constexpr (GEO::OUTER && GEO::NW == 1) {
@@ -26,9 +26,9 @@
     if constexpr (GEO::NW > 1 && !SP) {
       BD::setup_tables(a.tab, a.t);
       if (a.kfuse_k || a.kfuse_x) Modes<DevB, GEO, DT>::kfft_head(a, h);
-      BD::template conv_job<HALF, false, SZ, SP, GS>(a, h, chunk);
+      BD::template conv_job<HALF, false, SZ, SP, GS, PL>(a, h, chunk);
     } else {
-      BD::template conv<HALF, SZ, SP, GS>(a, h, chunk);
+      BD::template conv<HALF, SZ, SP, GS, PL>(a, h, chunk);
     }
   }
 }
@@ -59,8 +59,8 @@
     if constexpr (MP) return conv_rp_kernel<GEO, DT, HALF, SZ>;
     else return conv_kernel<GEO, DT, HALF, SZ, SP>;
   }
-  template <class GEO, int DT, bool SZ>
-  static constexpr auto kernel_gs() { return conv_kernel<GEO, DT, true, SZ, false, true>; }
+  template <class GEO, int DT, bool SZ, bool PL>
+  static constexpr auto kernel_gs() { return conv_kernel<GEO, DT, true, SZ, false, true, PL>; }
   static const char* what(bool mp, bool sz, bool sp, bool outer) {
     if (mp) return sz && outer ? "conv_rp_kernel (spectrum-saving)" : "conv_rp_kernel";
     if (sz) return outer ? "conv_kernel (spectrum-saving)" : "conv_kernel (spectrum-saving, single tile)";
@@ -205,7 +205,7 @@
   return ffc_conv_fwd_strided(p, u, kf, pregate, postgate, y, B, H, L, conj_kf, 0, 0, 0, 0, stream);
 }
 
-template <class GEO, int DT, bool GS = false>
+template <class GEO, int DT, bool GS = false, bool PL = false>
 __global__ __launch_bounds__(GEO::WGW * 64, 2) void conv_prof_kernel(ConvArgs a) {
   int h, chunk;
   if (!map_block(a.H, a.nchunk, &h, &chunk)) return;
@@ -219,7 +219,7 @@
   const int p0 = chunk * a.ppc;
   int p1 = p0 + a.ppc;
   if (p1 > a.npair) p1 = a.npair;
-  if constexpr (GS) BD::template outer_jobs<true, true, false, false, false, true>(a, h, p0, p1, u, un, blockIdx.x);
+  if constexpr (GS) BD::template outer_jobs<true, true, false, false, false, true, PL>(a, h, p0, p1, u, un, blockIdx.x);
   else if (16 * GEO::Mi >= a.L) BD::template outer_jobs<true, true>(a, h, p0, p1, u, un, blockIdx.x);
   else BD::template outer_jobs<false, true>(a, h, p0, p1, u, un, blockIdx.x);
 }
@@ -239,6 +239,7 @@
   const FwdRoute r = fwd_route<GEO>(a);
   const int grid = r.grid;
   if (grid_out) *grid_out = grid;
+  if (r.pl) return ffc_launch(conv_prof_kernel<GEO, DT_BF16, true, true>, "conv_prof_kernel", grid, GEO::WGW * 64, GEO::LDS_BYTES, GEO::LDS_BYTES, (hipStream_t)stream, a);
   if (r.gs) return ffc_launch(conv_prof_kernel<GEO, DT_BF16, true>, "conv_prof_kernel", grid, GEO::WGW * 64, GEO::LDS_BYTES, GEO::LDS_BYTES, (hipStream_t)stream, a);
   return ffc_launch(conv_prof_kernel<GEO, DT_BF16>, "conv_prof_kernel", grid, GEO::WGW * 64, GEO::LDS_BYTES, GEO::LDS_BYTES, (hipStream_t)stream, a);
 }
diff --git a/flash-fft-conv_amd/csrc/ffc_modes.h b/flash-fft-conv_amd/csrc/ffc_modes.h
--- a/flash-fft-conv_amd/csrc/ffc_modes.h
+++ b/flash-fft-conv_amd/csrc/ffc_modes.h
@@ -864,9 +864,10 @@
     }
     BD::cmul_conj(re, im, k);
   }
-  template <bool HALF = false, bool RP = false, bool SETUP = true, int ZM = -1, bool GS = false>
+  template <bool HALF = false, bool RP = false, bool SETUP = true, int ZM = -1, bool GS = false, bool PL = false>
   static FFC_FN void bwd(const DkfArgs& d, int h, int chunk, int wg_linear, int k0 = 0, int wv_in = 0) {
     static_assert(!GS || (HALF && !RP && BD::HALF_C), "direct-store phase C: single-pass fft 32768, L <= N/2");
+    static_assert(!PL || (GS && ZM >= 0), "plain input rows: a form of the direct-store kernels");
     const ConvArgs& a = d.c;
     const Pass ps = RP ? make_pass(a.tab, a.t, a.R, k0) : Pass();
     const int hk = RP ? h * a.R + k0 : h;
@@ -889,8 +890,8 @@
     ap.y = d.dpre; ap.postgate = a.u; ap.sby = d.sbdpre; ap.sbp = a.sbu;
     ConvArgs aq = a;
     aq.y = d.dpost; aq.postgate = d.dout; aq.sby = d.sbdpost; aq.sbp = d.sbd;
-    const bool dpost_tf = d.dpost != nullptr && d.yraw == nullptr;
-    if constexpr (!(RP && GEO::OUTER)) {
+    const bool dpost_tf = !PL && d.dpost != nullptr && d.yraw == nullptr;
+    if constexpr (!(RP && GEO::OUTER) && !PL) {
       if (d.dpost && d.yraw) { ad.aux_in = d.yraw; ad.aux_out = d.dpost; ad.sbai = (int64_t)a.H * a.L; ad.sbao = d.sbdpost; }
     }
     float* slab = RP ? d.ws + (((int64_t)chunk * a.H + h) * a.R + k0) * (GEO::NT * 2048)
@@ -904,14 +905,15 @@
       const bool have_z = ZM < 0 ? d.zin != nullptr : ZM == 1;
       constexpr bool FOLDZ = BD::CAN_FOLD && GEO::N1 == 32 && ZM == 1 && !RP;
       constexpr bool DMA_OK = BD::HAS_DMA && HALF && !RP && ZM != 0;
-      const bool dma = DMA_OK && have_z && a.fast && !ad.pregate && !ad.aux_in && !dpost_tf && !(a.flags & 8);
+      static_assert(!PL || ZM == 0 || DMA_OK, "plain rows on saved spectra: the rows come by LDS-DMA");
+      const bool dma = DMA_OK && (PL || (have_z && a.fast && !ad.pregate && !ad.aux_in && !dpost_tf && !(a.flags & 8)));
       if constexpr (DMA_OK) { if (dma && p0 + u < p1) BD::rows_dma(ad, h, p0 + u, un); }
       const bool second = wv >= 4;
 #define FFC_BPRIO(x) if constexpr (GEO::NW > 1) B::template setprio<x>();
 #pragma unroll 1
       for (int it = 0; it < iters; it++) {
         const int p = p0 + it * GEO::UPW + u;
-        const bool act = p < p1;
+        const bool act = (PL && GEO::UPW == 1) || p < p1;
         FFC_BPRIO(1)
         const void* zp = !have_z ? (const void*)zs
                          : RP ? (const void*)BD::z_slot_rp(const_cast<void*>(d.zin), h, a.npair, act ? p : p0, a.R, k0)
@@ -953,7 +955,7 @@
             }
             if (!done) {
               if constexpr (RP) BD::template rows_in_rp<NCX>(ad, h, p, un, ps);
-              else BD::template rows_in<NCX>(ad, h, p, un);
+              else BD::template rows_in_sel<NCX, PL>(ad, h, p, un);
               B::lds_fence();
               FFC_BPRIO(0)
               BD::template outer_stage<true, HALF, RP, false, FOLDZ>(a.L, un, a.s_fwd, ps);
@@ -962,7 +964,7 @@
         } else {
           if (act) {
             if constexpr (RP) BD::template rows_in_rp<NCX>(av, h, p, un, ps);
-            else BD::template rows_in<NCX>(av, h, p, un);
+            else BD::template rows_in_sel<NCX, PL>(av, h, p, un);
             B::lds_fence();
             FFC_BPRIO(0)
             BD::template outer_stage<true, HALF, RP>(a.L, un, a.s_fwd, ps);
@@ -997,7 +999,7 @@
           }
           if (act) {
             if constexpr (RP) BD::template rows_in_rp<NCX>(ad, h, p, un, ps);
-            else BD::template rows_in<NCX>(ad, h, p, un);
+            else BD::template rows_in_sel<NCX, PL>(ad, h, p, un);
             B::lds_fence();
             FFC_BPRIO(0)
             BD::template outer_stage<true, HALF, RP>(a.L, un, a.s_fwd, ps);
@@ -1042,7 +1044,8 @@
           using MB = Modes<B, GEO, DT_BF16>;
           if constexpr (DT != DT_BF16) {
             B::barrier();
-            MB::BD::setup_tables(d.tab_bf, d.t_bf);
+            if constexpr (PL) MB::BD::setup_tables(d.tab_bf, d.t_bf, wv);
+            else MB::BD::setup_tables(d.tab_bf, d.t_bf);
           }
           if constexpr (GEO::UPW == 1) MB::dk_tail(d, h, un.wq);
           else MB::dk_tail_multi(d, h, u, un.wq);
diff --git a/flash-fft-conv_amd/csrc/ffc_route.h b/flash-fft-conv_amd/csrc/ffc_route.h
--- a/flash-fft-conv_amd/csrc/ffc_route.h
+++ b/flash-fft-conv_amd/csrc/ffc_route.h
@@ -51,11 +51,13 @@
   int grid, lds_max, lds;
   const char* err;
   bool gs;
+  bool pl;
 };
 template <class GEO>
 inline bool direct_store_ok(bool half, bool multi_pass, int fast, bool plain, int flags) {
   return GEO::N == 32768 && half && !multi_pass && fast && plain && !(flags & 256);
 }
+inline bool plain_rows_ok(bool gs, bool plain_in, int flags) { return gs && plain_in && !(flags & 512); }
 template <class GEO>
 inline FwdRoute fwd_route(const ConvArgs& a) {
   FwdRoute r{};
@@ -86,6 +88,7 @@
   }
   r.sz = a.zsave || (!GEO::OUTER && a.yraw);
   r.gs = direct_store_ok<GEO>(r.half, false, a.fast, !a.postgate && !a.addend && !a.yraw, a.flags);
+  r.pl = plain_rows_ok(r.gs, !a.pregate && !a.aux_in, a.flags);
   return r;
 }
 template <class GEO>
@@ -103,6 +106,7 @@
   int grid, lds_max, lds;
   const char* err;
   bool gs;
+  bool pl;
 };
 template <class GEO>
 inline BwdRoute bwd_route(const DkfArgs& d, bool dkf) {
@@ -121,6 +125,7 @@
     if (GEO::NW == 1 && c.persist > 0 && r.grid > c.persist) r.grid = c.persist;
     r.half = (GEO::N1 / 2) * GEO::Mi >= c.L;
     r.gs = !dkf && direct_store_ok<GEO>(r.half, false, c.fast, !c.pregate && !d.dpre, c.flags);
+    r.pl = plain_rows_ok(r.gs, !c.postgate && !d.dpost && !d.yraw && !(c.flags & 8), c.flags);
     return r;
   }
   r.small = true;
diff --git a/flash-fft-conv_amd/csrc/ffc_sim.cpp b/flash-fft-conv_amd/csrc/ffc_sim.cpp
--- a/flash-fft-conv_amd/csrc/ffc_sim.cpp
+++ b/flash-fft-conv_amd/csrc/ffc_sim.cpp
@@ -51,6 +51,7 @@
 static thread_local Vec<float> g_agpr[128];
 static std::atomic<long> g_dma_count{0};
 static std::atomic<long> g_gs_count{0};
+static std::atomic<long> g_pl_count{0};
 static int g_sim_flags = 0;
 
 static inline float dt_to_f32(int DT, uint16_t h) { return DT == DT_BF16 ? bf16_to_f32(h) : f16_to_f32(h); }
@@ -358,13 +359,14 @@
   if (r.gs) {
     if constexpr (!SB::HAS_ADD && GEO::N == 32768) {
       g_gs_count++;
-      return pick([&](auto sz) -> int {
+      if (r.pl) g_pl_count++;
+      return pick([&](auto sz, auto pl) -> int {
         return sim_jobs(a.H, a.nchunk, r.lds, [&](int h, int c) {
           BD::setup_tables(a.tab, a.t);
           if (a.kfuse_k || a.kfuse_x) Modes<SB, GEO, DT>::kfft_head(a, h);
-          BD::template conv_job<true, false, decltype(sz)::value, false, true>(a, h, c);
+          BD::template conv_job<true, false, decltype(sz)::value, false, true, decltype(pl)::value>(a, h, c);
         });
-      }, r.sz);
+      }, r.sz, r.pl);
     } else {
       return NO_KERNEL;
     }
@@ -423,8 +425,12 @@
   if (r.gs) {
     if constexpr (GEO::N == 32768) {
       g_gs_count++;
-      if (d.zin) return sim_jobs(H, nchunk, lds, [&](int h, int c) { MO::template bwd<true, false, true, 1, true>(d, h, c, h * nchunk + c); });
-      return sim_jobs(H, nchunk, lds, [&](int h, int c) { MO::template bwd<true, false, true, 0, true>(d, h, c, h * nchunk + c); });
+      if (r.pl) g_pl_count++;
+      return pick([&](auto zm, auto pl) -> int {
+        return sim_jobs(H, nchunk, lds, [&](int h, int c) {
+          MO::template bwd<true, false, true, decltype(zm)::value ? 1 : 0, true, decltype(pl)::value>(d, h, c, h * nchunk + c);
+        });
+      }, d.zin != nullptr, r.pl);
     } else {
       return NO_KERNEL;
     }
@@ -563,6 +569,7 @@
 void ffcsim_set_z(void* z, void* yraw, int flags) { g_z = z; g_yraw = yraw; g_flags = flags; }
 long ffcsim_dma_count() { return g_dma_count.exchange(0); }
 long ffcsim_gs_count() { return g_gs_count.exchange(0); }
+long ffcsim_pl_count() { return g_pl_count.exchange(0); }
 void ffcsim_set_flags(int flags) { g_sim_flags = flags; }
 static float* g_dk_out = nullptr; static int g_dk_lk = 0;
 void ffcsim_set_fused_dk(float* dk, int Lk) { g_dk_out = dk; g_dk_lk = Lk; }
@@ -766,6 +773,29 @@
     a.pregate = (flags & (1 << 20)) ? buf : nullptr; d.dpre = (flags & (1 << 21)) ? buf : nullptr;
     out[1] = bwd_route<GEO>(d, false).gs;
     out[2] = bwd_route<GEO>(d, true).gs;
+  });
+  return 0;
+}
+
+int ffcsim_launch_plain(int N, int dtype, int B, int H, int L, int flags, int* out) {
+  HostPlan p;
+  if (!build_plan(N, dtype, &p)) return -1;
+  static char buf[16];
+  DkfArgs d{};
+  ConvArgs& a = d.c;
+  a.B = B; a.H = H; a.L = L; a.npair = (B + 1) / 2; a.nchunk = 1; a.R = p.R; a.flags = flags & 0xffff;
+  a.zsave = (flags & (1 << 16)) ? buf : nullptr;
+  a.fast = (flags & (1 << 19)) ? 1 : 0;
+  with_geo(N, [&](auto geo) {
+    using GEO = decltype(geo);
+    ConvArgs f = a;
+    f.pregate = (flags & (1 << 20)) ? buf : nullptr; f.aux_in = (flags & (1 << 21)) ? buf : nullptr;
+    out[0] = fwd_route<GEO>(f).pl;
+    a.postgate = (flags & (1 << 20)) ? buf : nullptr;
+    d.zin = a.zsave; a.zsave = nullptr;
+    if (flags & (3 << 21)) d.dpost = buf;
+    d.yraw = (flags & (1 << 21)) ? buf : nullptr;
+    out[1] = bwd_route<GEO>(d, false).pl;
   });
   return 0;
 }
```

Measured after the change: 11.28 million seq/s, median of 6. 1.4% higher.
